# jaswon/osu-dreamer

Hardware: AMD Instinct MI355X
Metric: denoiser train-steps/sec + 50-step sample latents/sec, 1/2/4/8 MI355X (higher is better)
Workload: dtype bf16

## Files before the change

include/osu_dreamer_hip.h:

```cpp
#ifndef OSU_DREAMER_HIP_H
#define OSU_DREAMER_HIP_H

#ifdef __cplusplus
extern "C" {
#endif

enum { OD_F32 = 0, OD_BF16 = 1,
       OD_F32X3 = 2,
       OD_F32X3W = 3,
       OD_F16 = 4 };
enum { OD_EPI_NONE = 0, OD_EPI_SILU = 1 };
enum { OD_ACT_NONE = 0, OD_ACT_SILU = 1 };
enum { OD_ERR_ARG = -1, OD_ERR_ALIGN = -2, OD_ERR_UNSUPPORTED = -3, OD_ERR_COMM = -4 };

int od_version(void);
const char* od_build_source_sha(void);
const char* od_error_string(int code);

int od_gemm_nt(int dtype, const void* A, int lda, const void* W, int ldw, const float* bias, void* C, int ldc,
               int M, int N, int K, int epilogue, int accumulate, void* stream);
int od_gemm_nt_qkrope(int dtype, const void* A, int lda, const void* W, int ldw, const float* bias, void* C, int ldc, int M,
                      int N, int K, const float* wq, const float* wk, const float* table, int L, int H, int hd, float eps,
                      float q_scale, void* stream);
int od_gemm_nt_qkrope_split(int dtype, const void* A, int lda, const void* W, int ldw, const float* bias, void* C, int ldc,
                            void* qk_out, int ldqk, int qk_dtype, int M, int N, int K, const float* wq, const float* wk, const float* table,
                            int L, int H, int hd, float eps, float q_scale, void* stream);
int od_gemm_tn(int dtype, const void* G, int ldg, const void* A, int lda, float* dW, int lddw, float* dbias, int M, int N,
               int K, void* stream);
int od_gemm_tn_blocks(int dtype, const void* G, int ldg, const void* A, int lda, float* dW, int lddw, float* dbias, int M, int N,
                      int K, int n_block, int n_valid, void* stream);
int od_colsum(int dtype, const void* G, int ldg, float* out, int M, int N, void* stream);
int od_pack_weight(int dtype, const float* src, int N, int K, void* dst, int Np, int Kp, int transpose,
                   const int* row_map, void* stream);

int od_linear_small(const float* x, const float* W, const float* b, float* out, float* pre, int B, int N, int K, int act,
                    void* stream);
int od_linear_small_bwd(const float* x, const float* W, const float* pre, const float* dout, float* dpre, float* dW,
                        float* db, float* dx, int accumulate_dx, int B, int N, int K, int act, void* stream);

int od_cl_to_frames(int dtype, const float* src, void* dst, int ldd, int B, int C, int L, void* stream);
int od_feed_gather(const float* store, long store_elems, const long* base, const long* cstride, const int* lens, float* out,
                   int N, int C, int Lpad, void* stream);
int od_feed_gather_quant(const void* store, long store_bytes, int elem_size, const long* base, const long* cstride, const int* lens,
                         const double* scale, const double* offset, const int* flip, float* out, int N, int C, int c0, int Ctot,
                         int Lpad, void* stream);
int od_replicate_tail(float* x, const int* lens, const int* plens, int N, int C, int Lpad, void* stream);
int od_proj_in(int dtype, const float* xt, const float* W, const float* bias, void* x, int ldx, int B, int E, int L,
               int D, void* stream);
int od_proj_in_bwd(int dtype, const float* xt, const void* dx, int ldx, float* dW, float* db, int B, int E, int L, int D,
                   void* stream);
int od_silu(int dtype, const void* x, void* y, long n, void* stream);
int od_silu_bwd(int dtype, const void* x, const void* dy, void* dx, long n, void* stream);

int od_rmsnorm_film(int dtype, const void* x, int ldx, const float* ssg, const void* cl, int ldcl, int cl_bcast,
                    void* h, int ldh, float* inv_rms, int B, int L, int C, float eps, void* stream);
int od_rmsnorm_film_bwd(int dtype, const void* x, int ldx, const float* inv_rms, const float* ssg, const void* dh,
                        int lddh, void* dres, int lddres, float* dssg, int B, int L, int C, void* stream);
int od_rmsnorm_gate_residual(int dtype, const void* x, int ldx, const void* h, int ldh, const float* ssg, void* xo,
                             int ldxo, float* inv_rms, int B, int L, int C, float eps, void* stream);
int od_rmsnorm_gate_residual_film(int dtype, const void* x, int ldx, const void* h, int ldh, const float* ssg_a, void* xo, int ldxo,
                                  float* inv_a, const float* ssg_b, const void* cl, int ldcl, int cl_bcast, void* h2, int ldh2,
                                  float* inv_b, int B, int L, int C, float eps, void* stream);
int od_rmsnorm_gate_residual_film_dwconv(int dtype, const void* x, int ldx, const void* h, int ldh, const float* ssg_a, void* xo, int ldxo,
                                         float* inv_a, const float* ssg_b, void* h2, int ldh2, float* inv_b, const float* conv_w,
                                         const float* conv_b, void* y, int ldy, int B, int L, int C, int ksize, float eps, void* stream);
int od_rmsnorm_gate_residual_bwd(int dtype, const void* h, int ldh, const float* inv_rms, const float* ssg,
                                 const void* dy, int lddy, void* dh, int lddh, float* dssg, int B, int L, int C,
                                 void* stream);

int od_rope_table(float* table, int L, int hd, void* stream);
int od_qk_norm_rope(int dtype, const void* qkv, int ldqkv, const float* wq, const float* wk, const float* table,
                    void* qk_out, int ldo, int B, int L, int H, int hd, float eps, float q_scale, void* stream);
int od_qk_norm_rope_bwd(int dtype, const void* qkv, int ldqkv, const float* wq, const float* wk, const float* table,
                        const void* dqk, int lddqk, void* dqkv, int lddqkv, float* dwq, float* dwk, int B, int L,
                        int H, int hd, float eps, float q_scale, void* stream);
int od_flash_attn_fwd(int dtype, const void* q, int ldq, const void* k, int ldk, const void* v, int ldv, void* o, int ldo,
                      float* lse, int B, int H, int L, int hd, float scale, int q_prescaled, void* stream);
int od_flash_attn_fwd_varlen(int dtype, const void* q, int ldq, const void* k, int ldk, const void* v, int ldv, void* o, int ldo,
                             float* lse, const int* lens, int B, int H, int L, int hd, float scale, int q_prescaled, void* stream);
int od_flash_attn_bwd(int dtype, const void* q, int ldq, const void* k, int ldk, const void* v, int ldv, const void* o,
                      int ldo, const void* dout, int lddo, const float* lse, float* delta, void* dq, int lddq, void* dk,
                      int lddk, void* dv, int lddv, int B, int H, int L, int hd, float scale, int q_prescaled, void* stream);
int od_attn_aux_create(void** aux_out);
int od_attn_aux_destroy(void* aux);
int od_flash_attn_bwd_aux(int dtype, const void* q, int ldq, const void* k, int ldk, const void* v, int ldv, const void* o,
                          int ldo, const void* dout, int lddo, const float* lse, float* delta, void* dq, int lddq, void* dk,
                          int lddk, void* dv, int lddv, int B, int H, int L, int hd, float scale, int q_prescaled, void* aux, void* stream);
int od_flash_attn_bwd_varlen(int dtype, const void* q, int ldq, const void* k, int ldk, const void* v, int ldv, const void* o,
                             int ldo, const void* dout, int lddo, const float* lse, float* delta, void* dq, int lddq, void* dk,
                             int lddk, void* dv, int lddv, const int* lens, int B, int H, int L, int hd, float scale, int q_prescaled,
                             void* aux, void* stream);
int od_flash_attn_bwd_fused_ws_bytes(int dtype, int B, int H, int L, long* total_out, long* zero_out);
int od_flash_attn_bwd_fused(int dtype, const void* q, int ldq, const void* k, int ldk, const void* v, int ldv, const void* o, int ldo,
                            const void* dout, int lddo, const float* lse, void* dq, int lddq, void* dk, int lddk, void* dv, int lddv,
                            int B, int H, int L, int hd, float scale, int q_prescaled, void* ws, long ws_bytes, void* stream);
int od_flash_attn_bwd_fused_status(const void* ws, int* err_out, void* stream);
int od_flash_attn_bwd_fused_err_offset(void);
int od_flash_attn_bwd_fused_passes(void);
int od_flash_attn_bwd_fused_prof(void* ws, long* out16);
int od_flash_attn_bwd_passes(void);

int od_dwconv(int dtype, const void* x, int ldx, const float* w, const float* bias, void* y, int ldy, int B, int L,
              int C, int ksize, void* stream);
int od_dwconv_varlen(int dtype, const void* x, int ldx, const float* w, const float* bias, void* y, int ldy, const int* lens,
                     int B, int L, int C, int ksize, void* stream);
int od_dwconv_bwd(int dtype, const void* x, int ldx, const float* w, const void* dy, int lddy, void* dx, int lddx,
                  float* dw, float* db, int B, int L, int C, int ksize, void* stream);
int od_dwconv_bwd_varlen(int dtype, const void* x, int ldx, const float* w, const void* dy, int lddy, void* dx, int lddx,
                         float* dw, float* db, const int* lens, int B, int L, int C, int ksize, void* stream);
int od_scale_channels(int dtype, void* x, int ldx, const float* scale, int B, int L, int C, void* stream);
int od_swiglu_rmsnorm(int dtype, const void* vg, int ldvg, void* hh, int ldhh, float* inv_rms, int M, int Hf, int Hp,
                      float eps, void* stream);
int od_swiglu_rmsnorm_bwd(int dtype, const void* vg, int ldvg, const float* inv_rms, const void* dhh, int lddhh,
                          void* dvg, int lddvg, int M, int Hf, int Hp, void* stream);

int od_final_norm_proj_out(int dtype, const void* x, int ldx, const float* W, const float* bias, float* v,
                           float* inv_rms, int B, int L, int C, int E, float eps, void* stream);
int od_final_norm_proj_out_bwd(int dtype, const void* x, int ldx, const float* inv_rms, const float* W, const float* dv,
                               void* dx, int lddx, float* dW, float* db, int B, int L, int C, int E, void* stream);
int od_uhead_fwd(const float* xt, const float* w0, const float* b0, const float* w1, const float* b1, const float* w3,
                 const float* b3, const float* w4, const float* b4, float* fsum, int B, int E, int L, int U,
                 void* stream);
int od_uhead_fwd_varlen(const float* xt, const float* w0, const float* b0, const float* w1, const float* b1, const float* w3,
                        const float* b3, const float* w4, const float* b4, float* fsum, const int* lens, int B, int E, int L,
                        int U, void* stream);
int od_uhead_bwd(const float* xt, const float* w0, const float* b0, const float* w1, const float* b1, const float* w3,
                 const float* b3, const float* w4, const float* b4, const float* dfm, float* dw0, float* db0, float* dw1,
                 float* db1, float* dw3, float* db3, float* dw4, float* db4, int B, int E, int L, int U, void* stream);
int od_uhead_bwd_varlen(const float* xt, const float* w0, const float* b0, const float* w1, const float* b1, const float* w3,
                        const float* b3, const float* w4, const float* b4, const float* dfm, float* dw0, float* db0, float* dw1,
                        float* db1, float* dw3, float* db3, float* dw4, float* db4, const int* lens, int B, int E, int L, int U,
                        void* stream);
int od_uhead_tail(const float* fsum, const float* mod, const float* w_out, const float* b_out, float* u, int B, int U,
                  int L, float u_scale, void* stream);
int od_uhead_tail_varlen(const float* fsum, const float* mod, const float* w_out, const float* b_out, float* u, const int* lens,
                         int B, int U, int L, float u_scale, void* stream);
int od_uhead_tail_bwd(const float* fsum, const float* mod, const float* w_out, const float* b_out, const float* du,
                      float* dfm, float* dmod, float* dw_out, float* db_out, int B, int U, int L, float u_scale,
                      void* stream);
int od_uhead_tail_bwd_varlen(const float* fsum, const float* mod, const float* w_out, const float* b_out, const float* du,
                             float* dfm, float* dmod, float* dw_out, float* db_out, const int* lens, int B, int U, int L,
                             float u_scale, void* stream);

int od_make_xt(const float* x0, const float* x1, const float* t, float* xt, float* dsq, int B, int E, int L, void* stream);
int od_make_xt_varlen(const float* x0, const float* x1, const float* t, float* xt, float* dsq, const int* lens, int B, int E, int L,
                      void* stream);
int od_loss_grad(const float* xt, const float* x1, const float* u, const float* v, const float* dsq, float* dv,
                 float* sums, int B, int E, int L, float c0, float osl_w, float del_w, void* stream);
int od_loss_grad_varlen(const float* xt, const float* x1, const float* u, const float* v, const float* dsq, float* dv,
                        float* sums, const int* lens, int B, int E, int L, float c0, float osl_w, float del_w, void* stream);
int od_loss_finalize(const float* sums, const float* dsq, const float* u, float* out, float* du, int B, float c0,
                     float osl_w, float del_w, void* stream);
int od_sampler_step(float* x, const float* u, const float* v, const float* eta, int B, int E, int L, void* stream);
int od_sampler_eta(const float* u, float* eta, int B, float c0, int num_steps, void* stream);
int od_sampler_eta_groups(const float* u, const int* offs, float* eta, int G, float c0, int num_steps, void* stream);
int od_sampler_step_varlen(float* x, const float* u, const float* v, const float* eta, const int* lens, const int* offs, int G,
                           int B, int E, int L, void* stream);

int od_det_clear(void);
int od_det_register(const float* base, long count, void* shadow_i64);
int od_det_enable(void* table_dev, void* stream);
int od_det_table_bytes(void);
int od_det_flush(float* dst, long count, void* stream);

int od_sqnorm(const float* g, long n, float* out, const int* status, void* stream);
int od_adamw_ema(float* p, const float* g, float* m, float* v, float* ema, long n, float lr, float beta1, float beta2,
                 float eps, float weight_decay, int step, float ema_decay, int ema_mode, const float* gnorm_sq,
                 float max_norm, const int* status, void* stream);

int od_ema_update(float* ema, const float* p, long n, float ema_decay, int ema_mode, void* stream);

int od_style_conditioning(const float* labels, const float* rff_w, const float* rff_b, const float* cond_w,
                          const float* cond_b, const float* null_labels, float* c, int B, int NL, int F, int H,
                          void* stream);
int od_rmsnorm_rows(const float* x, const float* gamma, float* y, int M, int C, float eps, void* stream);

int od_style_conditioning_bwd(const float* labels, const float* rff_w, const float* rff_b, const float* dc, float* dcond_w,
                              float* dcond_b, float* dnull_labels, int B, int NL, int F, int H, void* stream);
int od_rmsnorm_rows_bwd(const float* x, const float* gamma, const float* dy, float* dx, float* dgamma, int M, int C, float eps,
                        int accumulate_dx, void* stream);
int od_cast_rows(int src_dtype, const void* src, int dst_dtype, void* dst, long n, void* stream);

int od_spec_features_conv(int dtype, const float* audio, const float* w1, const float* b1, const float* g1, const float* w2,
                          const float* b2, const float* g2, void* out, int ldo, int B, int F, int L, float eps, void* stream);
int od_rmsnorm_affine_film(int dtype, const void* x, int ldx, const float* gamma, const float* ssg, void* y, int ldy, int B,
                           int L, int C, float eps, int act, void* stream);
int od_rmsnorm_affine_gate_residual(int dtype, const void* x, int ldx, const void* h, int ldh, const float* gamma,
                                    const float* ssg, void* xo, int ldxo, int B, int L, int C, float eps, void* stream);
int od_unet_mixer(int dtype, const void* x, int ldx, const void* p, int ldp, int p_bcast, const void* gx, int ldg,
                  const float* gamma, void* xo, int ldxo, int B, int L, int C, float eps, void* stream);
int od_unet_down(int dtype, const void* x, int ldx, const float* w, const float* bias, void* y, int ldy, int B, int Lo, int C,
                 int stride, void* stream);
int od_unet_up(int dtype, const void* x, int ldx, const float* w, const float* bias, void* y, int ldy, int B, int Li, int C,
               int stride, void* stream);
int od_chart_head(int dtype, const void* x, int ldx, const float* W, const float* bias, float* out, int B, int L, int C, int N,
                  int n_sigmoid, int rms, float eps, void* stream);
int od_attn_pool(int dtype, const void* scores, int lds, const void* values, int ldv, float* out, int B, int L, int Hh, int hd,
                 void* stream);
int od_latent_bwd_block_frames(int C);
int od_rmsnorm_affine_film_bwd(int dtype, const void* x, int ldx, const float* gamma, const float* ssg, const void* dy, int lddy, void* dx,
                               int lddx, int accumulate_dx, float* dgamma, float* dssg, float* ws, long ws_floats, int B, int L, int C,
                               float eps, int act, void* stream);
int od_rmsnorm_affine_gate_residual_bwd(int dtype, const void* h, int ldh, const float* gamma, const float* ssg, const void* dxo, int lddxo,
                                        void* dh, int lddh, float* dgamma, float* dssg, float* ws, long ws_floats, int B, int L, int C,
                                        float eps, void* stream);
int od_unet_mixer_bwd(int dtype, const void* p, int ldp, int p_bcast, const void* gx, int ldg, const float* gamma, const void* dxo,
                      int lddxo, void* dp, int lddp, void* dgx, int lddg, float* dgamma, float* ws, long ws_floats, int B, int L, int C,
                      float eps, void* stream);
int od_unet_down_bwd(int dtype, const void* x, int ldx, const float* w, const void* dy, int lddy, void* dx, int lddx, float* dw, float* db,
                     float* ws, long ws_floats, int B, int Lo, int C, int stride, void* stream);
int od_unet_up_bwd(int dtype, const void* x, int ldx, const float* w, const void* dy, int lddy, void* dx, int lddx, float* dw, float* db,
                   float* ws, long ws_floats, int B, int Li, int C, int stride, void* stream);
int od_chart_head_bwd(int dtype, const void* x, int ldx, const float* W, const float* bias, const float* dout, void* dx, int lddx,
                      float* dW, float* db, float* ws, long ws_floats, int B, int L, int C, int N, int rms, float eps, void* stream);
int od_attn_pool_bwd(int dtype, const void* scores, int lds, const void* values, int ldv, const float* dout, void* dscores, int ldds,
                     void* dvalues, int lddv, int B, int L, int Hh, int hd, void* stream);
int od_spec_features_conv_bwd(int dtype, const float* audio, const float* w1, const float* b1, const float* g1, const float* w2,
                              const float* b2, const float* g2, const void* dout, int ldo, float* dw1, float* db1, float* dg1, float* dw2,
                              float* db2, float* dg2, float* ws, long ws_floats, int B, int F, int L, float eps, void* stream);
int od_add_rows(int dtype, const void* x, void* y, long n, void* stream);
int od_proj_in_bwd_input(int dtype, const void* dx, int ldx, const float* W, float* dxt, int B, int E, int L, int D, void* stream);

int od_mmd_imq(const float* z, const float* prior, float* out, float* dz, float* ws, long ws_floats, int N, int D, void* stream);
int od_scale_by(const float* x, const float* g, float* y, long n, void* stream);
int od_latent_perturb(const float* z, long zsb, long zse, long zsl, const float* s, const float* eps_z, const float* eps_s,
                      const float* u_s, const float* repl, const float* u_span, const float* u_start, float* z_out, float* s_out,
                      void* masked, void* start_span, int B2, int E, int l, int S, float s_noise, float z_noise, float s_mask_frac,
                      float z_mask_frac, int training, void* stream);
int od_latent_perturb_bwd(const float* dz_out, const float* ds_out, const void* masked, const int* start_span, float* dz, float* ds,
                          int B2, int E, int l, int S, void* stream);
int od_latent_loss_block_frames(void);
int od_latent_loss_ws_floats(int B2, int L);
int od_latent_loss(const float* logits, const float* chart, const float* pred_labels, const float* true_labels, const void* masked,
                   const float* s_reg, float* loss_ema, void* ema_init, float* out, float* coef, float* ws, long ws_floats, int B2, int L,
                   float s_reg_weight, int training, void* stream);
int od_latent_loss_bwd(const float* logits, const float* chart, const float* pred_labels, const float* true_labels, const void* masked,
                       const float* coef, const float* g, float* dlogits, float* dlabels, float* ds_reg, int B2, int L,
                       float s_reg_weight, void* stream);

int od_mmd_imq_pairs(const float* s, const float* prior, float* out, float* ws, long ws_floats, int G, int S, void* stream);
int od_latent_loss_maps(const float* logits, const float* chart, const int* hlens, const float* pred_labels, const float* true_labels,
                        const float* s_reg, int s_reg_stride, const float* loss_ema, float* out, float* ws, long ws_floats, int G,
                        int Hmax, float s_reg_weight, void* stream);
int od_latent_eval_maps_ws_floats(int G, int Pmax);
int od_latent_eval_maps(const float* chart, const float* pred_chart, const int* plens, const float* z, const int* zlens,
                        const float* pred_labels, const float* true_labels, float* out, float* ws, long ws_floats, int G, int Pmax, int E,
                        int lmax, void* stream);

int od_spec_features_conv_varlen(int dtype, const float* audio, const float* w1, const float* b1, const float* g1, const float* w2,
                                 const float* b2, const float* g2, void* out, int ldo, const int* lens, int B, int F, int L, float eps,
                                 void* stream);
int od_rmsnorm_affine_film_varlen(int dtype, const void* x, int ldx, const float* gamma, const float* ssg, void* y, int ldy,
                                  const int* lens, int B, int L, int C, float eps, int act, void* stream);
int od_unet_mixer_varlen(int dtype, const void* x, int ldx, const void* p, int ldp, const int* prow, const void* gx, int ldg,
                         const float* gamma, void* xo, int ldxo, int B, int L, int C, float eps, void* stream);
int od_unet_down_varlen(int dtype, const void* x, int ldx, const float* w, const float* bias, void* y, int ldy, const int* lens,
                        int B, int Lo, int C, int stride, void* stream);
int od_unet_up_varlen(int dtype, const void* x, int ldx, const float* w, const float* bias, void* y, int ldy, const int* lens,
                      int B, int Li, int C, int stride, void* stream);
int od_chart_head_varlen(int dtype, const void* x, int ldx, const float* W, const float* bias, float* out, const int* lens, int B,
                         int L, int C, int N, int n_sigmoid, int rms, float eps, void* stream);
int od_attn_pool_varlen(int dtype, const void* scores, int lds, const void* values, int ldv, float* out, const int* lens, int B,
                        int L, int Hh, int hd, void* stream);

int od_comm_load(const char* path);
int od_comm_version(void);
int od_comm_unique_id(void* out, int nbytes);
int od_comm_init(void** comm_out, int nranks, int rank, const void* unique_id, int nbytes);
int od_comm_destroy(void* comm);
int od_comm_abort(void* comm);
int od_comm_count(void* comm);
int od_comm_ring_standin(float* buf, long count, int channels, int threads, int rounds, void* stream);
int od_allreduce_grads(void* comm, float* grads, long count, int average, void* stream);
int od_broadcast_f32(void* comm, float* buf, long count, int root, void* stream);

int od_graph_begin(void* stream);
int od_graph_end(void* stream, void** graph_exec_out);
int od_graph_launch(void* graph_exec, void* stream);
int od_graph_destroy(void* graph_exec);

int od_mfma_calibrate(float* scratch, int iters, double* flops_out, void* stream);

#ifdef __cplusplus
}
#endif
#endif
```

osu_dreamer_amd/csrc/attn_bwd_fused.hip:

```cpp
#include "od_common.h"
#include "od_tiles.h"
#include "od_api_internal.h"
#include <type_traits>
#include <stddef.h>
#include <stdlib.h>

namespace {

constexpr float FB_LOG2E = 1.4426950408889634f;
constexpr float FB_LN2 = 0.6931471805599453f;

constexpr int FB_NK = 3;
constexpr int FB_KB = 4 * FB_NK * 16;
constexpr int FB_TILE = 64 * 128;
constexpr int FB_STAGE = 2 * FB_TILE + 512;
constexpr int FB_DS = FB_KB * 128;
#ifndef FB_NSLOTS
#define FB_NSLOTS 4
#endif
constexpr int FB_SLOTS = FB_NSLOTS;
#ifndef FB_PACK
#define FB_PACK 1
#endif
constexpr int FB_NP = FB_PACK ? 3 : 4;
constexpr int FB_RUN_TILE = 4 * FB_NP * 64 * 4;
constexpr int FB_KST = 2 * FB_STAGE + 2 * FB_DS;
constexpr int FB_SMEM = FB_KST + FB_DS + 16;

#ifndef FB_ORDER
#define FB_ORDER 3
#endif
#ifndef FB_REQ
#define FB_REQ 2
#endif
#ifndef FB_SPLIT
#define FB_SPLIT 1
#endif
#ifndef FB_X
#define FB_X 0
#endif

#if defined(OD_EMU)
#define FB_INLINE
#else
#define FB_INLINE __attribute__((always_inline))
#endif
#ifndef FB_PROF
#define FB_PROF 0
#endif
#if FB_PROF && !defined(OD_EMU)
#define FB_CLK() __builtin_readcyclecounter()
#else
#define FB_CLK() 0ull
#endif

struct FbSync {
    int head[8];
    int finished;
    int jobs_done;
    int err;
    int calls;
    int shape[3];
    int pad;
    unsigned long long prof[16];
};

__device__ __forceinline__ unsigned fb_f2u(float x) { return __builtin_bit_cast(unsigned, x); }
__device__ __forceinline__ float fb_u2f(unsigned x) { return __builtin_bit_cast(float, x); }

__device__ __forceinline__ float fb_poison() {
#if defined(OD_EMU)
    volatile unsigned bits = 0x7fc00000u;
    return fb_u2f(bits);
#else
    float x;
    asm volatile("v_mov_b32 %0, 0x7fc00000" : "=v"(x));
    return x;
#endif
}

__device__ __forceinline__ int fb_swz(int row) { return (row & 7) ^ (((row >> 3) & 1) << 2); }

#if defined(OD_EMU)
__device__ __forceinline__ int fb_xcc_id() { return (int)(blockIdx.x & 7); }
__device__ __forceinline__ int fb_flag_load(const int* p) { return *p; }
__device__ __forceinline__ void fb_flag_store(int* p, int v) { *p = v; }
struct fb_rsrc_t { const unsigned char* base; };
__device__ __forceinline__ fb_rsrc_t fb_make_rsrc(const float* base, unsigned) { return fb_rsrc_t{(const unsigned char*)base}; }
__device__ __forceinline__ f32x4 fb_ld_l2(fb_rsrc_t r, unsigned voff, unsigned soff) { return *(const f32x4*)(r.base + voff + soff); }
__device__ __forceinline__ void fb_st_run(float* p, f32x4 t) { *(f32x4*)p = t; }
__device__ __forceinline__ void fb_sleep() {}
__device__ __forceinline__ unsigned long long fb_now(unsigned polls) { return polls; }
__device__ __forceinline__ int fb_atomic_inc(int* p) { return atomicAdd(p, 1); }
#define FB_WAIT_ALL() ((void)0)
#define FB_COMPILER_FENCE() ((void)0)
#define FB_WAIT_BUT(n) ((void)0)
#else
__device__ __forceinline__ int fb_xcc_id() {
    int v;
    asm volatile("s_getreg_b32 %0, hwreg(HW_REG_XCC_ID)" : "=s"(v));
    return v & 7;
}
__device__ __forceinline__ int fb_flag_load(const int* p) { return __hip_atomic_load(p, __ATOMIC_RELAXED, __HIP_MEMORY_SCOPE_AGENT); }
__device__ __forceinline__ void fb_flag_store(int* p, int v) { __hip_atomic_store(p, v, __ATOMIC_RELAXED, __HIP_MEMORY_SCOPE_AGENT); }
#ifndef FB_LD_AUX
#define FB_LD_AUX 2
#endif
typedef __amdgpu_buffer_rsrc_t fb_rsrc_t;
__device__ __forceinline__ fb_rsrc_t fb_make_rsrc(const float* base, unsigned bytes) {
    return __builtin_amdgcn_make_buffer_rsrc((void*)base, 0, (int)bytes, 0x00020000);
}
__device__ __forceinline__ f32x4 fb_ld_l2(fb_rsrc_t r, unsigned voff, unsigned soff) {
    return __builtin_bit_cast(f32x4, __builtin_amdgcn_raw_buffer_load_b128(r, (int)voff, (int)soff, FB_LD_AUX));
}
#ifndef FB_ST_POLICY
#define FB_ST_POLICY 0
#endif
__device__ __forceinline__ void fb_st_run(float* p, f32x4 t) {
#if FB_X & 16
    asm volatile("" :: "v"(t));
#elif FB_ST_POLICY == 0
    *(f32x4*)p = t;
#elif FB_ST_POLICY == 1
    asm volatile("global_store_dwordx4 %0, %1, off nt\n\ts_nop 0" :: "v"(p), "v"(t) : "memory");
#elif FB_ST_POLICY == 2
    asm volatile("global_store_dwordx4 %0, %1, off sc1\n\ts_nop 0" :: "v"(p), "v"(t) : "memory");
#else
    asm volatile("global_store_dwordx4 %0, %1, off sc0 sc1\n\ts_nop 0" :: "v"(p), "v"(t) : "memory");
#endif
}
__device__ __forceinline__ void fb_sleep() { __builtin_amdgcn_s_sleep(4); }
__device__ __forceinline__ unsigned long long fb_now(unsigned) { return __builtin_amdgcn_s_memrealtime(); }
__device__ __forceinline__ int fb_atomic_inc(int* p) { return __hip_atomic_fetch_add(p, 1, __ATOMIC_RELAXED, __HIP_MEMORY_SCOPE_AGENT); }
#define FB_WAIT_ALL() asm volatile("s_waitcnt vmcnt(0)" ::: "memory")
#define FB_COMPILER_FENCE() asm volatile("" ::: "memory")
#define FB_WAIT_BUT(n) asm volatile("s_waitcnt vmcnt(" #n ")" ::: "memory")
#endif

__global__ __launch_bounds__(256) void fb_prep_kernel(const bf16_t* __restrict__ o, int ldo, const bf16_t* __restrict__ dout, int lddo,
                                                      const float* __restrict__ lse, float* __restrict__ nl, float* __restrict__ nd,
                                                      int B, int H, int L, float inv_scale) {
    const int lane = threadIdx.x & 63;
    const long m = (long)blockIdx.x * 4 + (threadIdx.x >> 6);
    if (m >= (long)B * L) return;
    const int b = (int)(m / L), l = (int)(m % L);
    const int nch = H * 8;
    for (int it = 0; it * 64 < nch; it++) {
        const int qd = it * 64 + lane;
        const bool act = qd < nch;
        float s = 0.f;
        if (act) {
            float a[8], d[8];
            od_ld8(o + m * ldo + qd * 8, a); od_ld8(dout + m * lddo + qd * 8, d);
#pragma unroll
            for (int e = 0; e < 8; e++) s += a[e] * d[e];
        }
        s += __shfl_xor(s, 1); s += __shfl_xor(s, 2); s += __shfl_xor(s, 4);
        if (act && (qd & 7) == 0) {
            const size_t i = ((size_t)b * H + (qd >> 3)) * L + l;
            nd[i] = -s;
            nl[i] = -lse[i] * inv_scale;
        }
    }
}

__global__ __launch_bounds__(256) void fb_amax_kernel(const bf16_t* __restrict__ dout, int lddo, long M, int dh, unsigned* __restrict__ amax_bits) {
    const int nch = dh / 8;
    float m = 0.f;
    for (long i = (long)blockIdx.x * 256 + threadIdx.x; i < M * nch; i += (long)gridDim.x * 256) {
        float d[8];
        od_ld8(dout + (i / nch) * lddo + (i % nch) * 8, d);
#pragma unroll
        for (int e = 0; e < 8; e++) m = fmaxf(m, fabsf(d[e]));
    }
#pragma unroll
    for (int s = 32; s >= 1; s >>= 1) m = fmaxf(m, __shfl_xor(m, s));
    if ((threadIdx.x & 63) == 0 && m > 0.f) atomicMax(amax_bits, fb_f2u(m));
}
__device__ __forceinline__ float fb_dscale_of(unsigned amax_bits) {
    const unsigned e = (amax_bits >> 23) & 0xffu;
    if (amax_bits == 0u || e == 0u || e == 0xffu) return 1.0f;
    const int ex = (int)e - 127 + ((amax_bits & 0x7fffffu) ? 1 : 0);
    int se = 2 - ex; se = se < -100 ? -100 : se > 100 ? 100 : se;
    return fb_u2f((unsigned)(se + 127) << 23);
}
__global__ __launch_bounds__(256) void fb_prep_f16_kernel(const bf16_t* __restrict__ o, int ldo, const bf16_t* __restrict__ dout, int lddo,
                                                          const float* __restrict__ lse, float* __restrict__ nl, float* __restrict__ nd,
                                                          f16_t* __restrict__ do16, int ldd16, const unsigned* __restrict__ amax_bits,
                                                          float* __restrict__ dscale_out, int B, int H, int L, float inv_scale) {
    const float ds = fb_dscale_of(amax_bits[0]);
    if (blockIdx.x == 0 && threadIdx.x == 0) dscale_out[0] = ds;
    const int lane = threadIdx.x & 63;
    const long m = (long)blockIdx.x * 4 + (threadIdx.x >> 6);
    if (m >= (long)B * L) return;
    const int b = (int)(m / L), l = (int)(m % L);
    const int nch = H * 8;
    for (int it = 0; it * 64 < nch; it++) {
        const int qd = it * 64 + lane;
        const bool act = qd < nch;
        float s = 0.f;
        if (act) {
            float a[8], d[8];
            od_ld8(o + m * ldo + qd * 8, a); od_ld8(dout + m * lddo + qd * 8, d);
#pragma unroll
            for (int e = 0; e < 8; e++) { s += a[e] * d[e]; d[e] *= ds; }
            od_st8(do16 + m * ldd16 + qd * 8, d);
        }
        s += __shfl_xor(s, 1); s += __shfl_xor(s, 2); s += __shfl_xor(s, 4);
        if (act && (qd & 7) == 0) {
            const size_t i = ((size_t)b * H + (qd >> 3)) * L + l;
            nd[i] = -s * ds;
            nl[i] = -lse[i] * inv_scale;
        }
    }
}

template <bool PRE, class TA>
__global__ __launch_bounds__(512, 2) void flash_bwd_fused_kernel(const bf16_t* __restrict__ q, int ldq, const bf16_t* __restrict__ k, int ldk,
                                                                 const bf16_t* __restrict__ v, int ldv, const bf16_t* __restrict__ dout, int lddo,
                                                                 const float* __restrict__ nl, const float* __restrict__ nd,
                                                                 bf16_t* __restrict__ dq, int lddq, bf16_t* __restrict__ dk, int lddk,
                                                                 bf16_t* __restrict__ dv, int lddv, float* __restrict__ run,
                                                                 FbSync* __restrict__ sync, int B, int H, int L, float scale,
                                                                 unsigned wait_ticks, const float* __restrict__ dscale_p) {
    constexpr int NK = FB_NK, KB = FB_KB;
    OD_DYN_SMEM(smem);
    int* const s_job = (int*)(smem + FB_KST + FB_DS);
    const int BH = B * H, nkb = (L + KB - 1) / KB, nqt = (L + 63) / 64;
    const int jobs_per_xcd = ((BH + 7) / 8) * nkb;
    const int lane = threadIdx.x & 63, wave = od_uniform(threadIdx.x >> 6), x = lane & 15, g = lane >> 4;
    const bool key_wave = wave < 4;
    const int xcc = fb_xcc_id();
    const int calls = sync->calls;
    {
        const int s0 = sync->shape[0], s1 = sync->shape[1], s2 = sync->shape[2];
        if ((s0 | s1 | s2) != 0 && (s0 != B || s1 != H || s2 != L)) {
            if (blockIdx.x == 0 && threadIdx.x == 0) fb_flag_store(&sync->err, 2);
            return;
        }
    }
    const float inv_ds = std::is_same<TA, f16_t>::value ? 1.0f / dscale_p[0] : 1.0f;
    const float c = scale * FB_LOG2E, out_scale = (PRE ? FB_LN2 : scale) * inv_ds;
    int my_jobs = 0;

    if (threadIdx.x == 0) s_job[0] = fb_atomic_inc(&sync->head[xcc]);
    __syncthreads();
    int job = od_uniform(s_job[0]), jpar = 0;
    auto run_jobs = [&](auto role_) FB_INLINE {
    constexpr bool KEY_ROLE = decltype(role_)::value;
    for (;; jpar ^= 1) {
        if (job >= jobs_per_xcd) break;
        my_jobs++;
        const int bh = (job / nkb) * 8 + xcc, kblk = job % nkb;
        if (bh >= BH) {
            __syncthreads();
            if (threadIdx.x == 0) s_job[jpar ^ 1] = fb_atomic_inc(&sync->head[xcc]);
            __syncthreads();
            job = od_uniform(s_job[jpar ^ 1]);
            continue;
        }
        const int b = bh / H, h = bh % H;
        const bf16_t* qb = q + (size_t)b * L * ldq + h * 64;
        const bf16_t* kb_ = k + (size_t)b * L * ldk + h * 64;
        const bf16_t* vb = v + (size_t)b * L * ldv + h * 64;
        const bf16_t* dob = dout + (size_t)b * L * lddo + h * 64;
        const bool kragged = kblk * KB + KB > L;
#ifndef FB_PRIO
#define FB_PRIO 0
#endif
        if constexpr (KEY_ROLE) {
            if (FB_PRIO) __builtin_amdgcn_s_setprio(FB_PRIO);
            const int key0 = kblk * KB + wave * NK * 16;
            od_frag<TA> fk[NK][2], fv[NK][2];
#pragma unroll
            for (int ki = 0; ki < NK; ki++) {
                int row = key0 + ki * 16 + x; row = row < L ? row : L - 1;
#pragma unroll
                for (int s = 0; s < 2; s++) {
                    od_frag_load(fk[ki][s], (const TA*)(kb_ + (size_t)row * ldk + s * 32 + g * 8));
                    od_frag_load(fv[ki][s], (const TA*)(vb + (size_t)row * ldv + s * 32 + g * 8));
                }
            }
            f32x4 dkacc[NK][4], dvacc[NK][4];
#pragma unroll
            for (int ki = 0; ki < NK; ki++)
#pragma unroll
                for (int dt = 0; dt < 4; dt++) { dkacc[ki][dt] = (f32x4)(0.f); dvacc[ki][dt] = (f32x4)(0.f); }
            const int ds_off0 = (wave * 48 + x) * 128 + ((g ^ fb_swz(x)) << 4);
            __syncthreads();
            unsigned long long pk_bar = 0;
            int next_job = 0;
            auto tile = [&](int qt, auto masked_t) FB_INLINE {
                constexpr bool MASKED = decltype(masked_t)::value;
                const bool last_tile = qt == nqt - 1;
                if (last_tile && threadIdx.x == 0) next_job = fb_atomic_inc(&sync->head[xcc]);
                const unsigned char* st = smem + (qt & 1) * FB_STAGE;
                unsigned char* dsb = smem + 2 * FB_STAGE + (qt & 1) * FB_DS;
                const unsigned char* tQ = st;
                const unsigned char* tO = st + FB_TILE;
                const float* s_nl = (const float*)(st + 2 * FB_TILE);
                const float* s_nd = s_nl + 64;
                const int qbase = qt * 64;
#pragma unroll
                for (int u = 0; u < 2; u++) {
                    od_frag<TA> fp[NK], fds[NK];
#pragma unroll
                    for (int th = 0; th < 2; th++) {
                        const int t4 = 2 * u + th;
                        od_frag<TA> fqr[2], fdo[2];
#pragma unroll
                        for (int s = 0; s < 2; s++) {
                            if ((FB_X & 1024) && t4) { fqr[s] = fk[0][s]; fdo[s] = fv[0][s]; continue; }
                            frag_contig<128>(fqr[s], tQ, t4 * 16 + x, s * 32 + g * 8);
                            frag_contig<128>(fdo[s], tO, t4 * 16 + x, s * 32 + g * 8);
                        }
                        const f32x4 l4 = *(const f32x4*)(s_nl + t4 * 16 + 4 * g);
                        const f32x4 d4 = *(const f32x4*)(s_nd + t4 * 16 + 4 * g);
#pragma unroll
                        for (int ki = 0; ki < NK; ki++) {
                            f32x4 sa_ = l4, pa_ = d4;
#pragma unroll
                            for (int s = 0; s < 2; s++) { sa_ = od_mma(fqr[s], fk[ki][s], sa_); pa_ = od_mma(fdo[s], fv[ki][s], pa_); }
                            f32x4 e = sa_;
                            if constexpr (!PRE) e = od_mul4s(sa_, c);
                            f32x4 p;
#pragma unroll
                            for (int r = 0; r < 4; r++) p[r] = (FB_X & 256) ? e[r] : od_exp2(e[r]);
                            if constexpr (MASKED) {
                                const bool kvalid = key0 + ki * 16 + x < L;
#pragma unroll
                                for (int r = 0; r < 4; r++)
                                    if (!(kvalid && (qbase + t4 * 16 + 4 * g + r < L))) p[r] = 0.f;
                            }
                            const f32x4 ds = od_mul4(p, pa_);
                            od_frag_set4(fp[ki], th, p[0], p[1], p[2], p[3]);
                            od_frag_set4(fds[ki], th, ds[0], ds[1], ds[2], ds[3]);
                        }
                    }
                    od_frag<TA> fot[2], fqt[2];
                    frag_cols<128, 128>(fot[0], tO, tO, 0, x, u, g);
                    frag_cols<128, 128>(fqt[0], tQ, tQ, 0, x, u, g);
#pragma unroll
                    for (int dt = 0; dt < 4; dt++) {
                        if (dt < 3 && !(FB_X & 512)) {
                            frag_cols<128, 128>(fot[(dt + 1) & 1], tO, tO, (dt + 1) * 16, x, u, g);
                            frag_cols<128, 128>(fqt[(dt + 1) & 1], tQ, tQ, (dt + 1) * 16, x, u, g);
                        }
                        if (dt < NK && !(FB_X & 4)) *(s16x8*)(dsb + ((ds_off0 ^ (u * 64)) + dt * 2048)) = fds[dt].v;
                        __builtin_amdgcn_sched_barrier(0);
#pragma unroll
                        for (int ki = 0; ki < NK; ki++) {
                            dvacc[ki][dt] = od_mma(fot[dt & 1], fp[ki], dvacc[ki][dt]);
                            dkacc[ki][dt] = od_mma(fqt[dt & 1], fds[ki], dkacc[ki][dt]);
                        }
                        __builtin_amdgcn_sched_barrier(0);
                    }
                }
                if (last_tile && threadIdx.x == 0) s_job[jpar ^ 1] = next_job;
                const unsigned long long tb0 = FB_CLK();
                __syncthreads();
                pk_bar += FB_CLK() - tb0;
            };
            const unsigned long long tk0 = FB_CLK();
            const int nfull = kragged ? 0 : L / 64;
            for (int qt = 0; qt < nfull; qt++) tile(qt, std::false_type{});
            for (int qt = nfull; qt < nqt; qt++) tile(qt, std::true_type{});
            if (FB_PROF && threadIdx.x == 0) { atomicAdd(&sync->prof[0], pk_bar); atomicAdd(&sync->prof[1], FB_CLK() - tk0); }
#pragma unroll
            for (int ki = 0; ki < NK; ki++) {
                const int row = key0 + ki * 16 + x;
                if (row < L) {
                    bf16_t* dkr = dk + ((size_t)b * L + row) * lddk + h * 64;
                    bf16_t* dvr = dv + ((size_t)b * L + row) * lddv + h * 64;
#pragma unroll
                    for (int dt = 0; dt < 4; dt++) {
                        const f32x4 a = dkacc[ki][dt] * out_scale, e = dvacc[ki][dt] * inv_ds;
                        u32x2 w0, w1;
                        w0[0] = od_pack_bf2(a[0], a[1]); w0[1] = od_pack_bf2(a[2], a[3]);
                        w1[0] = od_pack_bf2(e[0], e[1]); w1[1] = od_pack_bf2(e[2], e[3]);
                        *(u32x2*)(dkr + dt * 16 + 4 * g) = w0;
                        *(u32x2*)(dvr + dt * 16 + 4 * g) = w1;
                    }
                }
            }
        } else {
            const int hh = wave - 4;
            constexpr int NJ = FB_SPLIT == 0 ? 1 : FB_SPLIT == 1 ? 4 : 2, NG = 4 / NJ;
            auto ji_of = [](int a) FB_INLINE { return FB_SPLIT == 0 ? 0 : FB_SPLIT == 1 ? a : a >> 1; };
            auto gi_of = [](int a) FB_INLINE { return FB_SPLIT == 0 ? a : FB_SPLIT == 1 ? 0 : a & 1; };
            const int j0 = FB_SPLIT == 0 ? hh : FB_SPLIT == 1 ? 0 : 2 * (hh & 1), G0 = FB_SPLIT == 0 ? 0 : FB_SPLIT == 1 ? hh : 2 * (hh >> 1);
            od_frag<TA> fkt[NJ][6];
            const od_srd_t rq = od_make_srd(qb, (unsigned)(((size_t)(L - 1) * ldq + 64) * 2));
            const od_srd_t ro = od_make_srd(dob, (unsigned)(((size_t)(L - 1) * lddo + 64) * 2));
            const od_srd_t rs = od_make_srd((hh == 0 ? nl : nd) + (size_t)bh * L, (unsigned)L * 4u);
            const int prow = lane >> 3, pslot = (lane & 7) ^ prow;
            const unsigned vq = (unsigned)((hh * 8 + prow) * ldq * 2 + pslot * 16), vo = (unsigned)((hh * 8 + prow) * lddo * 2 + pslot * 16);
            const unsigned smem_a = od_lds_addr(smem);
            const od_srd_t rk = od_make_srd(kb_, (unsigned)(((size_t)(L - 1) * ldk + 64) * 2));
            auto stage_k = [&]() FB_INLINE {
#pragma unroll
                for (int i = 0; i < 6; i++) {
                    const int pc = hh + 4 * i;
                    const int r = 8 * pc + (lane >> 3);
                    const unsigned vk = (unsigned)((lane >> 3) * ldk * 2 + (((lane & 7) ^ fb_swz(r)) << 4));
                    od_buffer_lds16_at(rk, vk, (unsigned)od_uniform((kblk * KB + 8 * pc) * ldk * 2), (unsigned)od_uniform((int)(smem_a + (unsigned)FB_KST + (unsigned)pc * 1024u)));
                }
            };
            int trk[NJ][2];
#pragma unroll
            for (int ji = 0; ji < NJ; ji++)
#pragma unroll
                for (int e = 0; e < 2; e++) {
                    const int row = 8 * g + (x >> 2) + 4 * e;
                    trk[ji][e] = row * 128 + (((2 * (j0 + ji) + ((x & 3) >> 1)) ^ fb_swz(row)) << 4) + (x & 1) * 8;
                }
            auto dma_piece = [&](int qt, int j) FB_INLINE {
                const unsigned st = (unsigned)od_uniform((int)(smem_a + (unsigned)((qt & 1) * FB_STAGE) + (unsigned)hh * 1024u));
                const unsigned qi = (unsigned)od_uniform(qt);
                const unsigned sq = qi * 64u * (unsigned)ldq * 2u, so = qi * 64u * (unsigned)lddo * 2u;
                if (j == 0) od_buffer_lds16_at(rq, vq, sq, st);
                if (j == 1) od_buffer_lds16_at(rq, vq, sq + 32u * (unsigned)ldq * 2u, st + 4096);
                if (j == 2) od_buffer_lds16_at(ro, vo, so, st + FB_TILE);
                if (j == 3) od_buffer_lds16_at(ro, vo, so + 32u * (unsigned)lddo * 2u, st + FB_TILE + 4096);
                if (j == 4 && hh < 2) od_buffer_lds4_at(rs, (unsigned)lane * 4u, qi * 256u, (unsigned)od_uniform((int)(st + 2 * FB_TILE - (unsigned)hh * 768u)));
            };
            auto dma = [&](int qt) FB_INLINE {
                qt = od_uniform(qt);
#pragma unroll
                for (int j = 0; j < 5; j++) dma_piece(qt, j);
            };
            int tr_off[NG][2], qcol[NG];
#pragma unroll
            for (int gi = 0; gi < NG; gi++) {
                const int G = G0 + gi;
#pragma unroll
                for (int e = 0; e < 2; e++) {
                    const int row = 8 * g + (x >> 2) + 4 * e;
                    tr_off[gi][e] = row * 128 + (((2 * G + ((x & 3) >> 1)) ^ fb_swz(row)) << 4) + (x & 1) * 8;
                }
                qcol[gi] = 16 * (2 * (G >> 1) + ((x >> 2) & 1)) + 4 * (2 * (G & 1) + (x >> 3)) + (x & 3);
            }

            f32x4 acc[4][4], rb[FB_NP];
            bool poisoned = false;
            unsigned long long ph[6] = {0, 0, 0, 0, 0, 0};
            const size_t tile_f = FB_RUN_TILE;
            const bool last = kblk == nkb - 1;
            const int bhq = bh >> 3, slot = bhq % FB_SLOTS, gen = bhq / FB_SLOTS;
            const int nbhq_x = (BH - xcc + 7) >> 3;
            const int gens = (nbhq_x - slot + FB_SLOTS - 1) / FB_SLOTS;
            const unsigned id_mine = (unsigned)od_uniform((int)((1u + ((unsigned)calls * (unsigned)gens + (unsigned)gen) * (unsigned)nkb + (unsigned)kblk) & 0xfffu)), id_pred = (id_mine - 1u) & 0xfffu;
            auto tag_of = [](unsigned id, int r) FB_INLINE -> unsigned { return (id >> (3 * r)) & 7u; };
            auto phase_b = [&](int tau, f32x4 (&a)[4], auto&& between) FB_INLINE {
                const unsigned char* dsb = smem + 2 * FB_STAGE + (tau & 1) * FB_DS;
                s16x4 f[2][NG][2];
                auto rd = [&](int s, s16x4 (&dst)[NG][2]) FB_INLINE {
#pragma unroll
                    for (int gi = 0; gi < NG; gi++)
#pragma unroll
                        for (int e = 0; e < 2; e++) dst[gi][e] = od_lds_tr_read((const bf16_t*)(dsb + s * 4096 + tr_off[gi][e]));
                };
                rd(0, f[0]);
#pragma unroll
                for (int s = 0; s < 6; s++) {
                    if (s + 1 < 6) rd(s + 1, f[(s + 1) & 1]);
                    __builtin_amdgcn_sched_barrier(0);
                    od_frag<TA> fb[NG];
#pragma unroll
                    for (int gi = 0; gi < NG; gi++) {
                        const s16x4 b0 = f[s & 1][gi][0], b1 = f[s & 1][gi][1];
                        fb[gi].v[0] = b0[0]; fb[gi].v[1] = b0[1]; fb[gi].v[2] = b0[2]; fb[gi].v[3] = b0[3];
                        fb[gi].v[4] = b1[0]; fb[gi].v[5] = b1[1]; fb[gi].v[6] = b1[2]; fb[gi].v[7] = b1[3];
                    }
#pragma unroll
                    for (int G = 0; G < 4; G++) a[G] = od_mma(fkt[ji_of(G)][s], fb[gi_of(G)], s == 0 ? (f32x4)(0.f) : a[G]);
                    __builtin_amdgcn_sched_barrier(0);
                    between(s);
                }
            };
            const size_t rbh = (size_t)od_uniform(xcc * FB_SLOTS + slot);
            const fb_rsrc_t run_rs = fb_make_rsrc(run + rbh * nqt * tile_f, (unsigned)((size_t)nqt * tile_f * 4));
            const unsigned run_vo = (unsigned)((hh * (FB_NP * 256) + lane * 4) * 4);
            float* const run_st = run + rbh * nqt * tile_f + (size_t)hh * (FB_NP * 256) + (size_t)lane * 4;
            auto chain_load = [&](int tau, f32x4 (&r4)[FB_NP]) FB_INLINE {
#pragma unroll
                for (int G = 0; G < FB_NP; G++) r4[G] = fb_ld_l2(run_rs, run_vo + G * 1024, (unsigned)((FB_X & 8) ? 0 : tau) * (unsigned)(FB_RUN_TILE * 4));
            };
            auto tags_good = [&](f32x4 (&r4)[FB_NP]) FB_INLINE -> bool {
                unsigned bad = 0;
#if FB_PACK
#pragma unroll
                for (int P = 0; P < FB_NP; P++) bad |= ((fb_f2u(r4[P][3]) >> 14) ^ id_pred) & 0x3ffu;
                if (FB_X & 32) return true;
                return !__any(bad != 0);
#else
#pragma unroll
                for (int G = 0; G < 4; G++)
#pragma unroll
                    for (int r = 0; r < 4; r++) bad |= fb_f2u(r4[G][r]) ^ tag_of(id_pred, r);
                if (FB_X & 32) return true;
                return !__any((bad & 7u) != 0);
#endif
            };
#if FB_PACK
            auto fb_unpack = [&](const f32x4 (&r4)[FB_NP], float (&v)[16]) FB_INLINE {
                unsigned last = 0;
#pragma unroll
                for (int P = 0; P < 3; P++) {
                    const unsigned d0 = fb_f2u(r4[P][0]), d1 = fb_f2u(r4[P][1]), d2 = fb_f2u(r4[P][2]), d3 = fb_f2u(r4[P][3]);
                    v[5 * P + 0] = fb_u2f(d0 << 10);
                    v[5 * P + 1] = fb_u2f(((d0 >> 22) | (d1 << 10)) << 10);
                    v[5 * P + 2] = fb_u2f(((d1 >> 12) | (d2 << 20)) << 10);
                    v[5 * P + 3] = fb_u2f((d2 << 8) & 0xfffffc00u);
                    v[5 * P + 4] = fb_u2f(((d2 >> 24) | (d3 << 8)) << 10);
                    last |= (d3 >> 24) << (P == 0 ? 0 : P == 1 ? 8 : 15);
                }
                v[15] = fb_u2f(last << 10);
            };
            auto fb_pack = [&](const float (&v)[16], unsigned id, f32x4 (&out)[FB_NP]) FB_INLINE {
                unsigned u[16];
#pragma unroll
                for (int i = 0; i < 16; i++) u[i] = (fb_f2u(v[i]) + 0x200u) >> 10;
#pragma unroll
                for (int P = 0; P < 3; P++) {
                    const unsigned a0 = u[5 * P], a1 = u[5 * P + 1], a2 = u[5 * P + 2], a3 = u[5 * P + 3], a4 = u[5 * P + 4];
                    const unsigned ex = P == 0 ? (u[15] & 0xffu) : P == 1 ? ((u[15] >> 8) & 0x7fu) : (u[15] >> 15);
                    out[P][0] = fb_u2f(a0 | (a1 << 22));
                    out[P][1] = fb_u2f((a1 >> 10) | (a2 << 12));
                    out[P][2] = fb_u2f((a2 >> 20) | (a3 << 2) | (a4 << 24));
                    out[P][3] = fb_u2f((a4 >> 8) | ((id & 0x3ffu) << 14) | (ex << 24));
                }
            };
#endif
            auto chain_commit = [&](int tau, f32x4 (&a)[4]) FB_INLINE {
#if FB_PACK
                {
                    float rv[16];
                    fb_unpack(rb, rv);
                    if (poisoned) {
#pragma unroll
                        for (int i = 0; i < 16; i++) rv[i] = fb_poison();
                    }
#pragma unroll
                    for (int G = 0; G < 4; G++)
#pragma unroll
                        for (int r = 0; r < 4; r++) a[G][r] += rv[4 * G + r];
                }
                if (!last) {
                    float sv[16];
#pragma unroll
                    for (int G = 0; G < 4; G++)
#pragma unroll
                        for (int r = 0; r < 4; r++) sv[4 * G + r] = a[G][r];
                    f32x4 t3[FB_NP];
                    fb_pack(sv, id_mine, t3);
#pragma unroll
                    for (int P = 0; P < FB_NP; P++) fb_st_run(run_st + (size_t)((FB_X & 8) ? 0 : tau) * tile_f + P * 256, t3[P]);
                } else {
#else
#pragma unroll
                for (int G = 0; G < 4; G++)
#pragma unroll
                    for (int r = 0; r < 4; r++) a[G][r] += fb_u2f(fb_f2u(rb[G][r]) & ~7u);
                if (!last) {
#pragma unroll
                    for (int G = 0; G < 4; G++) {
                        f32x4 t;
#pragma unroll
                        for (int r = 0; r < 4; r++) t[r] = fb_u2f((fb_f2u(a[G][r]) & ~7u) | tag_of(id_mine, r));
                        fb_st_run(run_st + (size_t)((FB_X & 8) ? 0 : tau) * tile_f + G * 256, t);
                    }
                } else {
#endif
#pragma unroll
                    for (int G = 0; G < 4; G++) {
                        const int qrow = tau * 64 + qcol[gi_of(G)];
                        if (qrow < L) {
                            u32x2 w;
                            w[0] = od_pack_bf2(a[G][0] * out_scale, a[G][1] * out_scale);
                            w[1] = od_pack_bf2(a[G][2] * out_scale, a[G][3] * out_scale);
                            *(u32x2*)(dq + ((size_t)b * L + qrow) * lddq + h * 64 + 16 * (j0 + ji_of(G)) + 4 * g) = w;
                        }
                    }
                    f32x4 t;
#if FB_PACK
                    t[0] = t[1] = t[2] = 0.f; t[3] = fb_u2f((id_mine & 0x3ffu) << 14);
#else
#pragma unroll
                    for (int r = 0; r < 4; r++) t[r] = fb_u2f(tag_of(id_mine, r));
#endif
#pragma unroll
                    for (int G = 0; G < FB_NP; G++) fb_st_run(run_st + (size_t)((FB_X & 8) ? 0 : tau) * tile_f + G * 256, t);
                }
            };
            auto commit_dyn = [&](int tau) FB_INLINE {
                switch (tau & 3) {
                    case 0: chain_commit(tau, acc[0]); break;
                    case 1: chain_commit(tau, acc[1]); break;
                    case 2: chain_commit(tau, acc[2]); break;
                    default: chain_commit(tau, acc[3]); break;
                }
            };
            int done = 0;
            bool inflight = false, aborted = false;
            auto chain_request = [&](int produced) FB_INLINE {
                if ((FB_X & 1) || inflight || done >= produced) return;
                if (!(FB_X & 64)) chain_load(done, rb);
                inflight = true;
            };
            auto chain_try = [&](int produced, int must_reach) FB_INLINE -> bool {
                if (FB_X & 1) { done = produced; return false; }
                bool four = false;
                if (done < produced) {
                    if (inflight) {
                        inflight = false;
                        if (tags_good(rb)) { commit_dyn(done); done++; four = !last; }
                        else if (FB_PROF) ph[5]++;
                    }
                }
                while (done < must_reach) {
                    four = false;
                    if (!aborted) {
                        unsigned long long t_start = 0;
                        for (unsigned polls = 0;; polls++) {
                            FB_COMPILER_FENCE();
                            chain_load(done, rb);
                            if (tags_good(rb)) break;
                            if ((polls & 15u) == 15u) {
                                const unsigned long long now = fb_now(polls);
                                if (polls == 15u) t_start = now;
                                else if (now - t_start > (unsigned long long)wait_ticks) aborted = true;
                                if (od_uniform(fb_flag_load(&sync->err)) == 3) aborted = true;
                                if (aborted) break;
                            }
                            fb_sleep();
                        }
                    }
                    if (aborted) {
                        if (lane == 0) fb_flag_store(&sync->err, 3);
#pragma unroll
                        for (int G = 0; G < FB_NP; G++) rb[G] = (f32x4)(fb_poison());
                        poisoned = true;
                    }
                    commit_dyn(done);
                    poisoned = false;
                    done++;
                }
                return four;
            };
            auto step = [&](int it, auto k_) FB_INLINE {
                constexpr int K = decltype(k_)::value;
                const unsigned long long t0 = FB_CLK();
                const int nxt = od_uniform(it + 1);
                const unsigned long long t1 = FB_CLK();
                if (!(FB_X & 2)) phase_b(it - 1, acc[(K + 3) & 3], [&](int s) FB_INLINE {
#if FB_ORDER == 2
                    if (s < 5) { if (nxt < nqt) dma_piece(nxt, s); }
                    else chain_request(it - 1);
#elif FB_ORDER == 1
                    if (s == 0) chain_request(it - 1);
                    else if (nxt < nqt) dma_piece(nxt, s - 1);
#else
                    if (s < 2) { if (nxt < nqt) { dma_piece(nxt, 2 * s); dma_piece(nxt, 2 * s + 1); } }
                    else if (s == 2) { if (nxt < nqt) dma_piece(nxt, 4); }
                    if (s == FB_REQ) chain_request(it - 1);
#endif
                });
                else { chain_request(it - 1); if (nxt < nqt) dma(nxt); }
#if FB_PROF && !defined(OD_EMU)
                asm volatile("" : "+v"(acc[(K + 3) & 3][0]), "+v"(acc[(K + 3) & 3][1]), "+v"(acc[(K + 3) & 3][2]), "+v"(acc[(K + 3) & 3][3]));
#endif
                const unsigned long long t2 = FB_CLK();
                FB_WAIT_ALL();
                const unsigned long long t3 = FB_CLK();
                const bool four = chain_try(it, it - 3);
                const unsigned long long t4 = FB_CLK();
                (void)four;
                od_barrier_raw();
                if (FB_PROF) { const unsigned long long t5 = FB_CLK(); ph[0] += t1 - t0; ph[1] += t2 - t1; ph[2] += t3 - t2; ph[3] += t4 - t3; ph[4] += t5 - t4; }
            };
            OD_DRAIN_VMEM();
            stage_k();
            dma(0);
            FB_WAIT_ALL();
            od_barrier_raw();
#pragma unroll
            for (int s = 0; s < 6; s++)
#pragma unroll
                for (int ji = 0; ji < NJ; ji++) {
                    const s16x4 b0 = od_lds_tr_read((const bf16_t*)(smem + FB_KST + s * 4096 + trk[ji][0]));
                    const s16x4 b1 = od_lds_tr_read((const bf16_t*)(smem + FB_KST + s * 4096 + trk[ji][1]));
                    fkt[ji][s].v[0] = b0[0]; fkt[ji][s].v[1] = b0[1]; fkt[ji][s].v[2] = b0[2]; fkt[ji][s].v[3] = b0[3];
                    fkt[ji][s].v[4] = b1[0]; fkt[ji][s].v[5] = b1[1]; fkt[ji][s].v[6] = b1[2]; fkt[ji][s].v[7] = b1[3];
                }
            if (1 < nqt) dma(1);
            FB_WAIT_ALL();
            od_barrier_raw();
            int it = 1;
            for (; it + 3 < nqt; it += 4) {
                step(it, std::integral_constant<int, 1>{}); step(it + 1, std::integral_constant<int, 2>{});
                step(it + 2, std::integral_constant<int, 3>{}); step(it + 3, std::integral_constant<int, 0>{});
            }
            if (it < nqt) { step(it, std::integral_constant<int, 1>{}); it++; }
            if (it < nqt) { step(it, std::integral_constant<int, 2>{}); it++; }
            if (it < nqt) { step(it, std::integral_constant<int, 3>{}); it++; }
            if (!(FB_X & 2)) {
                auto nothing = [](int) FB_INLINE {};
                switch ((nqt - 1) & 3) {
                    case 0: phase_b(nqt - 1, acc[0], nothing); break;
                    case 1: phase_b(nqt - 1, acc[1], nothing); break;
                    case 2: phase_b(nqt - 1, acc[2], nothing); break;
                    default: phase_b(nqt - 1, acc[3], nothing); break;
                }
            }
            inflight = false;
            chain_try(nqt, nqt);
            if (FB_PROF && threadIdx.x == 256) { for (int i = 0; i < 6; i++) atomicAdd(&sync->prof[2 + i], ph[i]); }
            FB_WAIT_ALL();
        }
        job = od_uniform(s_job[jpar ^ 1]);
    }
    };
    if (key_wave) run_jobs(std::true_type{}); else run_jobs(std::false_type{});
    if (threadIdx.x == 0) {
        if (my_jobs) {
#if defined(OD_EMU)
            sync->jobs_done += my_jobs;
#else
            __hip_atomic_fetch_add(&sync->jobs_done, my_jobs, __ATOMIC_RELAXED, __HIP_MEMORY_SCOPE_AGENT);
#endif
        }
#if !defined(OD_EMU)
        __builtin_amdgcn_fence(__ATOMIC_RELEASE, "agent");
        asm volatile("s_waitcnt vmcnt(0)" ::: "memory");
#endif
        const int t = fb_atomic_inc(&sync->finished);
        if (t == (int)gridDim.x - 1) {
#if !defined(OD_EMU)
            __builtin_amdgcn_fence(__ATOMIC_ACQUIRE, "agent");
#endif
            const int done = fb_flag_load(&sync->jobs_done);
            if (done != 8 * jobs_per_xcd) fb_flag_store(&sync->err, 1);
            for (int i = 0; i < 8; i++) fb_flag_store(&sync->head[i], 0);
            fb_flag_store(&sync->jobs_done, 0);
            fb_flag_store(&sync->calls, sync->calls + 1);
            fb_flag_store(&sync->shape[0], B); fb_flag_store(&sync->shape[1], H); fb_flag_store(&sync->shape[2], L);
            fb_flag_store(&sync->finished, 0);
        }
    }
}

inline size_t fb_align(size_t n) { return (n + 255) & ~(size_t)255; }
struct FbLayout { size_t sync, nl, nd, run, aux, do16, total; };
inline FbLayout fb_layout(int B, int H, int L, bool f16 = false) {
    const size_t BH = (size_t)B * H, nqt = (size_t)(L + 63) / 64;
    FbLayout l;
    l.sync = 0;
    l.run = fb_align(sizeof(FbSync));
    l.nl = l.run + fb_align((size_t)8 * FB_SLOTS * nqt * FB_RUN_TILE * sizeof(float));
    l.nd = l.nl + fb_align(BH * L * sizeof(float));
    l.aux = l.nd + fb_align(BH * L * sizeof(float));
    l.do16 = l.aux + 256;
    l.total = f16 ? l.do16 + fb_align(BH * L * 64 * sizeof(unsigned short)) : l.aux;
    return l;
}

inline unsigned fb_wait_ticks() {
    static const unsigned ticks = [] {
        const char* e = getenv("OD_FB_CHAIN_TIMEOUT_MS");
        long ms = e ? atol(e) : 1000;
        if (ms < 1) ms = 1;
        if (ms > 40000) ms = 40000;
#if defined(OD_EMU)
        return (unsigned)1024;
#else
        return (unsigned)(ms * 100000);
#endif
    }();
    return ticks;
}

}

extern "C" int od_flash_attn_bwd_fused_ws_bytes(int dtype, int B, int H, int L, long* total_out, long* zero_out) {
    if (B <= 0 || H <= 0 || L <= 0 || !total_out || !zero_out || (dtype != OD_BF16 && dtype != OD_F16)) return OD_ERR_ARG;
    const FbLayout lay = fb_layout(B, H, L, dtype == OD_F16);
    *total_out = (long)lay.total;
    *zero_out = (long)lay.nl;
    return 0;
}
extern "C" int od_flash_attn_bwd_fused_err_offset(void) { return (int)offsetof(FbSync, err); }
extern "C" int od_flash_attn_bwd_fused_passes(void) { return 5; }
extern "C" int od_flash_attn_bwd_fused_prof(void* ws, long* out16) {
    if (!ws || !out16) return OD_ERR_ARG;
    FbSync s;
#if defined(OD_EMU)
    s = *(FbSync*)ws;
#else
    if (hipDeviceSynchronize() != hipSuccess) return OD_ERR_ARG;
    if (hipMemcpy(&s, ws, sizeof(s), hipMemcpyDeviceToHost) != hipSuccess) return OD_ERR_ARG;
    if (hipMemset((unsigned char*)ws + offsetof(FbSync, prof), 0, sizeof(s.prof)) != hipSuccess) return OD_ERR_ARG;
#endif
    for (int i = 0; i < 16; i++) out16[i] = (long)s.prof[i];
    return 0;
}

extern "C" int od_flash_attn_bwd_fused(int dtype, const void* q, int ldq, const void* k, int ldk, const void* v, int ldv, const void* o, int ldo,
                                       const void* dout, int lddo, const float* lse, void* dq, int lddq, void* dk, int lddk, void* dv, int lddv,
                                       int B, int H, int L, int hd, float scale, int q_prescaled, void* ws, long ws_bytes, void* stream) {
    if ((dtype != OD_BF16 && dtype != OD_F16) || hd != 64) return OD_ERR_UNSUPPORTED;
    if (!ws || B <= 0 || H <= 0 || L <= 0) return OD_ERR_ARG;
    if (ldq % 8 || ldk % 8 || ldv % 8 || ldo % 8 || lddo % 8 || lddq % 8 || lddk % 8 || lddv % 8) return OD_ERR_ALIGN;
    const bool f16 = dtype == OD_F16;
    const FbLayout lay = fb_layout(B, H, L, f16);
    if (ws_bytes < (long)lay.total) return OD_ERR_ARG;
    if (((size_t)L * (size_t)(ldq > lddo ? (ldq > ldk ? ldq : ldk) : (lddo > ldk ? lddo : ldk))) * 2 >= 0xffffffffull) return OD_ERR_UNSUPPORTED;
    hipStream_t st = (hipStream_t)stream;
    unsigned char* w = (unsigned char*)ws;
    float* nl = (float*)(w + lay.nl);
    float* nd = (float*)(w + lay.nd);
    const long M = (long)B * L;
    const float inv_scale = q_prescaled ? FB_LOG2E : 1.0f / scale;
    const float* dscale_p = nullptr;
    if (f16) {
        unsigned* amax = (unsigned*)(w + lay.aux);
        float* dsc = (float*)(w + lay.aux) + 1;
        f16_t* do16 = (f16_t*)(w + lay.do16);
#if defined(OD_EMU)
        *amax = 0u;
#else
        if (hipMemsetAsync(amax, 0, sizeof(unsigned), st) != hipSuccess) return OD_ERR_ARG;
#endif
        OD_LAUNCH(fb_amax_kernel, dim3(2048), dim3(256), 0, st, (const bf16_t*)dout, lddo, M, H * 64, amax);
        OD_LAUNCH(fb_prep_f16_kernel, dim3((unsigned)((M + 3) / 4)), dim3(256), 0, st, (const bf16_t*)o, ldo, (const bf16_t*)dout, lddo, lse, nl, nd,
                  do16, H * 64, (const unsigned*)amax, dsc, B, H, L, inv_scale);
        dout = do16; lddo = H * 64; dscale_p = dsc;
    } else
        OD_LAUNCH(fb_prep_kernel, dim3((unsigned)((M + 3) / 4)), dim3(256), 0, st, (const bf16_t*)o, ldo, (const bf16_t*)dout, lddo, lse, nl, nd, B, H, L, inv_scale);
    const int grid = od_num_cus();
#define FB_ARGS dim3(grid), dim3(512), FB_SMEM, st, (const bf16_t*)q, ldq, (const bf16_t*)k, ldk, (const bf16_t*)v, ldv, (const bf16_t*)dout, lddo, \
        (const float*)nl, (const float*)nd, (bf16_t*)dq, lddq, (bf16_t*)dk, lddk, (bf16_t*)dv, lddv, (float*)(w + lay.run), (FbSync*)(w + lay.sync), B, H, L, scale, \
        fb_wait_ticks(), dscale_p
#define FB_LAUNCH_X(...) OD_LAUNCH_DYN(__VA_ARGS__)
    if (f16) {
        if (q_prescaled) FB_LAUNCH_X((flash_bwd_fused_kernel<true, f16_t>), FB_ARGS);
        else FB_LAUNCH_X((flash_bwd_fused_kernel<false, f16_t>), FB_ARGS);
    } else {
        if (q_prescaled) FB_LAUNCH_X((flash_bwd_fused_kernel<true, bf16_t>), FB_ARGS);
        else FB_LAUNCH_X((flash_bwd_fused_kernel<false, bf16_t>), FB_ARGS);
    }
#undef FB_LAUNCH_X
#undef FB_ARGS
    OD_CHECK_LAUNCH();
    return 0;
}

extern "C" int od_flash_attn_bwd_fused_status(const void* ws, int* err_out, void* stream) {
    if (!ws || !err_out) return OD_ERR_ARG;
#if defined(OD_EMU)
    (void)stream;
    *err_out = ((const FbSync*)ws)->err;
#else
    int v = -1;
    hipError_t e = hipMemcpyAsync(&v, (const unsigned char*)ws + offsetof(FbSync, err), sizeof(int), hipMemcpyDeviceToHost, (hipStream_t)stream);
    if (e == hipSuccess) e = hipStreamSynchronize((hipStream_t)stream);
    if (e != hipSuccess) return -(int)e - 1000;
    *err_out = v;
#endif
    return 0;
}
```

osu_dreamer_amd/csrc/rowops.hip:

```cpp
#include "od_common.h"
#include "od_api_internal.h"

namespace {

#ifndef OD_QK_BPW
#define OD_QK_BPW 8
#endif
constexpr int ROWS_PER_WAVE_BWD = 16;

template <class T, int NCH>
__device__ __forceinline__ void load_row(const T* row, int C, int lane, float (&v)[NCH][8]) {
#pragma unroll
    for (int i = 0; i < NCH; i++) {
        const int c = (lane + 64 * i) * 8;
        if (c < C) od_ld8(row + c, v[i]);
        else {
#pragma unroll
            for (int e = 0; e < 8; e++) v[i][e] = 0.f;
        }
    }
}
template <int NCH>
__device__ __forceinline__ float row_sumsq(const float (&v)[NCH][8]) {
    float s = 0.f;
// ... 259 lines not shown
#pragma unroll
            for (int k = 0; k < 8; k++) {
                float s = bv[k];
#pragma unroll
                for (int j = 0; j < KS; j++) s += wv[k][j] * win[j][k];
                o[k] = s;
            }
            od_st8(y + ((size_t)b * L + lc) * ldy + c, o);
        }
#pragma unroll
        for (int j = 0; j < KS - 1; j++)
#pragma unroll
            for (int e = 0; e < 8; e++) win[j][e] = win[j + 1][e];
    }
}

template <class T, int NCH>
__global__ __launch_bounds__(256) void rmsnorm_gate_res_bwd_kernel(const T* __restrict__ h, int ldh, const float* __restrict__ inv_rms,
                                                                   const float* __restrict__ ssg, const T* __restrict__ dy, int lddy,
                                                                   T* __restrict__ dh, int lddh, float* __restrict__ dssg,
                                                                   int B, int L, int C, const OdDetTable* __restrict__ det) {
    __shared__ float red[NCH * 512];
    const int lane = threadIdx.x & 63, wave = threadIdx.x >> 6;
    const int b = blockIdx.y;
    const int l0 = (blockIdx.x * 4 + wave) * ROWS_PER_WAVE_BWD;
    float dg[NCH][8], gate[NCH][8];
#pragma unroll
    for (int i = 0; i < NCH; i++) {
        const int c = (lane + 64 * i) * 8;
#pragma unroll
        for (int e = 0; e < 8; e++) { dg[i][e] = 0.f; gate[i][e] = 0.f; }
        if (c < C) od_ld8(ssg + (size_t)b * 3 * C + 2 * C + c, gate[i]);
    }
    for (int r = 0; r < ROWS_PER_WAVE_BWD; r++) {
        const int l = l0 + r;
        if (l >= L) break;
        const long m = (long)b * L + l;
        float hv[NCH][8], gv[NCH][8];
        load_row<T, NCH>(h + m * ldh, C, lane, hv);
        load_row<T, NCH>(dy + m * lddy, C, lane, gv);
        const float inv = inv_rms[m];
        float dot = 0.f;
#pragma unroll
        for (int i = 0; i < NCH; i++)
#pragma unroll
            for (int e = 0; e < 8; e++) {
                const float hh = hv[i][e] * inv;
                dg[i][e] += gv[i][e] * hh;
                gv[i][e] *= gate[i][e];
                dot += gv[i][e] * hh;
                hv[i][e] = hh;
            }
        dot = od_wave_sum(dot) / (float)C;
#pragma unroll
        for (int i = 0; i < NCH; i++) {
            const int c = (lane + 64 * i) * 8;
            if (c >= C) continue;
            float o[8];
#pragma unroll
            for (int e = 0; e < 8; e++) o[e] = inv * (gv[i][e] - hv[i][e] * dot);
            od_st8(dh + m * lddh + c, o);
        }
    }
    for (int w = 0; w < 4; w++) {
        if (wave == w) {
#pragma unroll
            for (int i = 0; i < NCH; i++)
#pragma unroll
                for (int e = 0; e < 8; e++) {
                    const int idx = (lane + 64 * i) * 8 + e;
                    if (w == 0) red[idx] = dg[i][e]; else red[idx] += dg[i][e];
                }
        }
        __syncthreads();
    }
    for (int c = threadIdx.x; c < C; c += 256) od_red_add(det, dssg + (size_t)b * 3 * C + 2 * C + c, red[c]);
}

template <class T, int NCH>
__global__ __launch_bounds__(256) void swiglu_rmsnorm_kernel(const T* __restrict__ vg, int ldvg, T* __restrict__ hh, int ldhh,
                                                             float* __restrict__ inv_rms, long M, int Hf, int Hp, float eps) {
    const int lane = threadIdx.x & 63;
    const long m = (long)blockIdx.x * 4 + (threadIdx.x >> 6);
    if (m >= M) return;
    float v[NCH][8], g[NCH][8];
    load_row<T, NCH>(vg + m * ldvg, Hp, lane, v);
    load_row<T, NCH>(vg + m * ldvg + Hp, Hp, lane, g);
#pragma unroll
    for (int i = 0; i < NCH; i++)
#pragma unroll
        for (int e = 0; e < 8; e++) v[i][e] *= od_silu(g[i][e]);
    const float inv = rsqrtf(row_sumsq<NCH>(v) / (float)Hf + eps);
    if (lane == 0 && inv_rms) inv_rms[m] = inv;
#pragma unroll
    for (int i = 0; i < NCH; i++) {
        const int c = (lane + 64 * i) * 8;
        if (c >= Hp) continue;
        float o[8];
#pragma unroll
        for (int e = 0; e < 8; e++) o[e] = v[i][e] * inv;
        od_st8(hh + m * ldhh + c, o);
    }
}

template <class T, int NCH>
__global__ __launch_bounds__(256) void swiglu_rmsnorm_bwd_kernel(const T* __restrict__ vg, int ldvg, const float* __restrict__ inv_rms,
                                                                 const T* __restrict__ dhh, int lddhh, T* __restrict__ dvg, int lddvg,
                                                                 long M, int Hf, int Hp) {
    const int lane = threadIdx.x & 63;
    const long m = (long)blockIdx.x * 4 + (threadIdx.x >> 6);
    if (m >= M) return;
    float v[NCH][8], g[NCH][8], d[NCH][8];
    load_row<T, NCH>(vg + m * ldvg, Hp, lane, v);
    load_row<T, NCH>(vg + m * ldvg + Hp, Hp, lane, g);
    load_row<T, NCH>(dhh + m * lddhh, Hp, lane, d);
    const float inv = inv_rms[m];
    float dot = 0.f;
    float sg[NCH][8], gs[NCH][8];
#pragma unroll
    for (int i = 0; i < NCH; i++)
#pragma unroll
        for (int e = 0; e < 8; e++) {
            gs[i][e] = od_sigmoid(g[i][e]);
            sg[i][e] = g[i][e] * gs[i][e];
            dot += d[i][e] * (v[i][e] * sg[i][e] * inv);
        }
    dot = od_wave_sum(dot) / (float)Hf;
#pragma unroll
    for (int i = 0; i < NCH; i++) {
        const int c = (lane + 64 * i) * 8;
        if (c >= Hp) continue;
        float ov[8], og[8];
#pragma unroll
        for (int e = 0; e < 8; e++) {
            const float sh = v[i][e] * sg[i][e] * inv;
            const float ds = inv * (d[i][e] - sh * dot);
            ov[e] = ds * sg[i][e];
            og[e] = ds * v[i][e] * (gs[i][e] * (1.0f + g[i][e] * (1.0f - gs[i][e])));
        }
        od_st8(dvg + m * lddvg + c, ov);
        od_st8(dvg + m * lddvg + Hp + c, og);
    }
}

template <class T, int NCH>
__global__ __launch_bounds__(256) void final_proj_kernel(const T* __restrict__ x, int ldx, const float* __restrict__ W,
                                                         const float* __restrict__ bias, float* __restrict__ vout,
                                                         float* __restrict__ inv_rms, int B, int L, int C, int E, float eps) {
    const int lane = threadIdx.x & 63;
    const long m = (long)blockIdx.x * 4 + (threadIdx.x >> 6);
    if (m >= (long)B * L) return;
    const int b = (int)(m / L), l = (int)(m % L);
    float v[NCH][8];
    load_row<T, NCH>(x + m * ldx, C, lane, v);
    const float inv = rsqrtf(row_sumsq<NCH>(v) / (float)C + eps);
    if (lane == 0 && inv_rms) inv_rms[m] = inv;
    for (int e = 0; e < E; e++) {
        float s = 0.f;
#pragma unroll
        for (int i = 0; i < NCH; i++) {
            const int c = (lane + 64 * i) * 8;
            if (c >= C) continue;
            float w[8]; od_ld8(W + (size_t)e * C + c, w);
#pragma unroll
            for (int k = 0; k < 8; k++) s += w[k] * v[i][k];
        }
        s = od_wave_sum(s) * inv;
        if (lane == 0) vout[((size_t)b * E + e) * L + l] = s + bias[e];
    }
}

template <class T, int NCH>
__global__ __launch_bounds__(256) void final_proj_bwd_kernel(const T* __restrict__ x, int ldx, const float* __restrict__ inv_rms,
                                                             const float* __restrict__ W, const float* __restrict__ dv,
                                                             T* __restrict__ dx, int lddx, float* __restrict__ dW,
                                                             float* __restrict__ db, int B, int L, int C, int E,
                                                             const OdDetTable* __restrict__ det) {
    constexpr int MAXE = 8;
    __shared__ float red[MAXE * NCH * 512];
    __shared__ float redb[4][MAXE];
    const int lane = threadIdx.x & 63, wave = threadIdx.x >> 6;
    const int b = blockIdx.y;
    const int l0 = (blockIdx.x * 4 + wave) * ROWS_PER_WAVE_BWD;
    float wv[MAXE][NCH][8], dw[MAXE][NCH][8], dbv[MAXE];
#pragma unroll
    for (int e = 0; e < MAXE; e++) {
        dbv[e] = 0.f;
#pragma unroll
        for (int i = 0; i < NCH; i++) {
            const int c = (lane + 64 * i) * 8;
#pragma unroll
            for (int k = 0; k < 8; k++) { wv[e][i][k] = 0.f; dw[e][i][k] = 0.f; }
            if (e < E && c < C) od_ld8(W + (size_t)e * C + c, wv[e][i]);
        }
    }
    for (int r = 0; r < ROWS_PER_WAVE_BWD; r++) {
        const int l = l0 + r;
        if (l >= L) break;
        const long m = (long)b * L + l;
        float xv[NCH][8], dn[NCH][8], dve[MAXE];
        load_row<T, NCH>(x + m * ldx, C, lane, xv);
        const float inv = inv_rms[m];
#pragma unroll
        for (int e = 0; e < MAXE; e++) { dve[e] = e < E ? dv[((size_t)b * E + e) * L + l] : 0.f; dbv[e] += dve[e]; }
        float dot = 0.f;
#pragma unroll
        for (int i = 0; i < NCH; i++)
#pragma unroll
            for (int k = 0; k < 8; k++) {
                const float xh = xv[i][k] * inv;
                float s = 0.f;
#pragma unroll
                for (int e = 0; e < MAXE; e++) { s += dve[e] * wv[e][i][k]; dw[e][i][k] += dve[e] * xh; }
                dn[i][k] = s;
                dot += s * xh;
                xv[i][k] = xh;
            }
        dot = od_wave_sum(dot) / (float)C;
#pragma unroll
        for (int i = 0; i < NCH; i++) {
            const int c = (lane + 64 * i) * 8;
            if (c >= C) continue;
            float o[8];
#pragma unroll
            for (int k = 0; k < 8; k++) o[k] = inv * (dn[i][k] - xv[i][k] * dot);
            od_st8(dx + m * lddx + c, o);
        }
    }
    if (lane == 0)
        for (int e = 0; e < MAXE; e++) redb[wave][e] = dbv[e];
    for (int w = 0; w < 4; w++) {
        if (wave == w) {
#pragma unroll
            for (int e = 0; e < MAXE; e++)
#pragma unroll
                for (int i = 0; i < NCH; i++)
#pragma unroll
                    for (int k = 0; k < 8; k++) {
                        const int idx = e * NCH * 512 + (lane + 64 * i) * 8 + k;
                        if (w == 0) red[idx] = dw[e][i][k]; else red[idx] += dw[e][i][k];
                    }
        }
        __syncthreads();
    }
    for (int e = 0; e < E; e++)
        for (int c = threadIdx.x; c < C; c += 256) od_red_add(det, dW + (size_t)e * C + c, red[e * NCH * 512 + c]);
    if (threadIdx.x < E) od_red_add(det, db + threadIdx.x, redb[0][threadIdx.x] + redb[1][threadIdx.x] + redb[2][threadIdx.x] + redb[3][threadIdx.x]);
}

template <class T, class TO = T>
__global__ __launch_bounds__(256) void qk_norm_rope_kernel(const T* __restrict__ qkv, int ldqkv, const float* __restrict__ wq,
                                                           const float* __restrict__ wk, const float* __restrict__ table,
                                                           TO* __restrict__ out, int ldo, int B, int L, int H, int hd, float eps,
                                                           float q_scale) {
    const int lane = threadIdx.x & 63;
    const long m = (long)blockIdx.x * 4 + (threadIdx.x >> 6);
    if (m >= (long)B * L) return;
    const int l = (int)(m % L);
    const int lph = hd / 8, half = lph / 2;
    const int nchunks = 2 * H * lph;
    const int niter = (nchunks + 63) / 64;
    for (int it = 0; it < niter; it++) {
        const int q = it * 64 + lane;
        const bool act = q < nchunks;
        const int slot = q / lph, c8 = q % lph;
        float v[8];
        if (act) od_ld8(qkv + m * ldqkv + (size_t)slot * hd + c8 * 8, v);
        else {
#pragma unroll
            for (int e = 0; e < 8; e++) v[e] = 0.f;
        }
        float ss = 0.f;
#pragma unroll
        for (int e = 0; e < 8; e++) ss += v[e] * v[e];
        for (int msk = 1; msk < lph; msk <<= 1) ss += __shfl_xor(ss, msk);
        const float inv = rsqrtf(ss / (float)hd + eps);
        const float* w = (slot < H ? wq : wk) + c8 * 8;
        float y[8], p[8];
#pragma unroll
        for (int e = 0; e < 8; e++) y[e] = act ? v[e] * inv * w[e] : 0.f;
#pragma unroll
        for (int e = 0; e < 8; e++) p[e] = __shfl_xor(y[e], half);
        if (act) {
            const bool first = c8 < half;
            const int j0 = (c8 % half) * 8;
            const float* tb = table + ((size_t)l * (hd / 2) + j0) * 2;
            float o[8];
#pragma unroll
            for (int e = 0; e < 8; e++) {
                const float cs = tb[2 * e], sn = tb[2 * e + 1];
                o[e] = (first ? (y[e] * cs - p[e] * sn) : (p[e] * sn + y[e] * cs)) * (slot < H ? q_scale : 1.f);
            }
            od_st8(out + m * ldo + (size_t)slot * hd + c8 * 8, o);
        }
    }
}

template <class T>
__global__ __launch_bounds__(256) void qk_norm_rope_bwd_kernel(const T* __restrict__ qkv, int ldqkv, const float* __restrict__ wq,
                                                               const float* __restrict__ wk, const float* __restrict__ table,
                                                               const T* __restrict__ dqk, int lddqk, T* __restrict__ dqkv, int lddqkv,
                                                               float* __restrict__ dwq, float* __restrict__ dwk,
                                                               int B, int L, int H, int hd, float eps, float q_scale,
                                                               const OdDetTable* __restrict__ det) {
    __shared__ long long sdw[2][256];
    __shared__ int s_bad;
    const int lane = threadIdx.x & 63, wave = threadIdx.x >> 6;
    for (int i = threadIdx.x; i < 512; i += 256) sdw[i >> 8][i & 255] = 0;
    if (threadIdx.x == 0) s_bad = 0;
    __syncthreads();
    const int lph = hd / 8, half = lph / 2;
    const int nchunks = 2 * H * lph;
    const int niter = (nchunks + 63) / 64;
    float aq[8], ak[8];
#pragma unroll
    for (int e = 0; e < 8; e++) { aq[e] = 0.f; ak[e] = 0.f; }
    const long M = (long)B * L;
    const long mbase = ((long)blockIdx.x * 4 + wave) * ROWS_PER_WAVE_BWD;
    for (int r = 0; r < ROWS_PER_WAVE_BWD; r++) {
        const long m = mbase + r;
        if (m >= M) break;
        const int l = (int)(m % L);
        for (int it = 0; it < niter; it++) {
            const int q = it * 64 + lane;
            const bool act = q < nchunks;
            const int slot = q / lph, c8 = q % lph;
            float v[8], d[8];
            if (act) {
                od_ld8(qkv + m * ldqkv + (size_t)slot * hd + c8 * 8, v); od_ld8(dqk + m * lddqk + (size_t)slot * hd + c8 * 8, d);
                if (slot < H) {
#pragma unroll
                    for (int e = 0; e < 8; e++) d[e] *= q_scale;
                }
            } else {
#pragma unroll
                for (int e = 0; e < 8; e++) { v[e] = 0.f; d[e] = 0.f; }
            }
            float ss = 0.f;
#pragma unroll
            for (int e = 0; e < 8; e++) ss += v[e] * v[e];
            for (int msk = 1; msk < lph; msk <<= 1) ss += __shfl_xor(ss, msk);
            const float inv = rsqrtf(ss / (float)hd + eps);
            float p[8], dy[8];
#pragma unroll
            for (int e = 0; e < 8; e++) p[e] = __shfl_xor(d[e], half);
            const bool first = c8 < half;
            const int j0 = (c8 % (half > 0 ? half : 1)) * 8;
            const float* tb = table + ((size_t)l * (hd / 2) + j0) * 2;
            const float* w = (slot < H ? wq : wk) + c8 * 8;
            float dot = 0.f;
#pragma unroll
            for (int e = 0; e < 8; e++) {
                const float cs = act ? tb[2 * e] : 0.f, sn = act ? tb[2 * e + 1] : 0.f;
                dy[e] = first ? (d[e] * cs + p[e] * sn) : (-p[e] * sn + d[e] * cs);
                const float xh = v[e] * inv;
                const float wv = act ? w[e] : 0.f;
                if (act) { if (slot < H) aq[e] += dy[e] * xh; else ak[e] += dy[e] * xh; }
                dy[e] *= wv;
                dot += dy[e] * xh;
                v[e] = xh;
            }
            for (int msk = 1; msk < lph; msk <<= 1) dot += __shfl_xor(dot, msk);
            dot /= (float)hd;
            if (act) {
                float o[8];
#pragma unroll
                for (int e = 0; e < 8; e++) o[e] = inv * (dy[e] - v[e] * dot);
                od_st8(dqkv + m * lddqkv + (size_t)slot * hd + c8 * 8, o);
            }
        }
    }
    const int c8 = lane % lph;
#pragma unroll
    for (int e = 0; e < 8; e++) {
        od_lds_fix_add(&sdw[0][c8 * 8 + e], aq[e], &s_bad);
        od_lds_fix_add(&sdw[1][c8 * 8 + e], ak[e], &s_bad);
    }
    __syncthreads();
    if (threadIdx.x < hd) {
        od_red_add(det, dwq + threadIdx.x, od_lds_unfix(sdw[0][threadIdx.x], s_bad));
        od_red_add(det, dwk + threadIdx.x, od_lds_unfix(sdw[1][threadIdx.x], s_bad));
    }
}

template <class T, int LPH, int NIT>
__global__ __launch_bounds__(256) void qk_norm_rope_pos_kernel(const T* __restrict__ qkv, int ldqkv, const float* __restrict__ wq,
                                                               const float* __restrict__ wk, const float* __restrict__ table,
                                                               T* __restrict__ out, int ldo, int B, int L, float eps, float q_scale,
                                                               int bpw, int lpw) {
    constexpr int HD = 8 * LPH, HALFL = LPH / 2;
    const int lane = threadIdx.x & 63, c8 = lane % LPH;
    const int wpl = (B + bpw - 1) / bpw;
    const long gw = (long)blockIdx.x * 4 + (threadIdx.x >> 6);
    const int l0 = (int)(gw / wpl) * lpw, b0 = (int)(gw % wpl) * bpw;
    if (l0 >= L) return;
    const int l1 = l0 + lpw < L ? l0 + lpw : L, b1 = b0 + bpw < B ? b0 + bpw : B;
    float w[2][8];
    od_ld8(wq + c8 * 8, w[0]); od_ld8(wk + c8 * 8, w[1]);
#pragma unroll
    for (int e = 0; e < 8; e++) w[0][e] *= q_scale;
    const bool first = c8 < HALFL;
    for (int l = l0; l < l1; l++) {
        float tb[16];
        const float* tp = table + ((size_t)l * (HD / 2) + (c8 % HALFL) * 8) * 2;
        od_ld8(tp, *(float(*)[8])&tb[0]); od_ld8(tp + 8, *(float(*)[8])&tb[8]);
        float cs[8], sn[8];
#pragma unroll
        for (int e = 0; e < 8; e++) { cs[e] = tb[2 * e]; sn[e] = first ? -tb[2 * e + 1] : tb[2 * e + 1]; }
        for (int b = b0; b < b1; b++) {
            const long m = (long)b * L + l;
            float v[NIT][8];
#pragma unroll
            for (int it = 0; it < NIT; it++) od_ld8(qkv + m * ldqkv + (size_t)(it * 64 + lane) * 8, v[it]);
#pragma unroll
            for (int it = 0; it < NIT; it++) {
                float ss = 0.f;
#pragma unroll
                for (int e = 0; e < 8; e++) ss += v[it][e] * v[it][e];
#pragma unroll
                for (int msk = 1; msk < LPH; msk <<= 1) ss += __shfl_xor(ss, msk);
                const float inv = rsqrtf(ss / (float)HD + eps);
                const float* wv = w[it < NIT / 2 ? 0 : 1];
                float y[8], o[8];
#pragma unroll
                for (int e = 0; e < 8; e++) y[e] = v[it][e] * inv * wv[e];
#pragma unroll
                for (int e = 0; e < 8; e++) o[e] = y[e] * cs[e] + __shfl_xor(y[e], HALFL) * sn[e];
                od_st8(out + m * ldo + (size_t)(it * 64 + lane) * 8, o);
            }
        }
    }
}

template <class T, int LPH, int NIT>
__global__ __launch_bounds__(256) void qk_norm_rope_pos_bwd_kernel(const T* __restrict__ qkv, int ldqkv, const float* __restrict__ wq,
                                                                   const float* __restrict__ wk, const float* __restrict__ table,
                                                                   const T* __restrict__ dqk, int lddqk, T* __restrict__ dqkv, int lddqkv,
                                                                   float* __restrict__ dwq, float* __restrict__ dwk,
                                                                   int B, int L, float eps, float q_scale, int bpw, int lpw,
                                                                   const OdDetTable* __restrict__ det) {
    constexpr int HD = 8 * LPH, HALFL = LPH / 2;
    __shared__ long long s_dw[2][HD];
    __shared__ int s_bad;
    for (int i = threadIdx.x; i < 2 * HD; i += 256) s_dw[i / HD][i % HD] = 0;
    if (threadIdx.x == 0) s_bad = 0;
    __syncthreads();
    const int lane = threadIdx.x & 63, c8 = lane % LPH;
    const int wpl = (B + bpw - 1) / bpw;
    const long gw = (long)blockIdx.x * 4 + (threadIdx.x >> 6);
    const int l0 = (int)(gw / wpl) * lpw, b0 = (int)(gw % wpl) * bpw;
    const int l1 = l0 + lpw < L ? l0 + lpw : L, b1 = b0 + bpw < B ? b0 + bpw : B;
    float w[2][8], acc[2][8];
    od_ld8(wq + c8 * 8, w[0]); od_ld8(wk + c8 * 8, w[1]);
#pragma unroll
    for (int e = 0; e < 8; e++) { acc[0][e] = 0.f; acc[1][e] = 0.f; }
    const bool first = c8 < HALFL;
    for (int l = l0; l < l1; l++) {
        float tb[16];
        const float* tp = table + ((size_t)l * (HD / 2) + (c8 % HALFL) * 8) * 2;
        od_ld8(tp, *(float(*)[8])&tb[0]); od_ld8(tp + 8, *(float(*)[8])&tb[8]);
        float cs[8], sn[8];
#pragma unroll
        for (int e = 0; e < 8; e++) { cs[e] = tb[2 * e]; sn[e] = first ? tb[2 * e + 1] : -tb[2 * e + 1]; }
        for (int b = b0; b < b1; b++) {
            const long m = (long)b * L + l;
            float v[NIT][8], d[NIT][8];
#pragma unroll
            for (int it = 0; it < NIT; it++) {
                od_ld8(qkv + m * ldqkv + (size_t)(it * 64 + lane) * 8, v[it]);
                od_ld8(dqk + m * lddqk + (size_t)(it * 64 + lane) * 8, d[it]);
            }
#pragma unroll
            for (int it = 0; it < NIT; it++) {
                const int qk = it < NIT / 2 ? 0 : 1;
                const float gs = qk == 0 ? q_scale : 1.f;
                float ss = 0.f;
#pragma unroll
                for (int e = 0; e < 8; e++) ss += v[it][e] * v[it][e];
#pragma unroll
                for (int msk = 1; msk < LPH; msk <<= 1) ss += __shfl_xor(ss, msk);
                const float inv = rsqrtf(ss / (float)HD + eps);
                float dy[8], xh[8], dot = 0.f;
#pragma unroll
                for (int e = 0; e < 8; e++) d[it][e] *= gs;
#pragma unroll
                for (int e = 0; e < 8; e++) {
                    const float u = d[it][e] * cs[e] + __shfl_xor(d[it][e], HALFL) * sn[e];
                    xh[e] = v[it][e] * inv;
                    acc[qk][e] += u * xh[e];
                    dy[e] = u * w[qk][e];
                    dot += dy[e] * xh[e];
                }
#pragma unroll
                for (int msk = 1; msk < LPH; msk <<= 1) dot += __shfl_xor(dot, msk);
                dot /= (float)HD;
                float o[8];
#pragma unroll
                for (int e = 0; e < 8; e++) o[e] = inv * (dy[e] - xh[e] * dot);
                od_st8(dqkv + m * lddqkv + (size_t)(it * 64 + lane) * 8, o);
            }
        }
    }
#pragma unroll
    for (int msk = LPH; msk < 64; msk <<= 1)
#pragma unroll
        for (int e = 0; e < 8; e++) { acc[0][e] += __shfl_xor(acc[0][e], msk); acc[1][e] += __shfl_xor(acc[1][e], msk); }
    if (lane < LPH) {
#pragma unroll
        for (int e = 0; e < 8; e++) { od_lds_fix_add(&s_dw[0][c8 * 8 + e], acc[0][e], &s_bad); od_lds_fix_add(&s_dw[1][c8 * 8 + e], acc[1][e], &s_bad); }
    }
    __syncthreads();
    if (threadIdx.x < HD) {
        od_red_add(det, dwq + threadIdx.x, od_lds_unfix(s_dw[0][threadIdx.x], s_bad));
        od_red_add(det, dwk + threadIdx.x, od_lds_unfix(s_dw[1][threadIdx.x], s_bad));
    }
}

__global__ void rope_table_kernel(float* __restrict__ table, int L, int hd) {
    const long i = (long)blockIdx.x * blockDim.x + threadIdx.x;
    const int half = hd / 2;
    if (i >= (long)L * half) return;
    const int l = (int)(i / half), j = (int)(i % half);
    const float e = (float)(2 * j) / (float)(-hd);
    const float inv_freq = (float)pow(10000.0, (double)e);
    const float ang = (float)l * inv_freq;
    table[2 * i] = cosf(ang);
    table[2 * i + 1] = sinf(ang);
}

inline int nch_for(int C) { return (C + 511) / 512; }

inline void qk_pos_split(int B, int L, int& bpw, int& lpw) {
    bpw = B < OD_QK_BPW ? B : OD_QK_BPW;
    lpw = OD_QK_BPW / bpw;
    if (lpw < 1) lpw = 1;
    (void)L;
}

}

#define DISPATCH_T_NCH(DT, NCHV, CALL)                                          \
    do {                                                                        \
        if ((DT) == OD_BF16) {                                                  \
            typedef bf16_t T_;                                                  \
            if ((NCHV) == 1) { constexpr int N_ = 1; CALL; }                    \
            else if ((NCHV) == 2) { constexpr int N_ = 2; CALL; }               \
            else if ((NCHV) == 3) { constexpr int N_ = 3; CALL; }               \
            else return OD_ERR_UNSUPPORTED;                                     \
        } else if ((DT) == OD_F32) {                                            \
            typedef float T_;                                                   \
            if ((NCHV) == 1) { constexpr int N_ = 1; CALL; }                    \
            else if ((NCHV) == 2) { constexpr int N_ = 2; CALL; }               \
            else if ((NCHV) == 3) { constexpr int N_ = 3; CALL; }               \
            else return OD_ERR_UNSUPPORTED;                                     \
        } else return OD_ERR_ARG;                                               \
    } while (0)

extern "C" int od_rmsnorm_film(int dtype, const void* x, int ldx, const float* ssg, const void* cl, int ldcl, int cl_bcast,
                               void* h, int ldh, float* inv_rms, int B, int L, int C, float eps, void* stream) {
    if (C % 8 || ldx % 8 || ldh % 8 || (cl && ldcl % 8)) return OD_ERR_ALIGN;
    const long M = (long)B * L;
    dim3 grid((unsigned)((M + 3) / 4));
    DISPATCH_T_NCH(dtype, nch_for(C),
        OD_LAUNCH((rmsnorm_film_kernel<T_, N_>), grid, dim3(256), 0, (hipStream_t)stream, (const T_*)x, ldx, ssg, (const T_*)cl, ldcl,
                  cl_bcast, (T_*)h, ldh, inv_rms, B, L, C, eps));
    OD_CHECK_LAUNCH();
    return 0;
}

extern "C" int od_rmsnorm_film_bwd(int dtype, const void* x, int ldx, const float* inv_rms, const float* ssg, const void* dh,
                                   int lddh, void* dres, int lddres, float* dssg, int B, int L, int C, void* stream) {
    if (C % 8 || ldx % 8 || lddh % 8 || lddres % 8) return OD_ERR_ALIGN;
    dim3 grid((L + 4 * ROWS_PER_WAVE_BWD - 1) / (4 * ROWS_PER_WAVE_BWD), B);
    DISPATCH_T_NCH(dtype, nch_for(C),
        OD_LAUNCH((rmsnorm_film_bwd_kernel<T_, N_>), grid, dim3(256), 0, (hipStream_t)stream, (const T_*)x, ldx, inv_rms, ssg,
                  (const T_*)dh, lddh, (T_*)dres, lddres, dssg, B, L, C, od_det_active()));
    OD_CHECK_LAUNCH();
    return 0;
}

extern "C" int od_rmsnorm_gate_residual(int dtype, const void* x, int ldx, const void* h, int ldh, const float* ssg, void* xo,
                                        int ldxo, float* inv_rms, int B, int L, int C, float eps, void* stream) {
    if (C % 8 || ldx % 8 || ldh % 8 || ldxo % 8) return OD_ERR_ALIGN;
    const long M = (long)B * L;
    dim3 grid((unsigned)((M + 3) / 4));
    DISPATCH_T_NCH(dtype, nch_for(C),
        OD_LAUNCH((rmsnorm_gate_res_kernel<T_, N_>), grid, dim3(256), 0, (hipStream_t)stream, (const T_*)x, ldx, (const T_*)h, ldh, ssg,
                  (T_*)xo, ldxo, inv_rms, B, L, C, eps));
    OD_CHECK_LAUNCH();
    return 0;
}

extern "C" int od_rmsnorm_gate_residual_film(int dtype, const void* x, int ldx, const void* h, int ldh, const float* ssg_a, void* xo,
                                             int ldxo, float* inv_a, const float* ssg_b, const void* cl, int ldcl, int cl_bcast,
                                             void* h2, int ldh2, float* inv_b, int B, int L, int C, float eps, void* stream) {
    if (C % 8 || ldx % 8 || ldh % 8 || ldxo % 8 || ldh2 % 8 || (cl && ldcl % 8)) return OD_ERR_ALIGN;
    const long M = (long)B * L;
    dim3 grid((unsigned)((M + 3) / 4));
    DISPATCH_T_NCH(dtype, nch_for(C),
        OD_LAUNCH((rmsnorm_gate_res_film_kernel<T_, N_>), grid, dim3(256), 0, (hipStream_t)stream, (const T_*)x, ldx, (const T_*)h, ldh,
                  ssg_a, (T_*)xo, ldxo, inv_a, ssg_b, (const T_*)cl, ldcl, cl_bcast, (T_*)h2, ldh2, inv_b, B, L, C, eps));
    OD_CHECK_LAUNCH();
    return 0;
}

extern "C" int od_rmsnorm_gate_residual_film_dwconv(int dtype, const void* x, int ldx, const void* h, int ldh, const float* ssg_a, void* xo,
                                                    int ldxo, float* inv_a, const float* ssg_b, void* h2, int ldh2, float* inv_b,
                                                    const float* conv_w, const float* conv_b, void* y, int ldy, int B, int L, int C,
                                                    int ksize, float eps, void* stream) {
    if (C % 8 || ldx % 8 || ldh % 8 || ldxo % 8 || (h2 && ldh2 % 8) || ldy % 8) return OD_ERR_ALIGN;
    if (C > 512 || (ksize != 3 && ksize != 5 && ksize != 7 && ksize != 9)) return OD_ERR_UNSUPPORTED;
    if (!x || !h || !xo || !y || !conv_w || !conv_b || xo == x || xo == h) return OD_ERR_ARG;
#ifndef OD_FD_SMALL_RUNS
#define OD_FD_SMALL_RUNS 2048
#endif
    const bool small = (long)B * ((L + 31) / 32) < OD_FD_SMALL_RUNS;
    const int run = small ? 8 : 32;
    dim3 grid((unsigned)((L + 4 * run - 1) / (4 * run)), (unsigned)B);
#define FD_GO2(T_, KS_, RUN_) OD_LAUNCH((rmsnorm_gate_res_film_dwconv_kernel<T_, KS_, RUN_>), grid, dim3(256), 0, (hipStream_t)stream, (const T_*)x, ldx, \
                   (const T_*)h, ldh, ssg_a, (T_*)xo, ldxo, inv_a, ssg_b, (T_*)h2, ldh2, inv_b, conv_w, conv_b, (T_*)y, ldy, B, L, C, eps)
#define FD_GO1(T_, KS_) do { if (small) FD_GO2(T_, KS_, 8); else FD_GO2(T_, KS_, 32); } while (0)
#define FD_GO(KS_) do { if (dtype == OD_BF16) FD_GO1(bf16_t, KS_); else if (dtype == OD_F32) FD_GO1(float, KS_); else return OD_ERR_UNSUPPORTED; } while (0)
    if (ksize == 5) FD_GO(5); else if (ksize == 3) FD_GO(3); else if (ksize == 7) FD_GO(7); else FD_GO(9);
#undef FD_GO
#undef FD_GO1
#undef FD_GO2
    OD_CHECK_LAUNCH();
    return 0;
}

extern "C" int od_rmsnorm_gate_residual_bwd(int dtype, const void* h, int ldh, const float* inv_rms, const float* ssg,
                                            const void* dy, int lddy, void* dh, int lddh, float* dssg, int B, int L, int C,
                                            void* stream) {
    if (C % 8 || ldh % 8 || lddy % 8 || lddh % 8) return OD_ERR_ALIGN;
    dim3 grid((L + 4 * ROWS_PER_WAVE_BWD - 1) / (4 * ROWS_PER_WAVE_BWD), B);
    DISPATCH_T_NCH(dtype, nch_for(C),
        OD_LAUNCH((rmsnorm_gate_res_bwd_kernel<T_, N_>), grid, dim3(256), 0, (hipStream_t)stream, (const T_*)h, ldh, inv_rms, ssg,
                  (const T_*)dy, lddy, (T_*)dh, lddh, dssg, B, L, C, od_det_active()));
    OD_CHECK_LAUNCH();
    return 0;
}

extern "C" int od_swiglu_rmsnorm(int dtype, const void* vg, int ldvg, void* hh, int ldhh, float* inv_rms, int M, int Hf, int Hp,
                                 float eps, void* stream) {
    if (Hp % 8 || ldvg % 8 || ldhh % 8 || Hf > Hp) return OD_ERR_ALIGN;
    dim3 grid((unsigned)((M + 3) / 4));
    DISPATCH_T_NCH(dtype, nch_for(Hp),
        OD_LAUNCH((swiglu_rmsnorm_kernel<T_, N_>), grid, dim3(256), 0, (hipStream_t)stream, (const T_*)vg, ldvg, (T_*)hh, ldhh, inv_rms,
                  (long)M, Hf, Hp, eps));
    OD_CHECK_LAUNCH();
    return 0;
}

extern "C" int od_swiglu_rmsnorm_bwd(int dtype, const void* vg, int ldvg, const float* inv_rms, const void* dhh, int lddhh,
                                     void* dvg, int lddvg, int M, int Hf, int Hp, void* stream) {
    if (Hp % 8 || ldvg % 8 || lddhh % 8 || lddvg % 8 || Hf > Hp) return OD_ERR_ALIGN;
    dim3 grid((unsigned)((M + 3) / 4));
    DISPATCH_T_NCH(dtype, nch_for(Hp),
        OD_LAUNCH((swiglu_rmsnorm_bwd_kernel<T_, N_>), grid, dim3(256), 0, (hipStream_t)stream, (const T_*)vg, ldvg, inv_rms,
                  (const T_*)dhh, lddhh, (T_*)dvg, lddvg, (long)M, Hf, Hp));
    OD_CHECK_LAUNCH();
    return 0;
}

extern "C" int od_final_norm_proj_out(int dtype, const void* x, int ldx, const float* W, const float* bias, float* v,
                                      float* inv_rms, int B, int L, int C, int E, float eps, void* stream) {
    if (C % 8 || ldx % 8) return OD_ERR_ALIGN;
    if (E > 8 || C > 1024) return OD_ERR_UNSUPPORTED;
    const long M = (long)B * L;
    dim3 grid((unsigned)((M + 3) / 4));
    DISPATCH_T_NCH(dtype, nch_for(C),
        OD_LAUNCH((final_proj_kernel<T_, N_>), grid, dim3(256), 0, (hipStream_t)stream, (const T_*)x, ldx, W, bias, v, inv_rms, B, L, C, E, eps));
    OD_CHECK_LAUNCH();
    return 0;
}

extern "C" int od_final_norm_proj_out_bwd(int dtype, const void* x, int ldx, const float* inv_rms, const float* W,
                                          const float* dv, void* dx, int lddx, float* dW, float* db, int B, int L, int C, int E,
                                          void* stream) {
    if (C % 8 || ldx % 8 || lddx % 8) return OD_ERR_ALIGN;
    if (E > 8 || C > 512) return OD_ERR_UNSUPPORTED;
    dim3 grid((L + 4 * ROWS_PER_WAVE_BWD - 1) / (4 * ROWS_PER_WAVE_BWD), B);
    if (dtype == OD_BF16)
        OD_LAUNCH((final_proj_bwd_kernel<bf16_t, 1>), grid, dim3(256), 0, (hipStream_t)stream, (const bf16_t*)x, ldx, inv_rms, W, dv,
                  (bf16_t*)dx, lddx, dW, db, B, L, C, E, od_det_active());
    else
        OD_LAUNCH((final_proj_bwd_kernel<float, 1>), grid, dim3(256), 0, (hipStream_t)stream, (const float*)x, ldx, inv_rms, W, dv,
                  (float*)dx, lddx, dW, db, B, L, C, E, od_det_active());
    OD_CHECK_LAUNCH();
    return 0;
}

extern "C" int od_rope_table(float* table, int L, int hd, void* stream) {
    if (hd % 2 || L <= 0) return OD_ERR_ARG;
    const long n = (long)L * (hd / 2);
    OD_LAUNCH(rope_table_kernel, dim3((unsigned)((n + 255) / 256)), dim3(256), 0, (hipStream_t)stream, table, L, hd);
    OD_CHECK_LAUNCH();
    return 0;
}

extern "C" int od_qk_norm_rope(int dtype, const void* qkv, int ldqkv, const float* wq, const float* wk, const float* table,
                               void* qk_out, int ldo, int B, int L, int H, int hd, float eps, float q_scale, void* stream) {
    if (hd % 16 || hd > 256 || 64 % (hd / 8)) return OD_ERR_UNSUPPORTED;
    if (ldqkv % 8 || ldo % 8) return OD_ERR_ALIGN;
    const long M = (long)B * L;
    const int lph = hd / 8;
    if (dtype != OD_F16 && (lph == 4 || lph == 8) && (H * lph) % 64 == 0 && ldqkv >= 2 * H * hd) {
        const int nit = 2 * H * lph / 64;
        if (nit == 2 || nit == 4 || nit == 8) {
            int bpw, lpw; qk_pos_split(B, L, bpw, lpw);
            const long waves = (long)((L + lpw - 1) / lpw) * ((B + bpw - 1) / bpw);
            dim3 g2((unsigned)((waves + 3) / 4));
#define QKP(TT, LPHV, NITV) OD_LAUNCH((qk_norm_rope_pos_kernel<TT, LPHV, NITV>), g2, dim3(256), 0, (hipStream_t)stream, (const TT*)qkv, ldqkv, wq, wk, table, (TT*)qk_out, ldo, B, L, eps, q_scale, bpw, lpw)
#define QKP_T(TT) do { if (lph == 8) { if (nit == 2) QKP(TT, 8, 2); else if (nit == 4) QKP(TT, 8, 4); else QKP(TT, 8, 8); } \
                       else { if (nit == 2) QKP(TT, 4, 2); else if (nit == 4) QKP(TT, 4, 4); else QKP(TT, 4, 8); } } while (0)
            if (dtype == OD_BF16) QKP_T(bf16_t); else QKP_T(float);
#undef QKP_T
#undef QKP
            OD_CHECK_LAUNCH();
            return 0;
        }
    }
    dim3 grid((unsigned)((M + 3) / 4));
    if (dtype == OD_F16)
        OD_LAUNCH((qk_norm_rope_kernel<bf16_t, f16_t>), grid, dim3(256), 0, (hipStream_t)stream, (const bf16_t*)qkv, ldqkv, wq, wk, table,
                  (f16_t*)qk_out, ldo, B, L, H, hd, eps, q_scale);
    else if (dtype == OD_BF16)
        OD_LAUNCH((qk_norm_rope_kernel<bf16_t>), grid, dim3(256), 0, (hipStream_t)stream, (const bf16_t*)qkv, ldqkv, wq, wk, table,
                  (bf16_t*)qk_out, ldo, B, L, H, hd, eps, q_scale);
    else
        OD_LAUNCH((qk_norm_rope_kernel<float>), grid, dim3(256), 0, (hipStream_t)stream, (const float*)qkv, ldqkv, wq, wk, table,
                  (float*)qk_out, ldo, B, L, H, hd, eps, q_scale);
    OD_CHECK_LAUNCH();
    return 0;
}

extern "C" int od_qk_norm_rope_bwd(int dtype, const void* qkv, int ldqkv, const float* wq, const float* wk, const float* table,
                                   const void* dqk, int lddqk, void* dqkv, int lddqkv, float* dwq, float* dwk, int B, int L,
                                   int H, int hd, float eps, float q_scale, void* stream) {
    if (hd % 16 || hd > 256 || 64 % (hd / 8)) return OD_ERR_UNSUPPORTED;
    if (ldqkv % 8 || lddqk % 8 || lddqkv % 8) return OD_ERR_ALIGN;
    const long M = (long)B * L;
    const int lph = hd / 8;
    if ((lph == 4 || lph == 8) && (H * lph) % 64 == 0) {
        const int nit = 2 * H * lph / 64;
        if (nit == 2 || nit == 4 || nit == 8) {
            int bpw, lpw; qk_pos_split(B, L, bpw, lpw);
            lpw *= 4;
            const long waves = (long)((L + lpw - 1) / lpw) * ((B + bpw - 1) / bpw);
            dim3 g2((unsigned)((waves + 3) / 4));
#define QKPB(TT, LPHV, NITV) OD_LAUNCH((qk_norm_rope_pos_bwd_kernel<TT, LPHV, NITV>), g2, dim3(256), 0, (hipStream_t)stream, (const TT*)qkv, ldqkv, wq, wk, table, (const TT*)dqk, lddqk, (TT*)dqkv, lddqkv, dwq, dwk, B, L, eps, q_scale, bpw, lpw, od_det_active())
#define QKPB_T(TT) do { if (lph == 8) { if (nit == 2) QKPB(TT, 8, 2); else if (nit == 4) QKPB(TT, 8, 4); else QKPB(TT, 8, 8); } \
                        else { if (nit == 2) QKPB(TT, 4, 2); else if (nit == 4) QKPB(TT, 4, 4); else QKPB(TT, 4, 8); } } while (0)
            if (dtype == OD_BF16) QKPB_T(bf16_t); else QKPB_T(float);
#undef QKPB_T
#undef QKPB
            OD_CHECK_LAUNCH();
            return 0;
        }
    }
    dim3 grid((unsigned)((M + 4 * ROWS_PER_WAVE_BWD - 1) / (4 * ROWS_PER_WAVE_BWD)));
    if (dtype == OD_BF16)
        OD_LAUNCH((qk_norm_rope_bwd_kernel<bf16_t>), grid, dim3(256), 0, (hipStream_t)stream, (const bf16_t*)qkv, ldqkv, wq, wk, table,
                  (const bf16_t*)dqk, lddqk, (bf16_t*)dqkv, lddqkv, dwq, dwk, B, L, H, hd, eps, q_scale, od_det_active());
    else
        OD_LAUNCH((qk_norm_rope_bwd_kernel<float>), grid, dim3(256), 0, (hipStream_t)stream, (const float*)qkv, ldqkv, wq, wk, table,
                  (const float*)dqk, lddqk, (float*)dqkv, lddqkv, dwq, dwk, B, L, H, hd, eps, q_scale, od_det_active());
    OD_CHECK_LAUNCH();
    return 0;
}
```

osu_dreamer_amd/engine.py:

```python
from __future__ import annotations


import math
import os
from collections import OrderedDict
from typing import Dict, List, Optional

import torch

from . import det, ops
from ._lib import OD_ACT_NONE, OD_ACT_SILU

OD_FUSE_FILM_DWCONV_DEFAULT = "0"

FP32_EPS = float(torch.finfo(torch.float32).eps)

PLAN_CACHE_DEFAULT = 16
PLAN_CACHE_DETERMINISTIC = 2


def _ceil(x: int, m: int) -> int:
    return (x + m - 1) // m * m


# ... 17 lines not shown
        return t


class DenoiserEngine:
    def __init__(self, model):
        self.model = model
        a = model.args
        ba = a.backbone_args
        self.E, self.A, self.S = model.emb_dim, model.a_dim, model.style_dim
        self.Cg, self.D, self.U = a.global_cond_dim, a.backbone_dim, a.u_head_dim
        self.H, self.hd, self.depth = ba.n_heads, ba.head_dim, ba.depth
        self.dh = self.H * self.hd
        self.q_scale = math.log2(math.e) / math.sqrt(self.hd)
        self.radius = ba.radius
        self.ksize = 1 + 2 * ba.radius
        self.Hf = int(self.D * ba.expand * 2 / 3)
        self.Hp = _ceil(self.Hf, 64)
        if ba.radius not in (0, 1, 2, 3, 4):
            raise NotImplementedError("depthwise kernel sizes 3, 5, 7, 9 (radius 1-4) are compiled; radius 0 is the identity")
        if not (0.0 <= ba.dropout < 1.0):
            raise ValueError(f"dropout probability has to be in [0, 1), got {ba.dropout}")
        self.dropout = float(ba.dropout)
        self._packed: Dict[str, torch.Tensor] = {}
        self._packed_key = None
        self._plan_key = None
        self.ws: Optional[Workspace] = None
        self._plans: "OrderedDict[tuple, Workspace]" = OrderedDict()
        self.plan_switches = 0
        self.plan_builds = 0
        self._rowmap = None
        self.generation = 0
        self._attn_aux = None
        self._attn_ws_cache: Dict[tuple, "ops.FusedAttnBwdWorkspace"] = {}
        self._attn_ws = None
        self.varlen = False
        self.attn_f16 = False

    def _det_flush(self, *tensors):
        ctx = det.context(self.model.arena.data.device)
        if ctx is not None:
            for t in tensors:
                ctx.flush(t)

    def _det_flush_segment(self, name: str):
        ctx = det.context(self.model.arena.data.device)
        if ctx is not None:
            s, e = self.model.arena.segments(self.depth)[name]
            ctx.flush(self.model.arena.ensure_grad()[s:e])

    def P(self, name: str) -> torch.Tensor:
        return self.model.arena.view(name)

    def G(self, name: str) -> torch.Tensor:
        return self.model.arena.grad_view(name)

    def _gemm_weights(self) -> List[str]:
        names = ["proj_audio.0"]
        for i in range(self.depth):
            p = f"net.layers.{i}."
            names += [p + "proj_cl", p + "attn.qkv_proj", p + "attn.out_proj", p + "ffn.proj_vg.1", p + "ffn.proj_o"]
        return names

    def pack_weights(self, dtype: torch.dtype, train: bool, x3: bool = False):
        dev = self.model.arena.data.device
        x3 = bool(x3 and dtype == torch.float32 and not train)
        key = (dtype, train, dev, x3)
        if self._packed_key != key:
            self._packed = {}
            self._packed_key = key
            self.generation += 1
            Hf, Hp = self.Hf, self.Hp
            rm = [-1] * (2 * Hp)
            for j in range(Hf):
                rm[j] = j
                rm[Hp + j] = Hf + j
            self._rowmap = torch.tensor(rm, dtype=torch.int32, device=dev)
        pk = self._packed
        for n in self._gemm_weights():
            w = self.P(n + ".weight")
            N, K = w.shape[0], w.shape[1]
            Np, Kp, rmap = N, K, None
            if n.endswith("ffn.proj_vg.1"):
                Np, rmap = 2 * self.Hp, self._rowmap
            if n.endswith("ffn.proj_o"):
                Kp = self.Hp
            if n not in pk:
                pk[n] = torch.empty(Np, Kp, dtype=dtype, device=dev)
                if x3 and Kp % 32 == 0:
                    pk[n] = ops.SplitWeight(pk[n])
                if train:
                    pk[n + ".T"] = torch.empty(Kp, Np, dtype=dtype, device=dev)
                if rmap is not None:
                    pk[n + ".b"] = torch.empty(Np, dtype=torch.float32, device=dev)
            ops.pack_weight(w, pk[n], row_map=rmap)
            if train:
                ops.pack_weight(w, pk[n + ".T"], transpose=True, row_map=rmap)
            if rmap is not None:
                ops.pack_weight(self.P(n + ".bias"), pk[n + ".b"].view(Np, 1), row_map=rmap)

    def W(self, name: str, T: bool = False) -> torch.Tensor:
        return self._packed[name + (".T" if T else "")]

    def plain_gemm(self, A: torch.Tensor, W: torch.Tensor, bias, C: torch.Tensor):
        ops.gemm_nt(A, W, bias, C, x3=self.x3)

    def plan(self, B: int, L: int, Ba: int, dtype: torch.dtype, train: bool, x3: bool = False, lens=None, offs=None):
        dev = self.model.arena.data.device
        assert not (x3 and train), "the f32x3 product exists for the forward kernels only"
        varlen = lens is not None
        x3 = bool(x3 and dtype == torch.float32)
        ngroups = len(offs) - 1 if offs is not None else 0
        key = (B, L, Ba, dtype, train, dev, x3, getattr(self.model, "attn_dtype", None), varlen, ngroups)
        if key != self._plan_key:
            self.plan_switches += 1
            self.ws = self._plans.get(key) if train else None
            if self.ws is None:
                self.plan_builds += 1
                self.ws = Workspace(dev)
                tab = self.ws.get("rope", (L, self.hd // 2, 2), torch.float32)
                ops.rope_table(tab, L, self.hd)
            if train:
                limit = max(1, int(os.environ.get("OD_PLAN_CACHE", PLAN_CACHE_DEFAULT)))
                if det.enabled():
                    limit = min(limit, PLAN_CACHE_DETERMINISTIC)
                self._plans[key] = self.ws
                self._plans.move_to_end(key)
                while len(self._plans) > limit:
                    self._plans.popitem(last=False)
            self._plan_key = key
            self.generation += 1
        self.varlen = varlen
        if varlen:
            lens_t = torch.as_tensor(lens).to("cpu", torch.int32)
            if lens_t.shape != (B,) or int(lens_t.min()) < 1 or int(lens_t.max()) > L:
                raise ValueError(f"lens must hold B = {B} lengths in [1, {L}]")
            self.ws.get("vl.lens", (B,), torch.int32).copy_(lens_t)
            if offs is not None:
                offs_t = torch.as_tensor(offs).to("cpu", torch.int32)
                if int(offs_t[0]) != 0 or int(offs_t[-1]) != B or bool((offs_t[1:] <= offs_t[:-1]).any()):
                    raise ValueError("offs must rise strictly from 0 to B")
                self.ws.get("vl.offs", (ngroups + 1,), torch.int32).copy_(offs_t)
        self.B, self.L, self.Ba, self.dtype, self.train, self.x3 = B, L, Ba, dtype, train, x3
        self.M, self.Ma = B * L, Ba * L
        self.attn_f16 = getattr(self.model, "attn_dtype", None) == torch.float16
        if self.attn_f16 and (dtype != torch.bfloat16 or self.hd != 64):
            if not getattr(self, "_warned_f16_fallback", False):
                import warnings
                warnings.warn(f"attn_dtype = float16 applies to compute_dtype bfloat16 with head_dim 64; this plan (dtype {dtype}, head_dim "
                              f"{self.hd}) runs its attention in {dtype}")
                self._warned_f16_fallback = True
            self.attn_f16 = False
        if varlen and train and self.attn_f16:
            raise NotImplementedError("ragged training has no half-operand attention (attn_dtype = float16 runs the fused backward, which has no "
                                      "varlen form): train ragged batches with attn_dtype = None")
        return self.ws

    def buf(self, name, shape, dtype=None):
        return self.ws.get(name, shape, self.dtype if dtype is None else dtype)

    def lbuf(self, name, i, shape, dtype=None):
        return self.buf(f"{name}.{i}" if self.train else name, shape, dtype)

    def conditioning(self, audio: torch.Tensor, style: torch.Tensor):
        B, Ba, L = self.B, self.Ba, self.L
        D, A, Cg, U = self.D, self.A, self.Cg, self.U
        f32 = torch.float32
        a_t = self.buf("a_t", (self.Ma, A))
        a_pre = self.buf("a_pre", (self.Ma, A))
        a = self.buf("a", (self.Ma, A))
        ops.cl_to_frames(audio, a_t)
        ops.gemm_nt(a_t, self.W("proj_audio.0"), self.P("proj_audio.0.bias"), a_pre, x3=self.x3)
        ops.silu(a_pre, a)
        cg, cg_pre = self.buf("cg", (B, Cg), f32), self.buf("cg_pre", (B, Cg), f32)
        ops.linear_small(style, self.P("proj_style.0.weight"), self.P("proj_style.0.bias"), cg, cg_pre, OD_ACT_SILU)
        for i in range(self.depth):
            p = f"net.layers.{i}."
            for s in ("ssg1", "ssg2"):
                ops.linear_small(cg, self.P(p + s + ".weight"), self.P(p + s + ".bias"),
                                 self.buf(f"{s}.{i}", (B, 3 * D), f32))
            if not self.train:
                ops.gemm_nt(a, self.W(p + "proj_cl"), self.P(p + "proj_cl.bias"), self.buf(f"cl.{i}", (self.Ma, D)), x3=self.x3)
        ops.linear_small(cg, self.P("u_mod.weight"), self.P("u_mod.bias"), self.buf("umod", (B, 2 * U), f32))

    def pred(self, xt: torch.Tensor, u: torch.Tensor, v: torch.Tensor):
        B, L, M, D, dh, Hp = self.B, self.L, self.M, self.D, self.dh, self.Hp
        f32 = torch.float32
        tab = self.ws.t["rope"]
        bcast = self.Ba == 1 and B > 1
        x = self.lbuf("x_in", 0, (M, D))
        ops.proj_in(xt, self.P("proj_in.weight"), self.P("proj_in.bias"), x)

        def cl_of(i):
            if not self.train:
                return self.ws.t[f"cl.{i}"]
            cl = self.buf("cl", (self.Ma, D))
            ops.gemm_nt(self.ws.t["a"], self.W(f"net.layers.{i}.proj_cl"), self.P(f"net.layers.{i}.proj_cl.bias"), cl)
            return cl

        h1 = self.lbuf("h1", 0, (M, D))
        ops.rmsnorm_film(x, self.ws.t["ssg1.0"], cl_of(0), bcast, h1, self.lbuf("inv1", 0, (M,), f32), B, L)
        for i in range(self.depth):
            p = f"net.layers.{i}."
            ssg1, ssg2 = self.ws.t[f"ssg1.{i}"], self.ws.t[f"ssg2.{i}"]
            qkv = self.lbuf("qkv", i, (M, 3 * dh))
            if self.train or self.attn_f16 or self.hd not in (32, 64) or (2 * dh) % 128:
                qk = self.lbuf("qk16" if self.attn_f16 else "qk", i, (M, 2 * dh), torch.float16 if self.attn_f16 else None)
                ops.gemm_nt_qkrope_split(h1, self.W(p + "attn.qkv_proj"), self.P(p + "attn.qkv_proj.bias"), qkv, qk,
                                         self.P(p + "attn.q_norm.weight"), self.P(p + "attn.k_norm.weight"), tab, L, self.H,
                                         self.hd, FP32_EPS, x3=self.x3, q_scale=self.q_scale)
            else:
                ops.gemm_nt_qkrope(h1, self.W(p + "attn.qkv_proj"), self.P(p + "attn.qkv_proj.bias"), qkv,
                                   self.P(p + "attn.q_norm.weight"), self.P(p + "attn.k_norm.weight"), tab, L,
                                   self.H, self.hd, FP32_EPS, x3=self.x3, q_scale=self.q_scale)
                qk = qkv
            y = self.lbuf("y", i, (M, dh))
            lse = self.lbuf("lse", i, (B, self.H, L), f32)
            if self.varlen:
                ops.flash_attn_fwd_varlen(qk[:, :dh], qk[:, dh:], self._v_of(qkv), y, lse, self.ws.t["vl.lens"], B, self.H, L, self.hd,
                                          1.0 / math.sqrt(self.hd), x3=self.x3, q_prescaled=True)
            else:
                ops.flash_attn_fwd(qk[:, :dh], qk[:, dh:], self._v_of(qkv), y, lse, B, self.H, L, self.hd,
                                   1.0 / math.sqrt(self.hd), x3=self.x3, q_prescaled=True)
            ao = self.lbuf("ao", i, (M, D))
            self.plain_gemm(y, self.W(p + "attn.out_proj"), self.P(p + "attn.out_proj.bias"), ao)
            x_mid = self.lbuf("x_mid", i, (M, D))
            h2 = self.lbuf("h2", i, (M, D))
            fuse_dw = (self.radius > 0 and not self.varlen and D <= 512 and x.data_ptr() != x_mid.data_ptr() and x.dtype in (torch.bfloat16, torch.float32)
                       and os.environ.get("OD_FUSE_FILM_DWCONV", OD_FUSE_FILM_DWCONV_DEFAULT) == "1")
            if fuse_dw:
                hdw = self.lbuf("hdw", i, (M, D))
                ops.rmsnorm_gate_residual_film_dwconv(x, ao, ssg1, x_mid, self.lbuf("inv2", i, (M,), f32), ssg2, h2 if self.train else None,
                                                      self.lbuf("inv3", i, (M,), f32),
                                                      self.P(p + "ffn.proj_vg.0.weight"), self.P(p + "ffn.proj_vg.0.bias"), hdw, B, L, self.ksize)
            else:
                ops.rmsnorm_gate_residual_film(x, ao, ssg1, x_mid, self.lbuf("inv2", i, (M,), f32), ssg2, None, False, h2,
                                               self.lbuf("inv3", i, (M,), f32), B, L)
            if fuse_dw:
                pass
            elif self.radius > 0:
                hdw = self.lbuf("hdw", i, (M, D))
                if self.varlen:
                    ops.dwconv_varlen(h2, self.P(p + "ffn.proj_vg.0.weight"), self.P(p + "ffn.proj_vg.0.bias"), hdw, self.ws.t["vl.lens"], B, L,
                                      self.ksize)
                else:
                    ops.dwconv(h2, self.P(p + "ffn.proj_vg.0.weight"), self.P(p + "ffn.proj_vg.0.bias"), hdw, B, L, self.ksize)
            else:
                hdw = h2
            vg = self.lbuf("vg", i, (M, 2 * Hp))
            ops.gemm_nt(hdw, self.W(p + "ffn.proj_vg.1"), self._packed[p + "ffn.proj_vg.1.b"], vg, x3=self.x3)
            hh = self.lbuf("hh", i, (M, Hp))
            ops.swiglu_rmsnorm(vg, hh, self.lbuf("inv4", i, (M,), f32), self.Hf, Hp)
            if self._drop_active():
                ops.scale_channels(hh, self.draw_dropout_mask(i), B, L)
            fo = self.lbuf("fo", i, (M, D))
            self.plain_gemm(hh, self.W(p + "ffn.proj_o"), self.P(p + "ffn.proj_o.bias"), fo)
            x = self.buf(f"x_in.{i + 1}", (M, D)) if self.train else self.buf(f"x_in.{(i + 1) & 1}", (M, D))
            if i + 1 < self.depth:
                h1 = self.lbuf("h1", i + 1, (M, D))
                ops.rmsnorm_gate_residual_film(x_mid, fo, ssg2, x, self.lbuf("inv5", i, (M,), f32),
                                               self.ws.t[f"ssg1.{i + 1}"], cl_of(i + 1), bcast, h1,
                                               self.lbuf("inv1", i + 1, (M,), f32), B, L)
            else:
                ops.rmsnorm_gate_residual(x_mid, fo, ssg2, x, self.lbuf("inv5", i, (M,), f32), B, L)
        self._x_last = x
        ops.final_norm_proj_out(x, self.P("proj_out.weight"), self.P("proj_out.bias"), v,
                                self.buf("invf", (M,), f32), B, L)
        fsum = self.buf("fsum", (B, self.U), f32)
        fsum.zero_()
        if self.varlen:
            ops.uhead_fwd_varlen(xt, self._uhead_w(), fsum, self.ws.t["vl.lens"], self.U)
            self._det_flush(fsum)
            ops.uhead_tail_varlen(fsum, self.ws.t["umod"], self.P("u_out.weight"), self.P("u_out.bias"), u, self.ws.t["vl.lens"], L,
                                  self.model.u_scale)
        else:
            ops.uhead_fwd(xt, self._uhead_w(), fsum, self.U)
            self._det_flush(fsum)
            ops.uhead_tail(fsum, self.ws.t["umod"], self.P("u_out.weight"), self.P("u_out.bias"), u, L, self.model.u_scale)

    def _v_of(self, qkv: torch.Tensor) -> torch.Tensor:
        v = qkv[:, 2 * self.dh:]
        return v.view(torch.float16) if self.attn_f16 else v

    def attn_bwd_passes(self) -> int:
        from . import _lib
        return int(_lib.lib().cdll.od_flash_attn_bwd_fused_passes() if self.fused_attn_bwd() else _lib.lib().cdll.od_flash_attn_bwd_passes())

    def fused_attn_bwd(self) -> bool:
        import os
        if self.dtype != torch.bfloat16 or self.hd != 64 or self.varlen:
            return False
        if self.attn_f16:
            return True
        env = os.environ.get("OD_ATTN_BWD_FUSED", "")
        if env in ("0", "1"):
            return env == "1"
        return self.L >= 2048

    def attn_bwd_launch(self, i: int, dy: torch.Tensor, delta: torch.Tensor, dqkv: torch.Tensor, core_only: bool = False):
        t, dh, p = self.ws.t, self.dh, f"net.layers.{i}."
        qk, qkv, y, lse = t[f"qk16.{i}" if self.attn_f16 else f"qk.{i}"], t[f"qkv.{i}"], t[f"y.{i}"], t[f"lse.{i}"]
        wq, wk = self.P(p + "attn.q_norm.weight"), self.P(p + "attn.k_norm.weight")
        gq, gk = self.G(p + "attn.q_norm.weight"), self.G(p + "attn.k_norm.weight")
        scale = 1.0 / math.sqrt(self.hd)
        dqk = self.buf("d.qk", (self.M, 2 * dh))
        if self.fused_attn_bwd():
            key = (self.B, self.H, self.L, qk.device, qk.dtype)
            ws = self._attn_ws_cache.get(key)
            if ws is None:
                if len(self._attn_ws_cache) >= 4:
                    self._attn_ws_cache.pop(next(iter(self._attn_ws_cache)))
                ws = self._attn_ws_cache[key] = ops.FusedAttnBwdWorkspace(self.B, self.H, self.L, qk.device, qk.dtype)
                ws.checked = False
            self._attn_ws = ws
            ops.flash_attn_bwd_fused(qk[:, :dh], qk[:, dh:], self._v_of(qkv), y, dy, lse, dqk[:, :dh], dqk[:, dh:], dqkv[:, 2 * dh:],
                                     self.B, self.H, self.L, self.hd, scale, self._attn_ws, q_prescaled=True)
        else:
            if (self._attn_aux is None or self._attn_aux.device != qk.device) and qk.is_cuda:
                if self._attn_aux is not None:
                    self._attn_aux.close()
                with torch.cuda.device(qk.device):
                    self._attn_aux = ops.AttnAux()
                self._attn_aux.device = qk.device
            if self.varlen:
                ops.flash_attn_bwd_varlen(qk[:, :dh], qk[:, dh:], qkv[:, 2 * dh:], y, dy, lse, delta, dqk[:, :dh], dqk[:, dh:],
                                          dqkv[:, 2 * dh:], self.ws.t["vl.lens"], self.B, self.H, self.L, self.hd, scale, q_prescaled=True,
                                          aux=self._attn_aux)
            else:
                ops.flash_attn_bwd(qk[:, :dh], qk[:, dh:], qkv[:, 2 * dh:], y, dy, lse, delta, dqk[:, :dh], dqk[:, dh:],
                                   dqkv[:, 2 * dh:], self.B, self.H, self.L, self.hd, scale, q_prescaled=True, aux=self._attn_aux)
        if not core_only:
            ops.qk_norm_rope_bwd(qkv, wq, wk, t["rope"], dqk, dqkv, gq, gk, self.B, self.L, self.H, self.hd, FP32_EPS, q_scale=self.q_scale)

    def _drop_active(self) -> bool:
        return self.dropout > 0.0 and self.model.training

    def _drop_mask(self, i: int) -> torch.Tensor:
        return self.ws.t[f"drop.{i}"]

    def draw_dropout_mask(self, i: int) -> torch.Tensor:
        keep = 1.0 - self.dropout
        m = self.buf(f"drop.{i}", (self.B, self.Hp), torch.float32)
        m.zero_()
        m[:, :self.Hf] = torch.empty(self.B, self.Hf, device=m.device, dtype=torch.float32).bernoulli_(keep) / keep
        return m

    def _uhead_w(self, grads=False):
        f = self.G if grads else self.P
        return [f(f"u_head.{j}.{s}") for j in (0, 1, 3, 4) for s in ("weight", "bias")]

    def backward(self, xt: torch.Tensor, style: torch.Tensor, du: torch.Tensor, dv: torch.Tensor, reducer=None):
        assert self.train
        B, L, M, D, dh, Hf, Hp, A = self.B, self.L, self.M, self.D, self.dh, self.Hf, self.Hp, self.A
        f32 = torch.float32
        dctx = det.context(self.model.arena.data.device)
        if dctx is not None:
            dctx.register(self.model.arena.ensure_grad())
        tab = self.ws.t["rope"]
        cg, a = self.ws.t["cg"], self.ws.t["a"]
        dx = self.buf("d.x", (M, D))
        dbr = self.buf("d.branch", (M, D))
        dtmp = self.buf("d.tmp", (M, D))
        dhh = self.buf("d.hh", (M, Hp))
        dvg = self.buf("d.vg", (M, 2 * Hp))
        dy = self.buf("d.y", (M, dh))
        dqkv = self.buf("d.qkv", (M, 3 * dh))
        da = self.buf("d.a", (self.Ma, A))
        delta = self.buf("d.delta", (B, self.H, L), f32)
        dcg = self.buf("d.cg", (B, self.Cg), f32)
        dssg1, dssg2 = self.buf("d.ssg1", (B, 3 * D), f32), self.buf("d.ssg2", (B, 3 * D), f32)

        ops.final_norm_proj_out_bwd(self._x_last, self.ws.t["invf"], self.P("proj_out.weight"), dv, dx,
                                    self.G("proj_out.weight"), self.G("proj_out.bias"), B, L)
        dfm, dmod = self.buf("d.fm", (B, self.U), f32), self.buf("d.mod", (B, 2 * self.U), f32)
        if self.varlen:
            lens = self.ws.t["vl.lens"]
            ops.uhead_tail_bwd_varlen(self.ws.t["fsum"], self.ws.t["umod"], self.P("u_out.weight"), self.P("u_out.bias"), du,
                                      dfm, dmod, self.G("u_out.weight"), self.G("u_out.bias"), lens, L, self.model.u_scale)
            ops.uhead_bwd_varlen(xt, self._uhead_w(), dfm, self._uhead_w(grads=True), lens, self.U)
        else:
            ops.uhead_tail_bwd(self.ws.t["fsum"], self.ws.t["umod"], self.P("u_out.weight"), self.P("u_out.bias"), du,
                               dfm, dmod, self.G("u_out.weight"), self.G("u_out.bias"), L, self.model.u_scale)
            ops.uhead_bwd(xt, self._uhead_w(), dfm, self._uhead_w(grads=True), self.U)
        ops.linear_small_bwd(cg, self.P("u_mod.weight"), None, dmod, self.buf("d.lin_pre_umod", (B, 2 * self.U), f32),
                             self.G("u_mod.weight"), self.G("u_mod.bias"), dcg, False, OD_ACT_NONE)
        self._det_flush_segment("tail")
        if reducer is not None:
            reducer.segment_done("tail")

        for i in reversed(range(self.depth)):
            p = f"net.layers.{i}."
            t = self.ws.t
            ssg1, ssg2 = t[f"ssg1.{i}"], t[f"ssg2.{i}"]
            dssg1.zero_()
            dssg2.zero_()
            ops.rmsnorm_gate_residual_bwd(t[f"fo.{i}"], t[f"inv5.{i}"], ssg2, dx, dbr, dssg2, B, L)
            ops.gemm_tn(dbr, t[f"hh.{i}"], self.G(p + "ffn.proj_o.weight"), n_cols=D, k_cols=Hf,
                        dbias=self.G(p + "ffn.proj_o.bias"))
            ops.gemm_nt(dbr, self.W(p + "ffn.proj_o", T=True), None, dhh)
            if self._drop_active():
                ops.scale_channels(dhh, self._drop_mask(i), B, L)
            ops.swiglu_rmsnorm_bwd(t[f"vg.{i}"], t[f"inv4.{i}"], dhh, dvg, Hf, Hp)
            gw, gb = self.G(p + "ffn.proj_vg.1.weight"), self.G(p + "ffn.proj_vg.1.bias")
            hdw = t[f"hdw.{i}"] if self.radius > 0 else t[f"h2.{i}"]
            ops.gemm_tn(dvg, hdw, gw, n_cols=2 * Hp, k_cols=D, dbias=gb, n_block=Hp, n_valid=Hf)
            if self.radius > 0:
                self.plain_gemm(dvg, self.W(p + "ffn.proj_vg.1", T=True), None, dtmp)
                if self.varlen:
                    ops.dwconv_bwd_varlen(t[f"h2.{i}"], self.P(p + "ffn.proj_vg.0.weight"), dtmp, dbr, self.G(p + "ffn.proj_vg.0.weight"),
                                          self.G(p + "ffn.proj_vg.0.bias"), self.ws.t["vl.lens"], B, L, self.ksize)
                else:
                    ops.dwconv_bwd(t[f"h2.{i}"], self.P(p + "ffn.proj_vg.0.weight"), dtmp, dbr,
                                   self.G(p + "ffn.proj_vg.0.weight"), self.G(p + "ffn.proj_vg.0.bias"), B, L, self.ksize)
            else:
                self.plain_gemm(dvg, self.W(p + "ffn.proj_vg.1", T=True), None, dbr)
            ops.rmsnorm_film_bwd(t[f"x_mid.{i}"], t[f"inv3.{i}"], ssg2, dbr, dx, dssg2, B, L)
            ops.rmsnorm_gate_residual_bwd(t[f"ao.{i}"], t[f"inv2.{i}"], ssg1, dx, dbr, dssg1, B, L)
            ops.gemm_tn(dbr, t[f"y.{i}"], self.G(p + "attn.out_proj.weight"), dbias=self.G(p + "attn.out_proj.bias"))
            ops.gemm_nt(dbr, self.W(p + "attn.out_proj", T=True), None, dy)
            self.attn_bwd_launch(i, dy, delta, dqkv)
            ops.gemm_tn(dqkv, t[f"h1.{i}"], self.G(p + "attn.qkv_proj.weight"), dbias=self.G(p + "attn.qkv_proj.bias"))
            self.plain_gemm(dqkv, self.W(p + "attn.qkv_proj", T=True), None, dtmp)
            ops.gemm_tn(dtmp, a, self.G(p + "proj_cl.weight"), dbias=self.G(p + "proj_cl.bias"))
            ops.gemm_nt(dtmp, self.W(p + "proj_cl", T=True), None, da, accumulate=(i != self.depth - 1))
            ops.rmsnorm_film_bwd(t[f"x_in.{i}"], t[f"inv1.{i}"], ssg1, dtmp, dx, dssg1, B, L)
            lp = self.buf("d.lin_pre_ssg", (B, 3 * D), f32)
            self._det_flush(dssg1, dssg2)
            ops.linear_small_bwd(cg, self.P(p + "ssg2.weight"), None, dssg2, lp, self.G(p + "ssg2.weight"),
                                 self.G(p + "ssg2.bias"), dcg, True, OD_ACT_NONE)
            ops.linear_small_bwd(cg, self.P(p + "ssg1.weight"), None, dssg1, lp, self.G(p + "ssg1.weight"),
                                 self.G(p + "ssg1.bias"), dcg, True, OD_ACT_NONE)
            self._det_flush_segment(f"layer{i}")
            if reducer is not None:
                reducer.segment_done(f"layer{i}")

        ops.proj_in_bwd(xt, dx, self.G("proj_in.weight"), self.G("proj_in.bias"))
        da_pre = self.buf("d.a_pre", (self.Ma, A))
        ops.silu_bwd(self.ws.t["a_pre"], da, da_pre)
        ops.gemm_tn(da_pre, self.ws.t["a_t"], self.G("proj_audio.0.weight"), dbias=self.G("proj_audio.0.bias"))
        self._det_flush(dcg)
        ops.linear_small_bwd(style, self.P("proj_style.0.weight"), self.ws.t["cg_pre"], dcg,
                             self.buf("d.lin_pre_style", (B, self.Cg), f32), self.G("proj_style.0.weight"),
                             self.G("proj_style.0.bias"), None, False, OD_ACT_SILU)
        self._det_flush_segment("head")
        if reducer is not None:
            reducer.segment_done("head")
        if self.fused_attn_bwd() and self._attn_ws is not None and not self._attn_ws.checked:
            self._attn_ws.checked = True
            self.check_attn_status()

    def attn_status_ptr(self) -> int:
        return self._attn_ws.err_ptr() if self._attn_ws is not None else 0

    def attn_status_view(self) -> torch.Tensor:
        return self._attn_ws.err_view()

    ATTN_STATUS = {1: "a launch left jobs unprocessed (an XCD ran none of its workgroups): gradients incomplete",
                   2: "a launch with another (B, H, L) than the workspace's earlier launches was refused",
                   3: "a chain wait ran out of time (the predecessor's write never came; OD_FB_CHAIN_TIMEOUT_MS): dq is NaN"}

    def check_attn_status(self):
        if self._attn_ws is None:
            return
        code = 0
        for ws in {id(w): w for w in [self._attn_ws, *self._attn_ws_cache.values()]}.values():
            code = code or ws.status()
        if code != 0:
            raise RuntimeError(f"od_flash_attn_bwd_fused status {code}: {self.ATTN_STATUS.get(code, '?')}; the optimizer steps since then "
                               "were skipped.  OD_ATTN_BWD_FUSED=0 selects the two-kernel backward.")
```

osu_dreamer_amd/ops.py:

```python
from __future__ import annotations

import os
from typing import Optional

import torch

from . import _lib
from ._lib import OD_ACT_NONE, OD_ACT_SILU, OD_BF16, OD_EPI_NONE, OD_EPI_SILU, OD_F32, OD_F32X3, OD_F32X3W


def dt_code(dtype: torch.dtype) -> int:
    if dtype == torch.float32:
        return OD_F32
    if dtype == torch.bfloat16:
        return OD_BF16
    if dtype == torch.float16:
        return _lib.OD_F16
    raise TypeError(f"unsupported compute dtype {dtype}")


class SplitWeight:

    def __init__(self, storage: torch.Tensor):
        self.t = storage


def mm_code(dtype: torch.dtype, x3: bool, w=None) -> int:
    if isinstance(w, SplitWeight):
        if not (x3 and dtype == torch.float32):
            raise ValueError("a pre-split weight can only feed the fp32-as-3-x-bf16 product")
        return OD_F32X3W
    return OD_F32X3 if (x3 and dtype == torch.float32) else dt_code(dtype)


def _w(W):
    return W.t if isinstance(W, SplitWeight) else W


def _stream(t: torch.Tensor) -> int:
    return torch.cuda.current_stream(t.device).cuda_stream if t.is_cuda else 0


def _p(t: Optional[torch.Tensor]) -> Optional[int]:
    return None if t is None else t.data_ptr()


def _ld(t: torch.Tensor) -> int:
    assert t.dim() == 2 and t.stride(1) == 1, "need a row-major 2-D view"
    return t.stride(0)


def _f32(*ts):
    for t in ts:
        assert t is None or (t.dtype == torch.float32 and t.is_contiguous()), "expected contiguous fp32"


def _i32(*ts):
    for t in ts:
        assert t.dtype == torch.int32 and t.is_contiguous(), "expected contiguous int32"


def gemm_nt(A, W, bias, C, epilogue=OD_EPI_NONE, accumulate=False, x3=False):
    code, W = mm_code(A.dtype, x3, W), _w(W)
    M, K = A.shape
    N = W.shape[0]
    assert W.shape[1] == K and tuple(C.shape) == (M, N)
    assert A.dtype == W.dtype == C.dtype
    _f32(bias)
    _lib.lib().od_gemm_nt(code, _p(A), _ld(A), _p(W), _ld(W), _p(bias), _p(C), _ld(C), M, N, K,
                          epilogue, int(accumulate), _stream(A))


def gemm_nt_qkrope(A, W, bias, C, wq, wk, table, L, H, hd, eps, x3=False, q_scale=1.0):
    code, W = mm_code(A.dtype, x3, W), _w(W)
    M, K = A.shape
    N = W.shape[0]
    assert W.shape[1] == K and tuple(C.shape) == (M, N) and A.dtype == W.dtype == C.dtype
    _f32(bias, wq, wk, table)
    _lib.lib().od_gemm_nt_qkrope(code, _p(A), _ld(A), _p(W), _ld(W), _p(bias), _p(C), _ld(C), M, N, K,
                                 _p(wq), _p(wk), _p(table), L, H, hd, eps, q_scale, _stream(A))


def gemm_nt_qkrope_split(A, W, bias, C, qk_out, wq, wk, table, L, H, hd, eps, x3=False, q_scale=1.0):
    code, W = mm_code(A.dtype, x3, W), _w(W)
    M, K = A.shape
    N = W.shape[0]
    assert W.shape[1] == K and tuple(C.shape) == (M, N) and tuple(qk_out.shape) == (M, 2 * H * hd)
    assert A.dtype == W.dtype == C.dtype
    assert qk_out.dtype == A.dtype or (qk_out.dtype == torch.float16 and A.dtype == torch.bfloat16)
    _f32(bias, wq, wk, table)
    qk_code = _lib.OD_F16 if qk_out.dtype == torch.float16 else (OD_F32 if A.dtype == torch.float32 else code)
    _lib.lib().od_gemm_nt_qkrope_split(code, _p(A), _ld(A), _p(W), _ld(W), _p(bias), _p(C), _ld(C), _p(qk_out),
                                       _ld(qk_out), qk_code, M, N, K, _p(wq), _p(wk), _p(table), L, H, hd, eps, q_scale, _stream(A))


def gemm_tn(G, A, dW, n_cols=None, k_cols=None, dbias=None, n_block=0, n_valid=0):
    M = G.shape[0]
    N = n_cols if n_cols is not None else G.shape[1]
    K = k_cols if k_cols is not None else A.shape[1]
    rows = N if not n_block else (N // n_block) * n_valid
    assert not n_block or N % n_block == 0
    assert dW.dtype == torch.float32 and dW.is_contiguous() and dW.numel() == rows * K
    _f32(dbias)
    _lib.lib().od_gemm_tn_blocks(dt_code(G.dtype), _p(G), _ld(G), _p(A), _ld(A), _p(dW), K, _p(dbias), M, N, K, n_block, n_valid, _stream(G))


def colsum(G, out, n_cols=None):
    M = G.shape[0]
    N = n_cols if n_cols is not None else G.shape[1]
    _f32(out)
    _lib.lib().od_colsum(dt_code(G.dtype), _p(G), _ld(G), _p(out), M, N, _stream(G))


def pack_weight(src, dst, transpose=False, row_map=None):
    N = src.shape[0]
    K = src.numel() // N
    _f32(src)
    code = OD_F32X3W if isinstance(dst, SplitWeight) else dt_code(_w(dst).dtype)
    dst = _w(dst)
    if transpose:
        Kp, Np = dst.shape
    else:
        Np, Kp = dst.shape
    assert dst.is_contiguous()
    _lib.lib().od_pack_weight(code, _p(src), N, K, _p(dst), Np, Kp, int(transpose), _p(row_map), _stream(src))


def linear_small(x, W, b, out, pre=None, act=OD_ACT_NONE):
    B, K = x.shape
    N = W.shape[0]
    _f32(x, W, b, out, pre)
    _lib.lib().od_linear_small(_p(x), _p(W), _p(b), _p(out), _p(pre), B, N, K, act, _stream(x))


def linear_small_bwd(x, W, pre, dout, dpre, dW, db, dx, accumulate_dx, act=OD_ACT_NONE):
    B, K = x.shape
    N = W.shape[0]
    _f32(x, W, pre, dout, dpre, dW, db, dx)
    _lib.lib().od_linear_small_bwd(_p(x), _p(W), _p(pre), _p(dout), _p(dpre), _p(dW), _p(db), _p(dx),
                                   int(accumulate_dx), B, N, K, act, _stream(x))


def cl_to_frames(src, dst):
    B, C, L = src.shape
    _f32(src)
    _lib.lib().od_cl_to_frames(dt_code(dst.dtype), _p(src), _p(dst), _ld(dst), B, C, L, _stream(src))


def _feed_rows(base, cstride, lens, N):
    assert lens.dtype == torch.int32 and lens.dim() == 1 and lens.shape[0] == N and lens.is_contiguous(), "lens must be a contiguous int32 [B]"
    for t in (base, cstride):
        assert t.dtype == torch.int64 and t.dim() == 1 and t.shape[0] == N and t.is_contiguous(), "base / cstride must be contiguous int64 [N]"


def feed_gather(store, base, cstride, lens, out):
    N, C, Lpad = out.shape
    _f32(store, out)
    _feed_rows(base, cstride, lens, N)
    assert store.device == out.device == base.device == cstride.device == lens.device, "feed_gather: every tensor on one device"
    _lib.lib().od_feed_gather(_p(store), store.numel(), _p(base), _p(cstride), _p(lens), _p(out), N, C, Lpad, _stream(out))


def feed_gather_quant(store, elem_size, base, cstride, lens, out, c0=0, channels=None, scale=None, offset=None, flip=None):
    N, Ctot, Lpad = out.shape
    C = Ctot - c0 if channels is None else channels
    _f32(out)
    _feed_rows(base, cstride, lens, N)
    assert store.dtype == torch.uint8 and store.dim() == 1 and store.is_contiguous(), "the store is a flat uint8 tensor (its bytes)"
    assert (scale is None) == (offset is None), "scale and offset come together"
    for t in (scale, offset):
        assert t is None or (t.dtype == torch.float64 and tuple(t.shape) == (N, C) and t.is_contiguous()), "scale / offset must be contiguous fp64 (N, channels)"
    if flip is not None:
        _lens(flip, N)
    assert all(t is None or t.device == out.device for t in (store, base, cstride, lens, scale, offset, flip)), "feed_gather_quant: every tensor on one device"
    _lib.lib().od_feed_gather_quant(_p(store), store.numel(), elem_size, _p(base), _p(cstride), _p(lens), _p(scale), _p(offset), _p(flip), _p(out),
                                    N, C, c0, Ctot, Lpad, _stream(out))


def replicate_tail(x, lens, plens):
    N, C, Lpad = x.shape
    _f32(x)
    _lens(lens, N)
    _lens(plens, N)
    assert x.device == lens.device == plens.device, "replicate_tail: every tensor on one device"
    _lib.lib().od_replicate_tail(_p(x), _p(lens), _p(plens), N, C, Lpad, _stream(x))


def proj_in(xt, W, bias, x):
    B, E, L = xt.shape
    D = x.shape[1]
    _f32(xt, W, bias)
    _lib.lib().od_proj_in(dt_code(x.dtype), _p(xt), _p(W), _p(bias), _p(x), _ld(x), B, E, L, D, _stream(xt))


def proj_in_bwd(xt, dx, dW, db):
    B, E, L = xt.shape
    D = dx.shape[1]
    _f32(xt, dW, db)
    _lib.lib().od_proj_in_bwd(dt_code(dx.dtype), _p(xt), _p(dx), _ld(dx), _p(dW), _p(db), B, E, L, D, _stream(xt))


def silu(x, y):
    assert x.is_contiguous() and y.is_contiguous()
    _lib.lib().od_silu(dt_code(x.dtype), _p(x), _p(y), x.numel(), _stream(x))


def silu_bwd(x, dy, dx):
    assert x.is_contiguous() and dy.is_contiguous() and dx.is_contiguous()
    _lib.lib().od_silu_bwd(dt_code(x.dtype), _p(x), _p(dy), _p(dx), x.numel(), _stream(x))


def rmsnorm_film(x, ssg, cl, cl_bcast, h, inv_rms, B, L, eps=1e-6):
    C = x.shape[1]
    _f32(ssg, inv_rms)
    _lib.lib().od_rmsnorm_film(dt_code(x.dtype), _p(x), _ld(x), _p(ssg), _p(cl), _ld(cl) if cl is not None else 0,
                               int(cl_bcast), _p(h), _ld(h), _p(inv_rms), B, L, C, eps, _stream(x))


def rmsnorm_film_bwd(x, inv_rms, ssg, dh, dres, dssg, B, L):
    C = x.shape[1]
    _f32(ssg, inv_rms, dssg)
    _lib.lib().od_rmsnorm_film_bwd(dt_code(x.dtype), _p(x), _ld(x), _p(inv_rms), _p(ssg), _p(dh), _ld(dh), _p(dres),
                                   _ld(dres), _p(dssg), B, L, C, _stream(x))


def rmsnorm_gate_residual(x, h, ssg, xo, inv_rms, B, L, eps=1e-6):
    C = x.shape[1]
    _f32(ssg, inv_rms)
    _lib.lib().od_rmsnorm_gate_residual(dt_code(x.dtype), _p(x), _ld(x), _p(h), _ld(h), _p(ssg), _p(xo), _ld(xo),
                                        _p(inv_rms), B, L, C, eps, _stream(x))


def rmsnorm_gate_residual_film(x, h, ssg_a, xo, inv_a, ssg_b, cl, cl_bcast, h2, inv_b, B, L, eps=1e-6):
    _f32(ssg_a, ssg_b, inv_a, inv_b)
    _lib.lib().od_rmsnorm_gate_residual_film(dt_code(x.dtype), _p(x), _ld(x), _p(h), _ld(h), _p(ssg_a), _p(xo), _ld(xo),
                                             _p(inv_a), _p(ssg_b), _p(cl), _ld(cl) if cl is not None else 0, int(cl_bcast),
                                             _p(h2), _ld(h2), _p(inv_b), B, L, x.shape[1], eps, _stream(x))


def rmsnorm_gate_residual_film_dwconv(x, h, ssg_a, xo, inv_a, ssg_b, h2, inv_b, conv_w, conv_b, y, B, L, ksize, eps=1e-6):
    _f32(ssg_a, ssg_b, inv_a, inv_b, conv_w, conv_b)
    assert xo.data_ptr() != x.data_ptr() and xo.data_ptr() != h.data_ptr()
    _lib.lib().od_rmsnorm_gate_residual_film_dwconv(dt_code(x.dtype), _p(x), _ld(x), _p(h), _ld(h), _p(ssg_a), _p(xo), _ld(xo), _p(inv_a),
                                                    _p(ssg_b), _p(h2), _ld(h2) if h2 is not None else 0, _p(inv_b), _p(conv_w), _p(conv_b),
                                                    _p(y), _ld(y), B, L, x.shape[1], ksize, eps, _stream(x))


def rmsnorm_gate_residual_bwd(h, inv_rms, ssg, dy, dh, dssg, B, L):
    C = h.shape[1]
    _f32(ssg, inv_rms, dssg)
    _lib.lib().od_rmsnorm_gate_residual_bwd(dt_code(h.dtype), _p(h), _ld(h), _p(inv_rms), _p(ssg), _p(dy), _ld(dy),
                                            _p(dh), _ld(dh), _p(dssg), B, L, C, _stream(h))


def rope_table(table, L, hd):
    _f32(table)
    _lib.lib().od_rope_table(_p(table), L, hd, _stream(table))


def qk_norm_rope(qkv, wq, wk, table, qk_out, B, L, H, hd, eps, q_scale=1.0):
    _f32(wq, wk, table)
    _lib.lib().od_qk_norm_rope(dt_code(qkv.dtype), _p(qkv), _ld(qkv), _p(wq), _p(wk), _p(table), _p(qk_out),
                               _ld(qk_out), B, L, H, hd, eps, q_scale, _stream(qkv))


def qk_norm_rope_bwd(qkv, wq, wk, table, dqk, dqkv, dwq, dwk, B, L, H, hd, eps, q_scale=1.0):
    _f32(wq, wk, table, dwq, dwk)
    _lib.lib().od_qk_norm_rope_bwd(dt_code(qkv.dtype), _p(qkv), _ld(qkv), _p(wq), _p(wk), _p(table), _p(dqk), _ld(dqk),
                                   _p(dqkv), _ld(dqkv), _p(dwq), _p(dwk), B, L, H, hd, eps, q_scale, _stream(qkv))


def flash_attn_fwd(q, k, v, o, lse, B, H, L, hd, scale, x3=False, q_prescaled=False):
    _f32(lse)
    assert q.dtype == k.dtype == v.dtype and (o.dtype == q.dtype or (q.dtype == torch.float16 and o.dtype == torch.bfloat16))
    _lib.lib().od_flash_attn_fwd(mm_code(q.dtype, x3), _p(q), _ld(q), _p(k), _ld(k), _p(v), _ld(v), _p(o), _ld(o), _p(lse),
                                 B, H, L, hd, scale, int(q_prescaled), _stream(q))


class AttnAux:

    def __init__(self):
        import ctypes
        self.handle = ctypes.c_void_p()
        _lib.lib().od_attn_aux_create(ctypes.byref(self.handle))

    def close(self):
        if self.handle:
            _lib.lib().od_attn_aux_destroy(self.handle)
            self.handle = None

    def __del__(self):
        try:
            self.close()
        except Exception:
            pass


def flash_attn_fwd_varlen(q, k, v, o, lse, lens, B, H, L, hd, scale, x3=False, q_prescaled=False):
    _f32(lse)
    _i32(lens)
    assert q.dtype == k.dtype == v.dtype and (o.dtype == q.dtype or (q.dtype == torch.float16 and o.dtype == torch.bfloat16))
    _lib.lib().od_flash_attn_fwd_varlen(mm_code(q.dtype, x3), _p(q), _ld(q), _p(k), _ld(k), _p(v), _ld(v), _p(o), _ld(o), _p(lse),
                                        _p(lens), B, H, L, hd, scale, int(q_prescaled), _stream(q))


def flash_attn_bwd(q, k, v, o, do, lse, delta, dq, dk, dv, B, H, L, hd, scale, q_prescaled=False, aux=None):
    _f32(lse, delta)
    _lib.lib().od_flash_attn_bwd_aux(dt_code(q.dtype), _p(q), _ld(q), _p(k), _ld(k), _p(v), _ld(v), _p(o), _ld(o), _p(do),
                                     _ld(do), _p(lse), _p(delta), _p(dq), _ld(dq), _p(dk), _ld(dk), _p(dv), _ld(dv),
                                     B, H, L, hd, scale, int(q_prescaled), aux.handle if aux is not None else None, _stream(q))


def flash_attn_bwd_varlen(q, k, v, o, do, lse, delta, dq, dk, dv, lens, B, H, L, hd, scale, q_prescaled=False, aux=None):
    _f32(lse, delta)
    _i32(lens)
    _lib.lib().od_flash_attn_bwd_varlen(dt_code(q.dtype), _p(q), _ld(q), _p(k), _ld(k), _p(v), _ld(v), _p(o), _ld(o), _p(do),
                                        _ld(do), _p(lse), _p(delta), _p(dq), _ld(dq), _p(dk), _ld(dk), _p(dv), _ld(dv), _p(lens),
                                        B, H, L, hd, scale, int(q_prescaled), aux.handle if aux is not None else None, _stream(q))


class FusedAttnBwdWorkspace:

    def __init__(self, B, H, L, device, dtype=torch.bfloat16):
        import ctypes
        total, zero = ctypes.c_long(), ctypes.c_long()
        _lib.lib().od_flash_attn_bwd_fused_ws_bytes(dt_code(dtype), B, H, L, ctypes.byref(total), ctypes.byref(zero))
        self.shape = (B, H, L)
        self.dtype = dtype
        self.bytes = total.value
        assert zero.value <= self.bytes
        self.zero_bytes = zero.value
        self.buf = torch.empty(self.bytes, dtype=torch.uint8, device=device)
        self.reset()

    def reset(self):
        self.buf[:self.zero_bytes].zero_()

    def err_ptr(self) -> int:
        return self.buf.data_ptr() + int(_lib.lib().cdll.od_flash_attn_bwd_fused_err_offset())

    def err_view(self) -> torch.Tensor:
        off = int(_lib.lib().cdll.od_flash_attn_bwd_fused_err_offset())
        return self.buf[off:off + 4].view(torch.int32)

    def status(self) -> int:
        import ctypes
        err = ctypes.c_int(-1)
        _lib.lib().od_flash_attn_bwd_fused_status(_p(self.buf), ctypes.byref(err), _stream(self.buf))
        return err.value


def flash_attn_bwd_fused(q, k, v, o, do, lse, dq, dk, dv, B, H, L, hd, scale, ws: FusedAttnBwdWorkspace, q_prescaled=False):
    _f32(lse)
    assert ws.shape == (B, H, L), (ws.shape, (B, H, L))
    assert q.dtype == k.dtype == v.dtype and o.dtype == do.dtype == dq.dtype == dk.dtype == dv.dtype == torch.bfloat16
    assert q.dtype == torch.bfloat16 or (q.dtype == torch.float16 and ws.dtype == torch.float16)
    _lib.lib().od_flash_attn_bwd_fused(dt_code(q.dtype), _p(q), _ld(q), _p(k), _ld(k), _p(v), _ld(v), _p(o), _ld(o), _p(do), _ld(do),
                                       _p(lse), _p(dq), _ld(dq), _p(dk), _ld(dk), _p(dv), _ld(dv), B, H, L, hd, scale, int(q_prescaled),
                                       _p(ws.buf), ws.bytes, _stream(q))


def dwconv(x, w, bias, y, B, L, ksize):
    C = x.shape[1]
    _f32(w, bias)
    _lib.lib().od_dwconv(dt_code(x.dtype), _p(x), _ld(x), _p(w), _p(bias), _p(y), _ld(y), B, L, C, ksize, _stream(x))


def dwconv_varlen(x, w, bias, y, lens, B, L, ksize):
    C = x.shape[1]
    _f32(w, bias)
    _i32(lens)
    _lib.lib().od_dwconv_varlen(dt_code(x.dtype), _p(x), _ld(x), _p(w), _p(bias), _p(y), _ld(y), _p(lens), B, L, C, ksize, _stream(x))


def dwconv_bwd(x, w, dy, dx, dw, db, B, L, ksize):
    C = x.shape[1]
    _f32(w, dw, db)
    _lib.lib().od_dwconv_bwd(dt_code(x.dtype), _p(x), _ld(x), _p(w), _p(dy), _ld(dy), _p(dx), _ld(dx), _p(dw), _p(db),
                             B, L, C, ksize, _stream(x))


def dwconv_bwd_varlen(x, w, dy, dx, dw, db, lens, B, L, ksize):
    C = x.shape[1]
    _f32(w, dw, db)
    _i32(lens)
    _lib.lib().od_dwconv_bwd_varlen(dt_code(x.dtype), _p(x), _ld(x), _p(w), _p(dy), _ld(dy), _p(dx), _ld(dx), _p(dw), _p(db),
                                    _p(lens), B, L, C, ksize, _stream(x))


def scale_channels(x, scale, B, L):
    _f32(scale)
    assert scale.shape == (B, x.shape[1]) and scale.is_contiguous()
    _lib.lib().od_scale_channels(dt_code(x.dtype), _p(x), _ld(x), _p(scale), B, L, x.shape[1], _stream(x))


def swiglu_rmsnorm(vg, hh, inv_rms, Hf, Hp, eps=1e-6):
    _f32(inv_rms)
    _lib.lib().od_swiglu_rmsnorm(dt_code(vg.dtype), _p(vg), _ld(vg), _p(hh), _ld(hh), _p(inv_rms), vg.shape[0], Hf, Hp,
                                 eps, _stream(vg))


def swiglu_rmsnorm_bwd(vg, inv_rms, dhh, dvg, Hf, Hp):
    _f32(inv_rms)
    _lib.lib().od_swiglu_rmsnorm_bwd(dt_code(vg.dtype), _p(vg), _ld(vg), _p(inv_rms), _p(dhh), _ld(dhh), _p(dvg),
                                     _ld(dvg), vg.shape[0], Hf, Hp, _stream(vg))


def final_norm_proj_out(x, W, bias, v, inv_rms, B, L, eps=1e-6):
    C = x.shape[1]
    E = W.shape[0]
    _f32(W, bias, v, inv_rms)
    _lib.lib().od_final_norm_proj_out(dt_code(x.dtype), _p(x), _ld(x), _p(W), _p(bias), _p(v), _p(inv_rms), B, L, C, E,
                                      eps, _stream(x))


def final_norm_proj_out_bwd(x, inv_rms, W, dv, dx, dW, db, B, L):
    C = x.shape[1]
    E = W.shape[0]
    _f32(W, dv, inv_rms, dW, db)
    _lib.lib().od_final_norm_proj_out_bwd(dt_code(x.dtype), _p(x), _ld(x), _p(inv_rms), _p(W), _p(dv), _p(dx), _ld(dx),
                                          _p(dW), _p(db), B, L, C, E, _stream(x))


def uhead_fwd(xt, w, fsum, U):
    B, E, L = xt.shape
    _f32(xt, fsum, *w)
    _lib.lib().od_uhead_fwd(_p(xt), *[_p(t) for t in w], _p(fsum), B, E, L, U, _stream(xt))


def uhead_fwd_varlen(xt, w, fsum, lens, U):
    B, E, L = xt.shape
    _f32(xt, fsum, *w)
    _i32(lens)
    _lib.lib().od_uhead_fwd_varlen(_p(xt), *[_p(t) for t in w], _p(fsum), _p(lens), B, E, L, U, _stream(xt))


def uhead_bwd(xt, w, dfm, g, U):
    B, E, L = xt.shape
    _f32(xt, dfm, *w, *g)
    _lib.lib().od_uhead_bwd(_p(xt), *[_p(t) for t in w], _p(dfm), *[_p(t) for t in g], B, E, L, U, _stream(xt))


def uhead_bwd_varlen(xt, w, dfm, g, lens, U):
    B, E, L = xt.shape
    _f32(xt, dfm, *w, *g)
    _i32(lens)
    _lib.lib().od_uhead_bwd_varlen(_p(xt), *[_p(t) for t in w], _p(dfm), *[_p(t) for t in g], _p(lens), B, E, L, U, _stream(xt))


def uhead_tail(fsum, mod, w_out, b_out, u, L, u_scale):
    B, U = fsum.shape
    _f32(fsum, mod, w_out, b_out, u)
    _lib.lib().od_uhead_tail(_p(fsum), _p(mod), _p(w_out), _p(b_out), _p(u), B, U, L, u_scale, _stream(fsum))


def uhead_tail_varlen(fsum, mod, w_out, b_out, u, lens, L, u_scale):
    B, U = fsum.shape
    _f32(fsum, mod, w_out, b_out, u)
    _i32(lens)
    _lib.lib().od_uhead_tail_varlen(_p(fsum), _p(mod), _p(w_out), _p(b_out), _p(u), _p(lens), B, U, L, u_scale, _stream(fsum))


def uhead_tail_bwd(fsum, mod, w_out, b_out, du, dfm, dmod, dw_out, db_out, L, u_scale):
    B, U = fsum.shape
    _f32(fsum, mod, w_out, b_out, du, dfm, dmod, dw_out, db_out)
    _lib.lib().od_uhead_tail_bwd(_p(fsum), _p(mod), _p(w_out), _p(b_out), _p(du), _p(dfm), _p(dmod), _p(dw_out),
                                 _p(db_out), B, U, L, u_scale, _stream(fsum))


def uhead_tail_bwd_varlen(fsum, mod, w_out, b_out, du, dfm, dmod, dw_out, db_out, lens, L, u_scale):
    B, U = fsum.shape
    _f32(fsum, mod, w_out, b_out, du, dfm, dmod, dw_out, db_out)
    _i32(lens)
    _lib.lib().od_uhead_tail_bwd_varlen(_p(fsum), _p(mod), _p(w_out), _p(b_out), _p(du), _p(dfm), _p(dmod), _p(dw_out),
                                        _p(db_out), _p(lens), B, U, L, u_scale, _stream(fsum))


def make_xt(x0, x1, t, xt, dsq):
    B, E, L = x0.shape
    _f32(x0, x1, t, xt, dsq)
    _lib.lib().od_make_xt(_p(x0), _p(x1), _p(t), _p(xt), _p(dsq), B, E, L, _stream(x0))


def make_xt_varlen(x0, x1, t, xt, dsq, lens):
    B, E, L = x0.shape
    _f32(x0, x1, t, xt, dsq)
    _i32(lens)
    _lib.lib().od_make_xt_varlen(_p(x0), _p(x1), _p(t), _p(xt), _p(dsq), _p(lens), B, E, L, _stream(x0))


def loss_grad(xt, x1, u, v, dsq, dv, sums, c0, osl_w, del_w):
    B, E, L = xt.shape
    _f32(xt, x1, u, v, dsq, dv, sums)
    _lib.lib().od_loss_grad(_p(xt), _p(x1), _p(u), _p(v), _p(dsq), _p(dv), _p(sums), B, E, L, c0, osl_w, del_w, _stream(xt))


def loss_grad_varlen(xt, x1, u, v, dsq, dv, sums, lens, c0, osl_w, del_w):
    B, E, L = xt.shape
    _f32(xt, x1, u, v, dsq, dv, sums)
    _i32(lens)
    _lib.lib().od_loss_grad_varlen(_p(xt), _p(x1), _p(u), _p(v), _p(dsq), _p(dv), _p(sums), _p(lens), B, E, L, c0, osl_w, del_w,
                                   _stream(xt))


def loss_finalize(sums, dsq, u, out, du, c0, osl_w, del_w):
    B = u.shape[0]
    _f32(sums, dsq, u, out, du)
    _lib.lib().od_loss_finalize(_p(sums), _p(dsq), _p(u), _p(out), _p(du), B, c0, osl_w, del_w, _stream(u))


def sampler_step(x, u, v, eta):
    B, E, L = x.shape
    _f32(x, u, v, eta)
    _lib.lib().od_sampler_step(_p(x), _p(u), _p(v), _p(eta), B, E, L, _stream(x))


def sampler_eta(u, eta, c0, num_steps):
    _f32(u, eta)
    _lib.lib().od_sampler_eta(_p(u), _p(eta), u.shape[0], c0, num_steps, _stream(u))


def sampler_eta_groups(u, offs, eta, c0, num_steps):
    _f32(u, eta)
    _i32(offs)
    G = offs.shape[0] - 1
    assert eta.numel() >= 2 * G
    _lib.lib().od_sampler_eta_groups(_p(u), _p(offs), _p(eta), G, c0, num_steps, _stream(u))


def sampler_step_varlen(x, u, v, eta, lens, offs):
    B, E, L = x.shape
    _f32(x, u, v, eta)
    _i32(lens, offs)
    _lib.lib().od_sampler_step_varlen(_p(x), _p(u), _p(v), _p(eta), _p(lens), _p(offs), offs.shape[0] - 1, B, E, L, _stream(x))


def sqnorm(g, out, status_ptr: int = 0):
    _f32(g, out)
    _lib.lib().od_sqnorm(_p(g), g.numel(), _p(out), status_ptr or None, _stream(g))


def adamw_ema(p, g, m, v, ema, lr, beta1, beta2, eps, weight_decay, step, ema_decay, ema_mode, gnorm_sq, max_norm, status_ptr: int = 0):
    _f32(p, g, m, v, ema, gnorm_sq)
    _lib.lib().od_adamw_ema(_p(p), _p(g), _p(m), _p(v), _p(ema), p.numel(), lr, beta1, beta2, eps, weight_decay, step,
                            ema_decay, ema_mode, _p(gnorm_sq), max_norm, status_ptr or None, _stream(p))


def ema_update(ema, p, decay, mode):
    _f32(ema, p)
    _lib.lib().od_ema_update(_p(ema), _p(p), p.numel(), decay, mode, _stream(p))


def style_conditioning(labels, rff_w, rff_b, cond_w, cond_b, null_labels, c):
    B, NL = labels.shape
    F, H = cond_w.shape[1], cond_w.shape[2]
    _f32(labels, rff_w, rff_b, cond_w, cond_b, null_labels, c)
    _lib.lib().od_style_conditioning(_p(labels), _p(rff_w), _p(rff_b), _p(cond_w), _p(cond_b), _p(null_labels), _p(c),
                                     B, NL, F, H, _stream(labels))


def rmsnorm_rows(x, gamma, y, eps):
    M, C = x.shape
    _f32(x, gamma, y)
    _lib.lib().od_rmsnorm_rows(_p(x), _p(gamma), _p(y), M, C, eps, _stream(x))


def style_conditioning_bwd(labels, rff_w, rff_b, dc, dcond_w, dcond_b, dnull_labels):
    B, NL = labels.shape
    F, H = dcond_w.shape[1], dcond_w.shape[2]
    _f32(labels, rff_w, rff_b, dc, dcond_w, dcond_b, dnull_labels)
    assert tuple(dc.shape) == (B, H) and rff_w.numel() == F and rff_b.numel() == F
    assert tuple(dcond_w.shape) == (NL, F, H) and tuple(dcond_b.shape) == (NL, H) and tuple(dnull_labels.shape) == (NL, H)
    _lib.lib().od_style_conditioning_bwd(_p(labels), _p(rff_w), _p(rff_b), _p(dc), _p(dcond_w), _p(dcond_b), _p(dnull_labels),
                                         B, NL, F, H, _stream(labels))


def rmsnorm_rows_bwd(x, gamma, dy, dx, dgamma, eps, accumulate_dx=False):
    M, C = x.shape
    _f32(x, gamma, dy, dx, dgamma)
    assert dy.shape == x.shape == dx.shape and (gamma is None or gamma.numel() == C) and (dgamma is None or dgamma.numel() == C)
    _lib.lib().od_rmsnorm_rows_bwd(_p(x), _p(gamma), _p(dy), _p(dx), _p(dgamma), M, C, eps, int(accumulate_dx), _stream(x))


def cast_rows(src, dst):
    assert src.is_contiguous() and dst.is_contiguous() and src.numel() == dst.numel()
    _lib.lib().od_cast_rows(dt_code(src.dtype), _p(src), dt_code(dst.dtype), _p(dst), src.numel(), _stream(src))


def spec_features_conv(audio, w1, b1, g1, w2, b2, g2, out, eps=1e-6):
    B, F, L = audio.shape
    _f32(audio, w1, b1, g1, w2, b2, g2)
    _lib.lib().od_spec_features_conv(dt_code(out.dtype), _p(audio), _p(w1), _p(b1), _p(g1), _p(w2), _p(b2), _p(g2),
                                     _p(out), _ld(out), B, F, L, eps, _stream(audio))


def rmsnorm_affine_film(x, gamma, ssg, y, B, L, act=OD_ACT_NONE, eps=1e-6):
    _f32(gamma, ssg)
    _lib.lib().od_rmsnorm_affine_film(dt_code(x.dtype), _p(x), _ld(x), _p(gamma), _p(ssg), _p(y), _ld(y), B, L, x.shape[1],
                                      eps, act, _stream(x))


def rmsnorm_affine_gate_residual(x, h, gamma, ssg, xo, B, L, eps=1e-6):
    _f32(gamma, ssg)
    _lib.lib().od_rmsnorm_affine_gate_residual(dt_code(x.dtype), _p(x), _ld(x), _p(h), _ld(h), _p(gamma), _p(ssg), _p(xo),
                                               _ld(xo), B, L, x.shape[1], eps, _stream(x))


def unet_mixer(x, p, p_bcast, gx, gamma, xo, B, L, eps=1e-6):
    _f32(gamma)
    _lib.lib().od_unet_mixer(dt_code(x.dtype), _p(x), _ld(x), _p(p), _ld(p), int(p_bcast), _p(gx), _ld(gx), _p(gamma),
                             _p(xo), _ld(xo), B, L, x.shape[1], eps, _stream(x))


def unet_down(x, w, bias, y, B, Lo, stride):
    _f32(w, bias)
    _lib.lib().od_unet_down(dt_code(x.dtype), _p(x), _ld(x), _p(w), _p(bias), _p(y), _ld(y), B, Lo, x.shape[1], stride,
                            _stream(x))


def unet_up(x, w, bias, y, B, Li, stride):
    _f32(w, bias)
    _lib.lib().od_unet_up(dt_code(x.dtype), _p(x), _ld(x), _p(w), _p(bias), _p(y), _ld(y), B, Li, x.shape[1], stride,
                          _stream(x))


def chart_head(x, W, bias, out, B, L, n_sigmoid, rms=False, eps=1e-6):
    _f32(W, bias, out)
    N = W.shape[0]
    _lib.lib().od_chart_head(dt_code(x.dtype), _p(x), _ld(x), _p(W), _p(bias), _p(out), B, L, x.shape[1], N, n_sigmoid,
                             int(rms), eps, _stream(x))


def attn_pool(scores, values, out, B, L, heads, hd):
    _f32(out)
    _lib.lib().od_attn_pool(dt_code(scores.dtype), _p(scores), _ld(scores), _p(values), _ld(values), _p(out), B, L, heads, hd,
                            _stream(scores))


def latent_bwd_ws_floats(kind, B, L, C, n=0):
    if kind == "spec":
        return B * -(-L // 32) * 4880
    f = _lib.lib().cdll.od_latent_bwd_block_frames(C)
    assert f > 0, "C must be a power of two in 8..512"
    per_row, flat = -(-L // f), -(-(B * L) // f)
    if kind == "film":
        return B * per_row * 3 * C
    if kind == "gate":
        return B * per_row * 2 * C
    if kind == "mixer":
        return (per_row if n else B * per_row) * C
    if kind in ("down", "up"):
        return flat * (2 * (n // 2) + 2) * C
    if kind == "head":
        return flat * n * (C + 1)
    raise ValueError(kind)


def rmsnorm_affine_film_bwd(x, gamma, ssg, dy, dx, dgamma, dssg, ws, B, L, act=OD_ACT_NONE, accumulate_dx=False, eps=1e-6):
    _f32(gamma, ssg, dgamma, dssg, ws)
# ... 224 lines not shown
```

Baseline: 3.121.

## Fold K RMSNorm+RoPE backward into fused flash-attention backward epilogue

Key-side waves in the fused attention backward kernel now apply the inverse RoPE and RMSNorm backward to dK while it is still in registers. They write dK straight into dqkv and accumulate dwk through LDS fixed-point reductions. A separate q-only norm/rope backward kernel handles dQ. This removes the dK round trip through the intermediate dqk buffer and halves the work of the separate qk_norm_rope_bwd pass. In exchange it adds register pressure, extra k_pre and rope table loads in the attention kernel, and a little more shared memory.

New measurement: 3.135, median of 6. No clear change (+0.5%).

```diff
diff --git a/include/osu_dreamer_hip.h b/include/osu_dreamer_hip.h
--- a/include/osu_dreamer_hip.h
+++ b/include/osu_dreamer_hip.h
@@ -74,6 +74,8 @@
 int od_qk_norm_rope_bwd(int dtype, const void* qkv, int ldqkv, const float* wq, const float* wk, const float* table,
                         const void* dqk, int lddqk, void* dqkv, int lddqkv, float* dwq, float* dwk, int B, int L,
                         int H, int hd, float eps, float q_scale, void* stream);
+int od_q_norm_rope_bwd(int dtype, const void* qkv, int ldqkv, const float* wq, const float* table, const void* dq, int lddq,
+                       void* dqkv, int lddqkv, float* dwq, int B, int L, int H, int hd, float eps, float q_scale, void* stream);
 int od_flash_attn_fwd(int dtype, const void* q, int ldq, const void* k, int ldk, const void* v, int ldv, void* o, int ldo,
                       float* lse, int B, int H, int L, int hd, float scale, int q_prescaled, void* stream);
 int od_flash_attn_fwd_varlen(int dtype, const void* q, int ldq, const void* k, int ldk, const void* v, int ldv, void* o, int ldo,
@@ -94,6 +96,10 @@
 int od_flash_attn_bwd_fused(int dtype, const void* q, int ldq, const void* k, int ldk, const void* v, int ldv, const void* o, int ldo,
                             const void* dout, int lddo, const float* lse, void* dq, int lddq, void* dk, int lddk, void* dv, int lddv,
                             int B, int H, int L, int hd, float scale, int q_prescaled, void* ws, long ws_bytes, void* stream);
+int od_flash_attn_bwd_fused_kfold(int dtype, const void* q, int ldq, const void* k, int ldk, const void* v, int ldv, const void* o, int ldo,
+                                  const void* dout, int lddo, const float* lse, void* dq, int lddq, void* dk, int lddk, void* dv, int lddv,
+                                  int B, int H, int L, int hd, float scale, int q_prescaled, const void* k_pre, int ldkpre,
+                                  const float* wk, const float* table, float eps, float* dwk, void* ws, long ws_bytes, void* stream);
 int od_flash_attn_bwd_fused_status(const void* ws, int* err_out, void* stream);
 int od_flash_attn_bwd_fused_err_offset(void);
 int od_flash_attn_bwd_fused_passes(void);
diff --git a/osu_dreamer_amd/csrc/attn_bwd_fused.hip b/osu_dreamer_amd/csrc/attn_bwd_fused.hip
--- a/osu_dreamer_amd/csrc/attn_bwd_fused.hip
+++ b/osu_dreamer_amd/csrc/attn_bwd_fused.hip
@@ -25,7 +25,8 @@
 constexpr int FB_NP = FB_PACK ? 3 : 4;
 constexpr int FB_RUN_TILE = 4 * FB_NP * 64 * 4;
 constexpr int FB_KST = 2 * FB_STAGE + 2 * FB_DS;
-constexpr int FB_SMEM = FB_KST + FB_DS + 16;
+constexpr int FB_DWK = FB_KST + FB_DS + 16;
+constexpr int FB_SMEM = FB_DWK + 64 * 8 + 16;
 
 #ifndef FB_ORDER
 #define FB_ORDER 3
@@ -63,6 +64,15 @@
     int shape[3];
     int pad;
     unsigned long long prof[16];
+};
+
+struct FbKFold {
+    const bf16_t* kpre; int ldkpre;
+    const float* wk;
+    const float* table;
+    float eps;
+    float* dwk;
+    const OdDetTable* det;
 };
 
 __device__ __forceinline__ unsigned fb_f2u(float x) { return __builtin_bit_cast(unsigned, x); }
@@ -215,17 +225,19 @@
     }
 }
 
-template <bool PRE, class TA>
+template <bool PRE, class TA, bool KF>
 __global__ __launch_bounds__(512, 2) void flash_bwd_fused_kernel(const bf16_t* __restrict__ q, int ldq, const bf16_t* __restrict__ k, int ldk,
                                                                  const bf16_t* __restrict__ v, int ldv, const bf16_t* __restrict__ dout, int lddo,
                                                                  const float* __restrict__ nl, const float* __restrict__ nd,
                                                                  bf16_t* __restrict__ dq, int lddq, bf16_t* __restrict__ dk, int lddk,
                                                                  bf16_t* __restrict__ dv, int lddv, float* __restrict__ run,
                                                                  FbSync* __restrict__ sync, int B, int H, int L, float scale,
-                                                                 unsigned wait_ticks, const float* __restrict__ dscale_p) {
+                                                                 unsigned wait_ticks, const float* __restrict__ dscale_p, FbKFold kf) {
     constexpr int NK = FB_NK, KB = FB_KB;
     OD_DYN_SMEM(smem);
     int* const s_job = (int*)(smem + FB_KST + FB_DS);
+    long long* const s_dwk = (long long*)(smem + FB_DWK);
+    int* const s_bad = (int*)(smem + FB_DWK + 64 * 8);
     const int BH = B * H, nkb = (L + KB - 1) / KB, nqt = (L + 63) / 64;
     const int jobs_per_xcd = ((BH + 7) / 8) * nkb;
     const int lane = threadIdx.x & 63, wave = od_uniform(threadIdx.x >> 6), x = lane & 15, g = lane >> 4;
@@ -244,6 +256,10 @@
     int my_jobs = 0;
 
     if (threadIdx.x == 0) s_job[0] = fb_atomic_inc(&sync->head[xcc]);
+    if constexpr (KF) {
+        if (threadIdx.x < 64) s_dwk[threadIdx.x] = 0;
+        if (threadIdx.x == 64) s_bad[0] = 0;
+    }
     __syncthreads();
     int job = od_uniform(s_job[0]), jpar = 0;
     auto run_jobs = [&](auto role_) FB_INLINE {
@@ -366,6 +382,81 @@
             for (int qt = 0; qt < nfull; qt++) tile(qt, std::false_type{});
             for (int qt = nfull; qt < nqt; qt++) tile(qt, std::true_type{});
             if (FB_PROF && threadIdx.x == 0) { atomicAdd(&sync->prof[0], pk_bar); atomicAdd(&sync->prof[1], FB_CLK() - tk0); }
+            if constexpr (KF) {
+                const int g4 = 4 * g;
+                float wv[4][4], dwl[4][4];
+#pragma unroll
+                for (int dt = 0; dt < 4; dt++) {
+                    const f32x4 w4 = *(const f32x4*)(kf.wk + dt * 16 + g4);
+#pragma unroll
+                    for (int r = 0; r < 4; r++) { wv[dt][r] = w4[r]; dwl[dt][r] = 0.f; }
+                }
+#pragma unroll
+                for (int ki = 0; ki < NK; ki++) {
+                    const int row = key0 + ki * 16 + x;
+                    const bool valid = row < L;
+                    const int rl = valid ? row : L - 1;
+                    const bf16_t* kp = kf.kpre + ((size_t)b * L + rl) * kf.ldkpre + h * 64 + g4;
+                    const float* tp = kf.table + ((size_t)rl * 32 + g4) * 2;
+                    float xv[4][4], cs[2][4], sn[2][4];
+#pragma unroll
+                    for (int dt = 0; dt < 4; dt++) {
+                        const u32x2 raw = *(const u32x2*)(kp + dt * 16);
+                        xv[dt][0] = fb_u2f(raw[0] << 16); xv[dt][1] = fb_u2f(raw[0] & 0xffff0000u);
+                        xv[dt][2] = fb_u2f(raw[1] << 16); xv[dt][3] = fb_u2f(raw[1] & 0xffff0000u);
+                    }
+#pragma unroll
+                    for (int dd = 0; dd < 2; dd++) {
+                        const f32x4 t0 = *(const f32x4*)(tp + dd * 32), t1 = *(const f32x4*)(tp + dd * 32 + 4);
+                        cs[dd][0] = t0[0]; sn[dd][0] = t0[1]; cs[dd][1] = t0[2]; sn[dd][1] = t0[3];
+                        cs[dd][2] = t1[0]; sn[dd][2] = t1[1]; cs[dd][3] = t1[2]; sn[dd][3] = t1[3];
+                    }
+                    float ss = 0.f;
+#pragma unroll
+                    for (int dt = 0; dt < 4; dt++)
+#pragma unroll
+                        for (int r = 0; r < 4; r++) ss += xv[dt][r] * xv[dt][r];
+                    ss += __shfl_xor(ss, 16); ss += __shfl_xor(ss, 32);
+                    const float inv = rsqrtf(ss / 64.f + kf.eps);
+                    float dy[4][4], dot = 0.f;
+#pragma unroll
+                    for (int dd = 0; dd < 2; dd++)
+#pragma unroll
+                        for (int r = 0; r < 4; r++) {
+                            const float d1 = dkacc[ki][dd][r] * out_scale, d2 = dkacc[ki][dd + 2][r] * out_scale;
+                            const float u1 = d1 * cs[dd][r] + d2 * sn[dd][r], u2 = d2 * cs[dd][r] - d1 * sn[dd][r];
+                            const float x1 = xv[dd][r] * inv, x2 = xv[dd + 2][r] * inv;
+                            if (valid) { dwl[dd][r] += u1 * x1; dwl[dd + 2][r] += u2 * x2; }
+                            dy[dd][r] = u1 * wv[dd][r]; dy[dd + 2][r] = u2 * wv[dd + 2][r];
+                            dot += dy[dd][r] * x1; dot += dy[dd + 2][r] * x2;
+                            xv[dd][r] = x1; xv[dd + 2][r] = x2;
+                        }
+                    dot += __shfl_xor(dot, 16); dot += __shfl_xor(dot, 32);
+                    dot /= 64.f;
+                    bf16_t* dkr = dk + ((size_t)b * L + rl) * lddk + h * 64;
+                    bf16_t* dvr = dv + ((size_t)b * L + rl) * lddv + h * 64;
+#pragma unroll
+                    for (int dt = 0; dt < 4; dt++) {
+                        const f32x4 e = dvacc[ki][dt] * inv_ds;
+                        u32x2 w0, w1;
+                        w0[0] = od_pack_bf2(inv * (dy[dt][0] - xv[dt][0] * dot), inv * (dy[dt][1] - xv[dt][1] * dot));
+                        w0[1] = od_pack_bf2(inv * (dy[dt][2] - xv[dt][2] * dot), inv * (dy[dt][3] - xv[dt][3] * dot));
+                        w1[0] = od_pack_bf2(e[0], e[1]); w1[1] = od_pack_bf2(e[2], e[3]);
+                        if (valid) {
+                            *(u32x2*)(dkr + dt * 16 + g4) = w0;
+                            *(u32x2*)(dvr + dt * 16 + g4) = w1;
+                        }
+                    }
+                }
+#pragma unroll
+                for (int dt = 0; dt < 4; dt++)
+#pragma unroll
+                    for (int r = 0; r < 4; r++) {
+                        float s = dwl[dt][r];
+                        s += __shfl_xor(s, 1); s += __shfl_xor(s, 2); s += __shfl_xor(s, 4); s += __shfl_xor(s, 8);
+                        if (x == 0) od_lds_fix_add(&s_dwk[dt * 16 + g4 + r], s, s_bad);
+                    }
+            } else {
 #pragma unroll
             for (int ki = 0; ki < NK; ki++) {
                 const int row = key0 + ki * 16 + x;
@@ -382,6 +473,7 @@
                         *(u32x2*)(dvr + dt * 16 + 4 * g) = w1;
                     }
                 }
+            }
             }
         } else {
             const int hh = wave - 4;
@@ -722,6 +814,21 @@
     }
     };
     if (key_wave) run_jobs(std::true_type{}); else run_jobs(std::false_type{});
+    if constexpr (KF) {
+        __syncthreads();
+        if (wave == 0) {
+#if defined(OD_EMU)
+            const int f = lane;
+#else
+            const int f = (int)__builtin_amdgcn_mbcnt_hi(~0u, __builtin_amdgcn_mbcnt_lo(~0u, 0u));
+#endif
+            const long long s = s_dwk[f];
+            const bool bad = s_bad[0] != 0;
+            long long* const shadow = od_det_find(kf.det, kf.dwk);
+            if (shadow && !bad) atomicAdd((unsigned long long*)(shadow + f), (unsigned long long)s);
+            else od_red_add(nullptr, kf.dwk + f, bad ? fb_poison() : od_unfix(s));
+        }
+    }
     if (threadIdx.x == 0) {
         if (my_jobs) {
 #if defined(OD_EMU)
@@ -805,9 +912,9 @@
     return 0;
 }
 
-extern "C" int od_flash_attn_bwd_fused(int dtype, const void* q, int ldq, const void* k, int ldk, const void* v, int ldv, const void* o, int ldo,
-                                       const void* dout, int lddo, const float* lse, void* dq, int lddq, void* dk, int lddk, void* dv, int lddv,
-                                       int B, int H, int L, int hd, float scale, int q_prescaled, void* ws, long ws_bytes, void* stream) {
+static int fb_run(int dtype, const void* q, int ldq, const void* k, int ldk, const void* v, int ldv, const void* o, int ldo,
+                  const void* dout, int lddo, const float* lse, void* dq, int lddq, void* dk, int lddk, void* dv, int lddv,
+                  int B, int H, int L, int hd, float scale, int q_prescaled, void* ws, long ws_bytes, void* stream, const FbKFold& kf) {
     if ((dtype != OD_BF16 && dtype != OD_F16) || hd != 64) return OD_ERR_UNSUPPORTED;
     if (!ws || B <= 0 || H <= 0 || L <= 0) return OD_ERR_ARG;
     if (ldq % 8 || ldk % 8 || ldv % 8 || ldo % 8 || lddo % 8 || lddq % 8 || lddk % 8 || lddv % 8) return OD_ERR_ALIGN;
@@ -840,19 +947,43 @@
     const int grid = od_num_cus();
 #define FB_ARGS dim3(grid), dim3(512), FB_SMEM, st, (const bf16_t*)q, ldq, (const bf16_t*)k, ldk, (const bf16_t*)v, ldv, (const bf16_t*)dout, lddo, \
         (const float*)nl, (const float*)nd, (bf16_t*)dq, lddq, (bf16_t*)dk, lddk, (bf16_t*)dv, lddv, (float*)(w + lay.run), (FbSync*)(w + lay.sync), B, H, L, scale, \
-        fb_wait_ticks(), dscale_p
+        fb_wait_ticks(), dscale_p, kf
 #define FB_LAUNCH_X(...) OD_LAUNCH_DYN(__VA_ARGS__)
-    if (f16) {
-        if (q_prescaled) FB_LAUNCH_X((flash_bwd_fused_kernel<true, f16_t>), FB_ARGS);
-        else FB_LAUNCH_X((flash_bwd_fused_kernel<false, f16_t>), FB_ARGS);
-    } else {
-        if (q_prescaled) FB_LAUNCH_X((flash_bwd_fused_kernel<true, bf16_t>), FB_ARGS);
-        else FB_LAUNCH_X((flash_bwd_fused_kernel<false, bf16_t>), FB_ARGS);
-    }
+#define FB_LAUNCH_KF(KFV)                                                                      \
+    do {                                                                                       \
+        if (f16) {                                                                             \
+            if (q_prescaled) FB_LAUNCH_X((flash_bwd_fused_kernel<true, f16_t, KFV>), FB_ARGS); \
+            else FB_LAUNCH_X((flash_bwd_fused_kernel<false, f16_t, KFV>), FB_ARGS);            \
+        } else {                                                                               \
+            if (q_prescaled) FB_LAUNCH_X((flash_bwd_fused_kernel<true, bf16_t, KFV>), FB_ARGS);\
+            else FB_LAUNCH_X((flash_bwd_fused_kernel<false, bf16_t, KFV>), FB_ARGS);           \
+        }                                                                                      \
+    } while (0)
+    if (kf.kpre) FB_LAUNCH_KF(true); else FB_LAUNCH_KF(false);
+#undef FB_LAUNCH_KF
 #undef FB_LAUNCH_X
 #undef FB_ARGS
     OD_CHECK_LAUNCH();
     return 0;
+}
+
+extern "C" int od_flash_attn_bwd_fused(int dtype, const void* q, int ldq, const void* k, int ldk, const void* v, int ldv, const void* o, int ldo,
+                                       const void* dout, int lddo, const float* lse, void* dq, int lddq, void* dk, int lddk, void* dv, int lddv,
+                                       int B, int H, int L, int hd, float scale, int q_prescaled, void* ws, long ws_bytes, void* stream) {
+    return fb_run(dtype, q, ldq, k, ldk, v, ldv, o, ldo, dout, lddo, lse, dq, lddq, dk, lddk, dv, lddv, B, H, L, hd, scale, q_prescaled, ws, ws_bytes,
+                  stream, FbKFold{});
+}
+
+extern "C" int od_flash_attn_bwd_fused_kfold(int dtype, const void* q, int ldq, const void* k, int ldk, const void* v, int ldv, const void* o, int ldo,
+                                             const void* dout, int lddo, const float* lse, void* dq, int lddq, void* dk, int lddk, void* dv, int lddv,
+                                             int B, int H, int L, int hd, float scale, int q_prescaled, const void* k_pre, int ldkpre,
+                                             const float* wk, const float* table, float eps, float* dwk, void* ws, long ws_bytes, void* stream) {
+    if (!k_pre || !wk || !table || !dwk) return OD_ERR_ARG;
+    if (ldkpre % 8 || ((size_t)k_pre & 7) || ((size_t)wk & 15) || ((size_t)table & 15)) return OD_ERR_ALIGN;
+    FbKFold kf;
+    kf.kpre = (const bf16_t*)k_pre; kf.ldkpre = ldkpre; kf.wk = wk; kf.table = table; kf.eps = eps; kf.dwk = dwk; kf.det = od_det_active();
+    return fb_run(dtype, q, ldq, k, ldk, v, ldv, o, ldo, dout, lddo, lse, dq, lddq, dk, lddk, dv, lddv, B, H, L, hd, scale, q_prescaled, ws, ws_bytes,
+                  stream, kf);
 }
 
 extern "C" int od_flash_attn_bwd_fused_status(const void* ws, int* err_out, void* stream) {
diff --git a/osu_dreamer_amd/csrc/rowops.hip b/osu_dreamer_amd/csrc/rowops.hip
--- a/osu_dreamer_amd/csrc/rowops.hip
+++ b/osu_dreamer_amd/csrc/rowops.hip
@@ -585,7 +585,7 @@
                                                                const T* __restrict__ dqk, int lddqk, T* __restrict__ dqkv, int lddqkv,
                                                                float* __restrict__ dwq, float* __restrict__ dwk,
                                                                int B, int L, int H, int hd, float eps, float q_scale,
-                                                               const OdDetTable* __restrict__ det) {
+                                                               const OdDetTable* __restrict__ det, int q_only) {
     __shared__ long long sdw[2][256];
     __shared__ int s_bad;
     const int lane = threadIdx.x & 63, wave = threadIdx.x >> 6;
@@ -593,7 +593,7 @@
     if (threadIdx.x == 0) s_bad = 0;
     __syncthreads();
     const int lph = hd / 8, half = lph / 2;
-    const int nchunks = 2 * H * lph;
+    const int nchunks = (q_only ? 1 : 2) * H * lph;
     const int niter = (nchunks + 63) / 64;
     float aq[8], ak[8];
 #pragma unroll
@@ -662,7 +662,7 @@
     __syncthreads();
     if (threadIdx.x < hd) {
         od_red_add(det, dwq + threadIdx.x, od_lds_unfix(sdw[0][threadIdx.x], s_bad));
-        od_red_add(det, dwk + threadIdx.x, od_lds_unfix(sdw[1][threadIdx.x], s_bad));
+        if (!q_only) od_red_add(det, dwk + threadIdx.x, od_lds_unfix(sdw[1][threadIdx.x], s_bad));
     }
 }
 
@@ -715,7 +715,7 @@
     }
 }
 
-template <class T, int LPH, int NIT>
+template <class T, int LPH, int NIT, bool QONLY = false>
 __global__ __launch_bounds__(256) void qk_norm_rope_pos_bwd_kernel(const T* __restrict__ qkv, int ldqkv, const float* __restrict__ wq,
                                                                    const float* __restrict__ wk, const float* __restrict__ table,
                                                                    const T* __restrict__ dqk, int lddqk, T* __restrict__ dqkv, int lddqkv,
@@ -747,14 +747,15 @@
         for (int e = 0; e < 8; e++) { cs[e] = tb[2 * e]; sn[e] = first ? tb[2 * e + 1] : -tb[2 * e + 1]; }
         for (int b = b0; b < b1; b++) {
             const long m = (long)b * L + l;
-            float v[NIT][8], d[NIT][8];
-#pragma unroll
-            for (int it = 0; it < NIT; it++) {
+            constexpr int NITW = QONLY ? NIT / 2 : NIT;
+            float v[NITW][8], d[NITW][8];
+#pragma unroll
+            for (int it = 0; it < NITW; it++) {
                 od_ld8(qkv + m * ldqkv + (size_t)(it * 64 + lane) * 8, v[it]);
                 od_ld8(dqk + m * lddqk + (size_t)(it * 64 + lane) * 8, d[it]);
             }
 #pragma unroll
-            for (int it = 0; it < NIT; it++) {
+            for (int it = 0; it < NITW; it++) {
                 const int qk = it < NIT / 2 ? 0 : 1;
                 const float gs = qk == 0 ? q_scale : 1.f;
                 float ss = 0.f;
@@ -787,15 +788,15 @@
 #pragma unroll
     for (int msk = LPH; msk < 64; msk <<= 1)
 #pragma unroll
-        for (int e = 0; e < 8; e++) { acc[0][e] += __shfl_xor(acc[0][e], msk); acc[1][e] += __shfl_xor(acc[1][e], msk); }
+        for (int e = 0; e < 8; e++) { acc[0][e] += __shfl_xor(acc[0][e], msk); if (!QONLY) acc[1][e] += __shfl_xor(acc[1][e], msk); }
     if (lane < LPH) {
 #pragma unroll
-        for (int e = 0; e < 8; e++) { od_lds_fix_add(&s_dw[0][c8 * 8 + e], acc[0][e], &s_bad); od_lds_fix_add(&s_dw[1][c8 * 8 + e], acc[1][e], &s_bad); }
+        for (int e = 0; e < 8; e++) { od_lds_fix_add(&s_dw[0][c8 * 8 + e], acc[0][e], &s_bad); if (!QONLY) od_lds_fix_add(&s_dw[1][c8 * 8 + e], acc[1][e], &s_bad); }
     }
     __syncthreads();
     if (threadIdx.x < HD) {
         od_red_add(det, dwq + threadIdx.x, od_lds_unfix(s_dw[0][threadIdx.x], s_bad));
-        od_red_add(det, dwk + threadIdx.x, od_lds_unfix(s_dw[1][threadIdx.x], s_bad));
+        if (!QONLY) od_red_add(det, dwk + threadIdx.x, od_lds_unfix(s_dw[1][threadIdx.x], s_bad));
     }
 }
 
@@ -1014,6 +1015,39 @@
     else
         OD_LAUNCH((qk_norm_rope_kernel<float>), grid, dim3(256), 0, (hipStream_t)stream, (const float*)qkv, ldqkv, wq, wk, table,
                   (float*)qk_out, ldo, B, L, H, hd, eps, q_scale);
+    OD_CHECK_LAUNCH();
+    return 0;
+}
+
+extern "C" int od_q_norm_rope_bwd(int dtype, const void* qkv, int ldqkv, const float* wq, const float* table, const void* dq, int lddq,
+                                  void* dqkv, int lddqkv, float* dwq, int B, int L, int H, int hd, float eps, float q_scale, void* stream) {
+    if (dtype != OD_BF16 && dtype != OD_F32) return OD_ERR_UNSUPPORTED;
+    if (hd % 16 || hd > 256 || 64 % (hd / 8)) return OD_ERR_UNSUPPORTED;
+    if (ldqkv % 8 || lddq % 8 || lddqkv % 8) return OD_ERR_ALIGN;
+    const int lph = hd / 8;
+    const int nit = 2 * H * lph / 64;
+    if (!((lph == 4 || lph == 8) && (H * lph) % 64 == 0 && (nit == 2 || nit == 4 || nit == 8))) {
+        const long M = (long)B * L;
+        dim3 grid((unsigned)((M + 4 * ROWS_PER_WAVE_BWD - 1) / (4 * ROWS_PER_WAVE_BWD)));
+        if (dtype == OD_BF16)
+            OD_LAUNCH((qk_norm_rope_bwd_kernel<bf16_t>), grid, dim3(256), 0, (hipStream_t)stream, (const bf16_t*)qkv, ldqkv, wq, wq, table,
+                      (const bf16_t*)dq, lddq, (bf16_t*)dqkv, lddqkv, dwq, (float*)nullptr, B, L, H, hd, eps, q_scale, od_det_active(), 1);
+        else
+            OD_LAUNCH((qk_norm_rope_bwd_kernel<float>), grid, dim3(256), 0, (hipStream_t)stream, (const float*)qkv, ldqkv, wq, wq, table,
+                      (const float*)dq, lddq, (float*)dqkv, lddqkv, dwq, (float*)nullptr, B, L, H, hd, eps, q_scale, od_det_active(), 1);
+        OD_CHECK_LAUNCH();
+        return 0;
+    }
+    int bpw, lpw; qk_pos_split(B, L, bpw, lpw);
+    lpw *= 4;
+    const long waves = (long)((L + lpw - 1) / lpw) * ((B + bpw - 1) / bpw);
+    dim3 g2((unsigned)((waves + 3) / 4));
+#define QPB(TT, LPHV, NITV) OD_LAUNCH((qk_norm_rope_pos_bwd_kernel<TT, LPHV, NITV, true>), g2, dim3(256), 0, (hipStream_t)stream, (const TT*)qkv, ldqkv, wq, wq, table, (const TT*)dq, lddq, (TT*)dqkv, lddqkv, dwq, (float*)nullptr, B, L, eps, q_scale, bpw, lpw, od_det_active())
+#define QPB_T(TT) do { if (lph == 8) { if (nit == 2) QPB(TT, 8, 2); else if (nit == 4) QPB(TT, 8, 4); else QPB(TT, 8, 8); } \
+                       else { if (nit == 2) QPB(TT, 4, 2); else if (nit == 4) QPB(TT, 4, 4); else QPB(TT, 4, 8); } } while (0)
+    if (dtype == OD_BF16) QPB_T(bf16_t); else QPB_T(float);
+#undef QPB_T
+#undef QPB
     OD_CHECK_LAUNCH();
     return 0;
 }
@@ -1045,10 +1079,10 @@
     dim3 grid((unsigned)((M + 4 * ROWS_PER_WAVE_BWD - 1) / (4 * ROWS_PER_WAVE_BWD)));
     if (dtype == OD_BF16)
         OD_LAUNCH((qk_norm_rope_bwd_kernel<bf16_t>), grid, dim3(256), 0, (hipStream_t)stream, (const bf16_t*)qkv, ldqkv, wq, wk, table,
-                  (const bf16_t*)dqk, lddqk, (bf16_t*)dqkv, lddqkv, dwq, dwk, B, L, H, hd, eps, q_scale, od_det_active());
+                  (const bf16_t*)dqk, lddqk, (bf16_t*)dqkv, lddqkv, dwq, dwk, B, L, H, hd, eps, q_scale, od_det_active(), 0);
     else
         OD_LAUNCH((qk_norm_rope_bwd_kernel<float>), grid, dim3(256), 0, (hipStream_t)stream, (const float*)qkv, ldqkv, wq, wk, table,
-                  (const float*)dqk, lddqk, (float*)dqkv, lddqkv, dwq, dwk, B, L, H, hd, eps, q_scale, od_det_active());
-    OD_CHECK_LAUNCH();
-    return 0;
-}
+                  (const float*)dqk, lddqk, (float*)dqkv, lddqkv, dwq, dwk, B, L, H, hd, eps, q_scale, od_det_active(), 0);
+    OD_CHECK_LAUNCH();
+    return 0;
+}
diff --git a/osu_dreamer_amd/engine.py b/osu_dreamer_amd/engine.py
--- a/osu_dreamer_amd/engine.py
+++ b/osu_dreamer_amd/engine.py
@@ -343,8 +343,8 @@
         wq, wk = self.P(p + "attn.q_norm.weight"), self.P(p + "attn.k_norm.weight")
         gq, gk = self.G(p + "attn.q_norm.weight"), self.G(p + "attn.k_norm.weight")
         scale = 1.0 / math.sqrt(self.hd)
-        dqk = self.buf("d.qk", (self.M, 2 * dh))
         if self.fused_attn_bwd():
+            dq = self.buf("d.q", (self.M, dh))
             key = (self.B, self.H, self.L, qk.device, qk.dtype)
             ws = self._attn_ws_cache.get(key)
             if ws is None:
@@ -353,22 +353,26 @@
                 ws = self._attn_ws_cache[key] = ops.FusedAttnBwdWorkspace(self.B, self.H, self.L, qk.device, qk.dtype)
                 ws.checked = False
             self._attn_ws = ws
-            ops.flash_attn_bwd_fused(qk[:, :dh], qk[:, dh:], self._v_of(qkv), y, dy, lse, dqk[:, :dh], dqk[:, dh:], dqkv[:, 2 * dh:],
-                                     self.B, self.H, self.L, self.hd, scale, self._attn_ws, q_prescaled=True)
+            ops.flash_attn_bwd_fused(qk[:, :dh], qk[:, dh:], self._v_of(qkv), y, dy, lse, dq, dqkv[:, dh:2 * dh], dqkv[:, 2 * dh:],
+                                     self.B, self.H, self.L, self.hd, scale, self._attn_ws, q_prescaled=True,
+                                     kfold=(qkv[:, dh:2 * dh], wk, t["rope"], FP32_EPS, gk))
+            if not core_only:
+                ops.q_norm_rope_bwd(qkv, wq, t["rope"], dq, dqkv, gq, self.B, self.L, self.H, self.hd, FP32_EPS, q_scale=self.q_scale)
+            return
+        dqk = self.buf("d.qk", (self.M, 2 * dh))
+        if (self._attn_aux is None or self._attn_aux.device != qk.device) and qk.is_cuda:
+            if self._attn_aux is not None:
+                self._attn_aux.close()
+            with torch.cuda.device(qk.device):
+                self._attn_aux = ops.AttnAux()
+            self._attn_aux.device = qk.device
+        if self.varlen:
+            ops.flash_attn_bwd_varlen(qk[:, :dh], qk[:, dh:], qkv[:, 2 * dh:], y, dy, lse, delta, dqk[:, :dh], dqk[:, dh:],
+                                      dqkv[:, 2 * dh:], self.ws.t["vl.lens"], self.B, self.H, self.L, self.hd, scale, q_prescaled=True,
+                                      aux=self._attn_aux)
         else:
-            if (self._attn_aux is None or self._attn_aux.device != qk.device) and qk.is_cuda:
-                if self._attn_aux is not None:
-                    self._attn_aux.close()
-                with torch.cuda.device(qk.device):
-                    self._attn_aux = ops.AttnAux()
-                self._attn_aux.device = qk.device
-            if self.varlen:
-                ops.flash_attn_bwd_varlen(qk[:, :dh], qk[:, dh:], qkv[:, 2 * dh:], y, dy, lse, delta, dqk[:, :dh], dqk[:, dh:],
-                                          dqkv[:, 2 * dh:], self.ws.t["vl.lens"], self.B, self.H, self.L, self.hd, scale, q_prescaled=True,
-                                          aux=self._attn_aux)
-            else:
-                ops.flash_attn_bwd(qk[:, :dh], qk[:, dh:], qkv[:, 2 * dh:], y, dy, lse, delta, dqk[:, :dh], dqk[:, dh:],
-                                   dqkv[:, 2 * dh:], self.B, self.H, self.L, self.hd, scale, q_prescaled=True, aux=self._attn_aux)
+            ops.flash_attn_bwd(qk[:, :dh], qk[:, dh:], qkv[:, 2 * dh:], y, dy, lse, delta, dqk[:, :dh], dqk[:, dh:],
+                               dqkv[:, 2 * dh:], self.B, self.H, self.L, self.hd, scale, q_prescaled=True, aux=self._attn_aux)
         if not core_only:
             ops.qk_norm_rope_bwd(qkv, wq, wk, t["rope"], dqk, dqkv, gq, gk, self.B, self.L, self.H, self.hd, FP32_EPS, q_scale=self.q_scale)
 
diff --git a/osu_dreamer_amd/ops.py b/osu_dreamer_amd/ops.py
--- a/osu_dreamer_amd/ops.py
+++ b/osu_dreamer_amd/ops.py
@@ -270,6 +270,12 @@
                                    _p(dqkv), _ld(dqkv), _p(dwq), _p(dwk), B, L, H, hd, eps, q_scale, _stream(qkv))
 
 
+def q_norm_rope_bwd(qkv, wq, table, dq, dqkv, dwq, B, L, H, hd, eps, q_scale=1.0):
+    _f32(wq, table, dwq)
+    _lib.lib().od_q_norm_rope_bwd(dt_code(qkv.dtype), _p(qkv), _ld(qkv), _p(wq), _p(table), _p(dq), _ld(dq), _p(dqkv), _ld(dqkv), _p(dwq),
+                                  B, L, H, hd, eps, q_scale, _stream(qkv))
+
+
 def flash_attn_fwd(q, k, v, o, lse, B, H, L, hd, scale, x3=False, q_prescaled=False):
     _f32(lse)
     assert q.dtype == k.dtype == v.dtype and (o.dtype == q.dtype or (q.dtype == torch.float16 and o.dtype == torch.bfloat16))
@@ -350,11 +356,19 @@
         return err.value
 
 
-def flash_attn_bwd_fused(q, k, v, o, do, lse, dq, dk, dv, B, H, L, hd, scale, ws: FusedAttnBwdWorkspace, q_prescaled=False):
+def flash_attn_bwd_fused(q, k, v, o, do, lse, dq, dk, dv, B, H, L, hd, scale, ws: FusedAttnBwdWorkspace, q_prescaled=False, kfold=None):
     _f32(lse)
     assert ws.shape == (B, H, L), (ws.shape, (B, H, L))
     assert q.dtype == k.dtype == v.dtype and o.dtype == do.dtype == dq.dtype == dk.dtype == dv.dtype == torch.bfloat16
     assert q.dtype == torch.bfloat16 or (q.dtype == torch.float16 and ws.dtype == torch.float16)
+    if kfold is not None:
+        k_pre, wk, table, eps, dwk = kfold
+        _f32(wk, table, dwk)
+        assert k_pre.dtype == torch.bfloat16 and table.shape[0] >= L
+        _lib.lib().od_flash_attn_bwd_fused_kfold(dt_code(q.dtype), _p(q), _ld(q), _p(k), _ld(k), _p(v), _ld(v), _p(o), _ld(o), _p(do), _ld(do),
+                                                 _p(lse), _p(dq), _ld(dq), _p(dk), _ld(dk), _p(dv), _ld(dv), B, H, L, hd, scale, int(q_prescaled),
+                                                 _p(k_pre), _ld(k_pre), _p(wk), _p(table), eps, _p(dwk), _p(ws.buf), ws.bytes, _stream(q))
+        return
     _lib.lib().od_flash_attn_bwd_fused(dt_code(q.dtype), _p(q), _ld(q), _p(k), _ld(k), _p(v), _ld(v), _p(o), _ld(o), _p(do), _ld(do),
                                        _p(lse), _p(dq), _ld(dq), _p(dk), _ld(dk), _p(dv), _ld(dv), B, H, L, hd, scale, int(q_prescaled),
                                        _p(ws.buf), ws.bytes, _stream(q))
```
